# D-Hank/NeRF-tiny

Hardware: AMD Instinct MI355X
Metric: rays/sec (64 coarse + 128 fine samples), lego 400x400 (higher is better)
Workload: dtype f32

## Files before the change

### nerf-tiny_amd/csrc/api.hip

```cpp
#include <math.h>
#include <stdlib.h>

#include <atomic>
#include <mutex>

#include "api_common.h"
#include "bf16_common.h"

using namespace nerf;

thread_local char nerf::g_err[512] = "";

namespace {

int next_pow2(int n) {
  int p = 2;
  while (p < n) p <<= 1;
  return p;
}

int check_sizes(int B, int Nc, int Nf) {
  if (B < 2) return fail(NERF_HIP_ERR_ARG, "B=%d: the reference needs B >= 2 (nerf.py:208 .squeeze())", B);
  if (Nc < 2 || Nc > 1024 || Nf < 1 || Nf > 1024) return fail(NERF_HIP_ERR_ARG, "Nc=%d Nf=%d outside 2..1024 / 1..1024", Nc, Nf);
  if ((long long)B * (Nc + Nf) + DUMP_ROWS + 256 >= (1ll << 31))
// ... 119 lines not shown
  }
  L.total = c.o;
  return L;
}

struct Prof {
  std::atomic<bool> on{false};
  std::mutex mu;
  int cap = 0, used = 0, pool_used = 0;
  hipEvent_t* ev = nullptr;
  hipEvent_t* e0 = nullptr;
  hipEvent_t* e1 = nullptr;
  int* kid = nullptr;
} g_prof;

struct ProfChain {
  hipEvent_t last = nullptr;
};

struct ProfScope {
  hipStream_t st;
  hipEvent_t stop = nullptr;
  ProfChain* chain;
  ProfScope(int kernel_id, hipStream_t s, ProfChain* ch = nullptr) : st(s), chain(ch) {
    if (!g_prof.on.load(std::memory_order_acquire)) return;
    hipEvent_t start = nullptr;
    bool record_start = false;
    {
      std::lock_guard<std::mutex> lk(g_prof.mu);
      if (g_prof.on.load(std::memory_order_relaxed) && g_prof.used < g_prof.cap) {
        const int slot = g_prof.used++;
        g_prof.kid[slot] = kernel_id;
        if (chain && chain->last) {
          start = chain->last;
        } else {
          start = g_prof.ev[g_prof.pool_used++];
          record_start = true;
        }
        stop = g_prof.ev[g_prof.pool_used++];
        g_prof.e0[slot] = start;
        g_prof.e1[slot] = stop;
      }
    }
    if (record_start) (void)hipEventRecord(start, st);
  }
  ~ProfScope() {
    if (stop) (void)hipEventRecord(stop, st);
    if (chain) chain->last = stop;
  }
};

}

extern "C" {

int nerf_hip_abi_version(void) { return NERF_HIP_ABI_VERSION; }

const char* nerf_hip_last_error(void) { return g_err; }

int nerf_hip_ws_bytes(int B, int Nc, int Nf, int flags, size_t* bytes) {
  if (!bytes) return fail(NERF_HIP_ERR_ARG, "bytes is null");
  if (int rc = check_sizes(B, Nc, Nf)) return rc;
  *bytes = layout(B, Nc, Nf, flags).total;
  return NERF_HIP_OK;
}

}

namespace {
struct TrainLoss {
  const float* C_true;
  float *dC_c, *dC_f, *terms, *loss;
  bool fused;
};
int forward_impl(const float* const* weights24, const int64_t* row, const int64_t* col, const float* poses_bound, const float* K_inv9,
                 const float* ray0_near_far, int B, int Nc, int Nf, float last_delta, float* C_coarse, float* C_fine, void* ws, size_t ws_bytes,
                 int flags, void* stream, TrainLoss* tl, float* maps = nullptr);
int backward_impl(const float* const* weights24, const float* dC_coarse, const float* dC_fine, const float* ray0_near_far, int B, int Nc, int Nf,
                  float last_delta, float* const* dweights24, void* ws, size_t ws_bytes, int flags, void* stream, void* early_event,
                  const TrainLoss* tl, const float* dmaps = nullptr);
}

extern "C" {

int nerf_hip_forward(const float* const* weights24, const int64_t* row, const int64_t* col, const float* poses_bound,
                     const float* K_inv9, const float* ray0_near_far, int B, int Nc, int Nf, float last_delta, float* C_coarse,
                     float* C_fine, void* ws, size_t ws_bytes, int flags, void* stream) {
  return forward_impl(weights24, row, col, poses_bound, K_inv9, ray0_near_far, B, Nc, Nf, last_delta, C_coarse, C_fine, ws, ws_bytes, flags, stream,
                      nullptr);
}

int nerf_hip_forward_maps(const float* const* weights24, const int64_t* row, const int64_t* col, const float* poses_bound,
                          const float* K_inv9, const float* ray0_near_far, int B, int Nc, int Nf, float last_delta, float* C_coarse,
                          float* C_fine, float* maps, void* ws, size_t ws_bytes, int flags, void* stream) {
  if (flags & NERF_HIP_SAVE_FOR_BACKWARD) return fail(NERF_HIP_ERR_ARG, "nerf_hip_forward_maps is inference only (NERF_HIP_SAVE_FOR_BACKWARD set)");
  if (!maps) return fail(NERF_HIP_ERR_ARG, "maps is null");
  return forward_impl(weights24, row, col, poses_bound, K_inv9, ray0_near_far, B, Nc, Nf, last_delta, C_coarse, C_fine, ws, ws_bytes, flags, stream,
                      nullptr, maps);
}

int nerf_hip_forward_maps_train(const float* const* weights24, const int64_t* row, const int64_t* col, const float* poses_bound,
                                const float* K_inv9, const float* ray0_near_far, int B, int Nc, int Nf, float last_delta, float* C_coarse,
                                float* C_fine, float* maps, void* ws, size_t ws_bytes, int flags, void* stream) {
  if (!(flags & NERF_HIP_SAVE_FOR_BACKWARD))
    return fail(NERF_HIP_ERR_ARG, "nerf_hip_forward_maps_train is training only (NERF_HIP_SAVE_FOR_BACKWARD not set)");
  if (!maps) return fail(NERF_HIP_ERR_ARG, "maps is null");
  return forward_impl(weights24, row, col, poses_bound, K_inv9, ray0_near_far, B, Nc, Nf, last_delta, C_coarse, C_fine, ws, ws_bytes, flags, stream,
                      nullptr, maps);
}

}

namespace {

int forward_impl(const float* const* weights24, const int64_t* row, const int64_t* col, const float* poses_bound, const float* K_inv9,
                 const float* ray0_near_far, int B, int Nc, int Nf, float last_delta, float* C_coarse, float* C_fine, void* ws, size_t ws_bytes,
                 int flags, void* stream, TrainLoss* tl, float* maps) {
  if (int rc = check_sizes(B, Nc, Nf)) return rc;
  if (int rc = check_weights(weights24)) return rc;
  if (!row || !col || !poses_bound || !K_inv9 || !C_coarse || !C_fine || !ws) return fail(NERF_HIP_ERR_ARG, "null argument");
  const WsLayout L = layout(B, Nc, Nf, flags);
  if (int rc = check_ws(ws, ws_bytes, L.total)) return rc;
  if (int rc = check_device()) return rc;
  hipStream_t st = static_cast<hipStream_t>(stream);
  const bool save = (flags & NERF_HIP_SAVE_FOR_BACKWARD) != 0;
  const bool bf16 = (flags & NERF_HIP_BF16_MLP) != 0;
  const bool bf16x = bf16 && !save && !(flags & NERF_HIP_FORCE_TILE_KERNEL);
  const bool split = (flags & NERF_HIP_SPLIT_MLP) && !bf16;
  const Weights24 w = as_w24(weights24);

  ProfChain pc;
  const bool one_prep = bf16 && !split && !prep_bf16_disabled();
  const bool corrected = (flags & NERF_HIP_CORRECTED) != 0;
  const bool pair = bf16x && Nc == 64 && Nf == 128 && pair_bf16(B) && !corrected && !maps;
  if (!(flags & NERF_HIP_WEIGHTS_UNCHANGED) && !one_prep) {
    ProfScope ps(NERF_HIP_K_PACK, st, &pc);
    if (bf16 || split) HIP_TRY(launch_fold_weights(w, at<float>(ws, L.fold), st));
    if (split) {
      HIP_TRY(launch_pack_weights_split(w, at<float>(ws, L.fold), at<unsigned char>(ws, L.packed_sp), st));
      if (save) HIP_TRY(launch_pack_weights_split_bwd(w, at<float>(ws, L.fold), at<unsigned char>(ws, L.packed_sp_bwd), st));
    } else
    if (bf16 && bf16x) HIP_TRY(launch_pack_weights_bf16x(w, at<float>(ws, L.fold), at<unsigned char>(ws, L.packed_bf), st));
    else if (bf16) HIP_TRY(launch_pack_weights_bf16(w, at<float>(ws, L.fold), at<unsigned char>(ws, L.packed_bf), st));
    else HIP_TRY(launch_pack_weights(w, at<float>(ws, L.fold), at<float4>(ws, L.packed), save ? NSEG : NSEG_FWD, st));
  }

  RaysArgs ra;
  memset(&ra, 0, sizeof(ra));
  ra.row = row; ra.col = col; ra.pb = poses_bound;
  memcpy(ra.K, K_inv9, 9 * sizeof(float));
  ra.B = B; ra.Nc = Nc;
  ra.rayf = at<float>(ws, L.rayf);
  ra.dvec = (bf16 || split) ? nullptr : at<float>(ws, L.dvec);
  ra.w_dir = w.p[W_DIR]; ra.b_dir = w.p[B_DIR];
  ra.b_fold = at<float>(ws, L.fold);
  ra.t_c = at<float>(ws, L.t_c);
  ra.status = at<unsigned>(ws, L.status);
  static std::atomic<unsigned> g_token{0};
  unsigned token = ++g_token;
  if ((token & 0xffffffu) == 0) token = ++g_token;
  if (one_prep) {
    const bool pack = !(flags & NERF_HIP_WEIGHTS_UNCHANGED);
    RaysArgs rp = ra;
    if (pair) rp.B = 0;
    if (pack || rp.B > 0) {
      ProfScope ps(pack ? NERF_HIP_K_PACK : NERF_HIP_K_RAYS, st, &pc);
      HIP_TRY(launch_prep_bf16(w, at<float>(ws, L.fold), pack ? at<unsigned char>(ws, L.packed_bf) : nullptr, bf16x ? 1 : 0,
                               pack && save ? at<unsigned char>(ws, L.packed_bf_bwd) : nullptr,
                               reinterpret_cast<unsigned*>(at<float>(ws, L.fold) + FOLD_FLOATS), token,
                               at<unsigned>(ws, L.status) + STATUS_STICKY_WORD, rp, st));
    }
  } else if (!pair) {
    ProfScope ps(NERF_HIP_K_RAYS, st, &pc);
    HIP_TRY(launch_rays(ra, st));
  }

  FieldArgs fa;
  memset(&fa, 0, sizeof(fa));
  fa.wp = at<float4>(ws, L.packed);
  if (bf16) fa.wbf = at<unsigned char>(ws, L.packed_bf);
  if (split) fa.wbf = at<unsigned char>(ws, L.packed_sp);
  fa.w = w;
  fa.rayf = at<float>(ws, L.rayf);
  fa.dvec = at<float>(ws, L.dvec);
  fa.t = at<float>(ws, L.t_c);
  fa.rgb = at<float>(ws, L.rgb_c);
  fa.sigma = at<float>(ws, L.sig_c);
  fa.N = Nc; fa.M = B * Nc;
#ifdef NERF_STAMPS
  fa.stamps = at<unsigned long long>(ws, L.dbg);
#endif
  const int tiles_c = (B * Nc + TM - 1) / TM, tiles_f = (B * Nf + TM - 1) / TM;
  if (save) {
    fa.spre = at<float>(ws, L.spre);
    fa.row0 = 0; fa.tile0 = 0; fa.tiles_tot = tiles_c + tiles_f; fa.Mtot = (long long)B * (Nc + Nf); fa.MSrows = fa.Mtot + DUMP_ROWS;
    if (bf16 || split) {
      fa.bsave = at<unsigned char>(ws, L.bsave); fa.bmask = at<uint16_t>(ws, L.bmask);
      if (split) fa.bsave2 = at<unsigned char>(ws, L.bsave2);
      fa.wb0 = 0; fa.wb_tot = (int)(wave_blocks(B, Nc) + wave_blocks(B, Nf));
    } else {
      fa.save = at<float>(ws, L.save); fa.masks = at<uint16_t>(ws, L.masks);
    }
  }
  if (pair) {
    PairArgs pa;
    memset(&pa, 0, sizeof(pa));
    pa.wbf = at<unsigned char>(ws, L.packed_bf); pa.rays = ra; pa.rays.status = nullptr; pa.B = B; pa.gen = token & 0xffffffu;
    if (ray0_near_far) { pa.ray0_override = 1; pa.near0 = ray0_near_far[0]; pa.far0 = ray0_near_far[1]; }
    pa.last = last_delta; pa.C_coarse = C_coarse; pa.C_fine = C_fine;
    pa.status = at<uint32_t>(ws, L.status); pa.sticky = at<uint32_t>(ws, L.status) + STATUS_STICKY_WORD;
    pa.sig_c = at<float>(ws, L.sig_c); pa.rgb_c = at<float>(ws, L.rgb_c); pa.w_c = at<float>(ws, L.w_c); pa.t_f = at<float>(ws, L.t_f);
    pa.sig_f = at<float>(ws, L.sig_f); pa.rgb_f = at<float>(ws, L.rgb_f);
    ProfScope ps(NERF_HIP_K_RENDER_PAIR, st, &pc);
    HIP_TRY(launch_render_pair_bf16x(pa, st));
    return NERF_HIP_OK;
  }
  const bool fuse_rays = bf16 && save && Nc == 64 && Nf == 128 && fuse_rays_bf16(B) && !corrected && !maps;
  FwdFuse ff;
  memset(&ff, 0, sizeof(ff));
  const bool tile_kernel = (flags & NERF_HIP_FORCE_TILE_KERNEL) != 0;
  auto field = [&](const FieldArgs& f) { return split ? launch_field_fwd_split(f, save, st) : bf16x ? launch_field_fwd_bf16x(f, st) : bf16 ? launch_field_fwd_bf16(f, save, st, ff.mode ? &ff : nullptr) : tile_kernel ? launch_field_fwd(f, save, st) : launch_field_fwd_reg(f, save, st); };

  CoarseArgs ca;
  memset(&ca, 0, sizeof(ca));
  ca.t_c = at<float>(ws, L.t_c); ca.sigma = at<float>(ws, L.sig_c); ca.rgb = at<float>(ws, L.rgb_c);
  ca.rayf = at<float>(ws, L.rayf);
  ca.B = B; ca.Nc = Nc; ca.Nf = Nf;
  ca.delta0_mode = 0;
  if (ray0_near_far) { ca.ray0_override = 1; ca.near0 = ray0_near_far[0]; ca.far0 = ray0_near_far[1]; }
  ca.w_c = at<float>(ws, L.w_c); ca.C_coarse = C_coarse; ca.t_f = at<float>(ws, L.t_f);
  ca.status = at<uint32_t>(ws, L.status);
  ca.sticky = at<uint32_t>(ws, L.status) + STATUS_STICKY_WORD;
  if (fuse_rays) {
    ff.mode = 1; ff.c = ca;
    { ProfScope ps(NERF_HIP_K_FIELD_COARSE, st, &pc); HIP_TRY(field(fa)); }
    ff.mode = 0;
  } else {
    { ProfScope ps(NERF_HIP_K_FIELD_COARSE, st, &pc); HIP_TRY(field(fa)); }
    { ProfScope ps(NERF_HIP_K_COARSE, st, &pc); HIP_TRY(launch_coarse(ca, st, maps)); }
  }

  fa.t = at<float>(ws, L.t_f);
  fa.rgb = at<float>(ws, L.rgb_f);
  fa.sigma = at<float>(ws, L.sig_f);
  fa.N = Nf; fa.M = B * Nf;
  if (save) { fa.row0 = B * Nc; fa.tile0 = tiles_c; fa.wb0 = (int)wave_blocks(B, Nc); }
  MergeArgs ma;
  memset(&ma, 0, sizeof(ma));
  ma.t_c = at<float>(ws, L.t_c); ma.t_f = at<float>(ws, L.t_f);
  ma.sig_c = at<float>(ws, L.sig_c); ma.sig_f = at<float>(ws, L.sig_f);
  ma.rgb_c = at<float>(ws, L.rgb_c); ma.rgb_f = at<float>(ws, L.rgb_f);
  ma.B = B; ma.Nc = Nc; ma.Nf = Nf; ma.P = next_pow2(Nc + Nf);
  ma.last = last_delta;
  ma.joint = corrected ? 1 : 0;
  if (save) { ma.bundle = at<float>(ws, L.bundle); ma.w = at<float>(ws, L.w_m); ma.perm = at<uint16_t>(ws, L.perm); }
  ma.C_fine = C_fine;
  if (fuse_rays) {
    ff.mode = 2; ff.m = ma;
    if (tl) {
      ff.C_true = tl->C_true; ff.C_coarse = C_coarse; ff.dC_c = tl->dC_c; ff.dC_f = tl->dC_f; ff.loss_terms = tl->terms;
      tl->fused = true;
    }
    { ProfScope ps(NERF_HIP_K_FIELD_FINE, st, &pc); HIP_TRY(field(fa)); }
  } else {
    { ProfScope ps(NERF_HIP_K_FIELD_FINE, st, &pc); HIP_TRY(field(fa)); }
    { ProfScope ps(NERF_HIP_K_MERGE, st, &pc); HIP_TRY(launch_merge(ma, st, maps)); }
  }
  return NERF_HIP_OK;
}

}

extern "C" {

int nerf_hip_profile_begin(int max_launches) {
  if (g_prof.ev) return fail(NERF_HIP_ERR_ARG, "profile already active");
  if (max_launches < 1 || max_launches > (1 << 20)) return fail(NERF_HIP_ERR_ARG, "bad max_launches");
  g_prof.ev = new hipEvent_t[2 * (size_t)max_launches];
  g_prof.e0 = new hipEvent_t[max_launches];
  g_prof.e1 = new hipEvent_t[max_launches];
  g_prof.kid = new int[max_launches];
  for (int i = 0; i < 2 * max_launches; ++i) HIP_TRY(hipEventCreate(&g_prof.ev[i]));
  g_prof.cap = max_launches;
  g_prof.used = 0;
  g_prof.pool_used = 0;
  g_prof.on.store(true, std::memory_order_release);
  return NERF_HIP_OK;
}

int nerf_hip_profile_end(double* ms_sum, int* count, int n_kernels) {
  if (!g_prof.ev) return fail(NERF_HIP_ERR_ARG, "profile not active");
  {
    std::lock_guard<std::mutex> lk(g_prof.mu);
    g_prof.on.store(false, std::memory_order_release);
  }
  for (int k = 0; k < n_kernels; ++k) { if (ms_sum) ms_sum[k] = 0.0; if (count) count[k] = 0; }
  int rc = NERF_HIP_OK;
  for (int i = 0; i < g_prof.used; ++i) {
    float ms = 0.f;
    hipError_t e = hipEventSynchronize(g_prof.e1[i]);
    if (e == hipSuccess) e = hipEventElapsedTime(&ms, g_prof.e0[i], g_prof.e1[i]);
    if (e != hipSuccess) { rc = fail(NERF_HIP_ERR_DEVICE, "profile event: %s", hipGetErrorString(e)); break; }
    const int k = g_prof.kid[i];
    if (k >= 0 && k < n_kernels) { if (ms_sum) ms_sum[k] += ms; if (count) count[k] += 1; }
  }
  for (int i = 0; i < 2 * g_prof.cap; ++i) (void)hipEventDestroy(g_prof.ev[i]);
// ... 156 lines not shown
    sg.save = save; sg.G = G; sg.dz = at<float>(ws, L.dz); sg.dspre = at<float>(ws, L.dspre); sg.rayf = at<float>(ws, L.rayf);
    sg.Mtot = Mtot; sg.MSrows = Mtot + DUMP_ROWS; sg.B = B; sg.Nc = Nc; sg.Nf = Nf;
    sg.dW_color = dw[W_COLOR]; sg.db_color = dw[B_COLOR]; sg.dw_sigma = dw[W_SIGMA]; sg.db_sigma = dw[B_SIGMA]; sg.dW_dir = dw[W_DIR];
    sg.sbuf = at<float>(ws, L.sbuf); sg.gdbuf = at<float>(ws, L.gdbuf); sg.sums_done = ray_duty ? 1 : 0;
    HIP_TRY(launch_small_grads(sg, slabs, st));
  }
  return NERF_HIP_OK;
}

}

extern "C" {

int nerf_hip_train_step(const float* const* weights24, const int64_t* row, const int64_t* col, const float* poses_bound,
                        const float* K_inv9, const float* ray0_near_far, const float* C_true, int B, int Nc, int Nf, float last_delta,
                        float* C_coarse, float* C_fine, float* loss, float* const* dweights24, void* ws, size_t ws_bytes, int flags,
                        void* stream, void* early_event) {
  if (!C_true || !loss || !C_coarse || !C_fine) return fail(NERF_HIP_ERR_ARG, "null argument");
  flags |= NERF_HIP_SAVE_FOR_BACKWARD;
  if (int rc = check_weights(const_cast<const float* const*>(dweights24))) return rc;
  if (int rc = check_sizes(B, Nc, Nf)) return rc;
  if (!ws) return fail(NERF_HIP_ERR_ARG, "null argument");
  const WsLayout L = layout(B, Nc, Nf, flags);
  if (ws_bytes < L.total) return fail(NERF_HIP_ERR_WORKSPACE, "workspace %zu < %zu bytes", ws_bytes, L.total);
  TrainLoss tl;
  tl.C_true = C_true; tl.dC_c = at<float>(ws, L.dC); tl.dC_f = tl.dC_c + (size_t)B * 3; tl.terms = tl.dC_f + (size_t)B * 3; tl.loss = loss;
  tl.fused = false;
  if (int rc = forward_impl(weights24, row, col, poses_bound, K_inv9, ray0_near_far, B, Nc, Nf, last_delta, C_coarse, C_fine, ws, ws_bytes, flags,
                            stream, &tl))
    return rc;
  if (!tl.fused)
    if (int rc = nerf_hip_ray_loss(C_coarse, C_fine, C_true, B, loss, tl.dC_c, tl.dC_f, stream)) return rc;
  return backward_impl(weights24, tl.dC_c, tl.dC_f, ray0_near_far, B, Nc, Nf, last_delta, dweights24, ws, ws_bytes,
                       flags & ~NERF_HIP_WEIGHTS_UNCHANGED, stream, early_event, &tl);
}

int nerf_hip_ws_offset(int B, int Nc, int Nf, int flags, const char* name, size_t* offset) {
  if (!name || !offset) return fail(NERF_HIP_ERR_ARG, "null argument");
  if (int rc = check_sizes(B, Nc, Nf)) return rc;
  const WsLayout L = layout(B, Nc, Nf, flags);
  struct { const char* n; size_t o; } tab[] = {
      {"status", L.status}, {"dbg", L.dbg}, {"packed", L.packed}, {"packed_bf", L.packed_bf}, {"bsave", L.bsave}, {"bsave2", L.bsave2}, {"bmask", L.bmask}, {"bG", L.bG}, {"bG2", L.bG2}, {"rayf", L.rayf}, {"dvec", L.dvec}, {"t_c", L.t_c}, {"sig_c", L.sig_c},
      {"rgb_c", L.rgb_c}, {"w_c", L.w_c}, {"t_f", L.t_f}, {"sig_f", L.sig_f}, {"rgb_f", L.rgb_f}, {"perm", L.perm},
      {"w_m", L.w_m}, {"bundle", L.bundle}, {"save", L.save}, {"masks", L.masks}, {"spre", L.spre}, {"G", L.G}, {"dz", L.dz},
      {"dspre", L.dspre}, {"mbuf", L.mbuf}, {"fold", L.fold}, {"drgb_c", L.drgb_c}, {"dsig_c", L.dsig_c}, {"drgb_f", L.drgb_f}, {"dsig_f", L.dsig_f},
      {"dt_f", L.dt_f}, {"slabs", L.slabs}, {"masks", L.masks}, {"sbuf", L.sbuf}, {"gdbuf", L.gdbuf}};
  for (auto& e : tab)
    if (strcmp(e.n, name) == 0) {
      if (e.o == 0 && strcmp(name, "status") != 0) return fail(NERF_HIP_ERR_ARG, "buffer %s is not part of this layout (flags=%d)", name, flags);
      *offset = e.o;
      return NERF_HIP_OK;
    }
  return fail(NERF_HIP_ERR_ARG, "unknown workspace buffer %s", name);
}

int nerf_hip_ray_loss(const float* C_coarse, const float* C_fine, const float* C_true, int B, float* loss, float* dC_coarse,
                      float* dC_fine, void* stream) {
  if (!C_coarse || !C_fine || !C_true || !loss || B < 1) return fail(NERF_HIP_ERR_ARG, "null argument");
  HIP_TRY(launch_ray_loss(C_coarse, C_fine, C_true, B, loss, dC_coarse, dC_fine, static_cast<hipStream_t>(stream)));
  return NERF_HIP_OK;
}

int nerf_hip_read_status(const void* ws, size_t ws_bytes, uint32_t* status, void* stream) {
  if (!ws || !status || ws_bytes < 256) return fail(NERF_HIP_ERR_ARG, "null argument");
  hipStream_t st = static_cast<hipStream_t>(stream);
  uint32_t w[STATUS_STICKY_WORD + 3];
  memset(w, 0, sizeof(w));
  HIP_TRY(hipMemcpyAsync(w, ws, sizeof(w), hipMemcpyDeviceToHost, st));
  HIP_TRY(hipStreamSynchronize(st));
  if (w[STATUS_SCHEME_WORD] == 1u) *status = ((w[STATUS_STAMPED_WORD] >> 8) == w[STATUS_GEN_WORD]) ? (w[STATUS_STAMPED_WORD] & 0xffu) : 0u;
  else *status = w[0] & ~(uint32_t)NERF_HIP_STATUS_PREP_TIMEOUT;
  if (w[STATUS_STICKY_WORD + 1] != 0u && w[STATUS_STICKY_WORD + 1] == w[STATUS_STICKY_WORD + 2]) *status |= NERF_HIP_STATUS_PREP_TIMEOUT;
  return NERF_HIP_OK;
}

int nerf_hip_read_status_sticky(void* ws, size_t ws_bytes, uint32_t* status, int clear, void* stream) {
  if (!ws || !status || ws_bytes < 256) return fail(NERF_HIP_ERR_ARG, "null argument");
  hipStream_t st = static_cast<hipStream_t>(stream);
  uint32_t* word = static_cast<uint32_t*>(ws) + STATUS_STICKY_WORD;
  HIP_TRY(hipMemcpyAsync(status, word, sizeof(uint32_t), hipMemcpyDeviceToHost, st));
  if (clear) HIP_TRY(hipMemsetAsync(word, 0, sizeof(uint32_t), st));
  HIP_TRY(hipStreamSynchronize(st));
  return NERF_HIP_OK;
}

int nerf_hip_rays(const int64_t* row, const int64_t* col, const float* poses_bound, const float* K_inv9, int B, int Nc,
                  float* d_cam, float* d_wrd, float* t_coarse, void* stream) {
  if (!row || !col || !poses_bound || !K_inv9 || B < 1 || Nc < 2) return fail(NERF_HIP_ERR_ARG, "bad argument");
  if (int rc = check_device()) return rc;
  RaysArgs ra;
  memset(&ra, 0, sizeof(ra));
  ra.row = row; ra.col = col; ra.pb = poses_bound;
  memcpy(ra.K, K_inv9, 9 * sizeof(float));
  ra.B = B; ra.Nc = Nc;
  ra.d_cam = d_cam; ra.d_wrd = d_wrd; ra.t_c = t_coarse;
  HIP_TRY(launch_rays(ra, static_cast<hipStream_t>(stream)));
  return NERF_HIP_OK;
}

int nerf_hip_field(const float* const* weights24, const int64_t* row, const int64_t* col, const float* poses_bound,
                   const float* K_inv9, const float* t, int B, int N, float* rgb, float* sigma, float* pts, float* gamma_p,
                   void* ws, size_t ws_bytes, void* stream) {
  if (B < 1 || N < 1 || N > 1024) return fail(NERF_HIP_ERR_ARG, "bad sizes");
  if (int rc = check_weights(weights24)) return rc;
  if (!row || !col || !poses_bound || !K_inv9 || !t || !rgb || !sigma || !ws) return fail(NERF_HIP_ERR_ARG, "null argument");
  const int Nl = N < 2 ? 2 : N;
  const WsLayout L = layout(B < 2 ? 2 : B, Nl, Nl, 0);
  if (ws_bytes < L.total) return fail(NERF_HIP_ERR_WORKSPACE, "workspace %zu < %zu bytes", ws_bytes, L.total);
  if (int rc = check_device()) return rc;
  hipStream_t st = static_cast<hipStream_t>(stream);
  const Weights24 w = as_w24(weights24);
  HIP_TRY(launch_pack_weights(w, at<float>(ws, L.fold), at<float4>(ws, L.packed), NSEG_FWD, st));
  RaysArgs ra;
  memset(&ra, 0, sizeof(ra));
  ra.row = row; ra.col = col; ra.pb = poses_bound;
  memcpy(ra.K, K_inv9, 9 * sizeof(float));
  ra.B = B; ra.Nc = Nl;
  ra.rayf = at<float>(ws, L.rayf);
  ra.dvec = at<float>(ws, L.dvec);
  ra.w_dir = w.p[W_DIR]; ra.b_dir = w.p[B_DIR]; ra.b_fold = at<float>(ws, L.fold);
  HIP_TRY(launch_rays(ra, st));
  FieldArgs fa;
  memset(&fa, 0, sizeof(fa));
  fa.wp = at<float4>(ws, L.packed);
  fa.w = w;
  fa.rayf = at<float>(ws, L.rayf);
  fa.dvec = at<float>(ws, L.dvec);
  fa.t = t; fa.rgb = rgb; fa.sigma = sigma; fa.pts_dbg = pts; fa.gp_dbg = gamma_p;
  fa.N = N; fa.M = B * N;
  HIP_TRY(launch_field_fwd_reg(fa, false, st));
  return NERF_HIP_OK;
}

int nerf_hip_field_bf16(const float* const* weights24, const int64_t* row, const int64_t* col, const float* poses_bound,
                        const float* K_inv9, const float* t, int B, int N, float* rgb, float* sigma, void* ws, size_t ws_bytes,
                        void* stream) {
  if (B < 1 || N < 1 || N > 1024) return fail(NERF_HIP_ERR_ARG, "bad sizes");
  if (int rc = check_weights(weights24)) return rc;
  if (!row || !col || !poses_bound || !K_inv9 || !t || !rgb || !sigma || !ws) return fail(NERF_HIP_ERR_ARG, "null argument");
  const int Nl = N < 2 ? 2 : N;
  const WsLayout L = layout(B < 2 ? 2 : B, Nl, Nl, NERF_HIP_BF16_MLP);
  if (ws_bytes < L.total) return fail(NERF_HIP_ERR_WORKSPACE, "workspace %zu < %zu bytes", ws_bytes, L.total);
  if (int rc = check_device()) return rc;
  hipStream_t st = static_cast<hipStream_t>(stream);
  const Weights24 w = as_w24(weights24);
  HIP_TRY(launch_fold_weights(w, at<float>(ws, L.fold), st));
  HIP_TRY(launch_pack_weights_bf16(w, at<float>(ws, L.fold), at<unsigned char>(ws, L.packed_bf), st));
  RaysArgs ra;
  memset(&ra, 0, sizeof(ra));
  ra.row = row; ra.col = col; ra.pb = poses_bound;
  memcpy(ra.K, K_inv9, 9 * sizeof(float));
  ra.B = B; ra.Nc = Nl;
  ra.rayf = at<float>(ws, L.rayf);
  HIP_TRY(launch_rays(ra, st));
  FieldArgs fa;
  memset(&fa, 0, sizeof(fa));
  fa.wbf = at<unsigned char>(ws, L.packed_bf);
  fa.w = w;
  fa.rayf = at<float>(ws, L.rayf);
  fa.t = t; fa.rgb = rgb; fa.sigma = sigma;
  fa.N = N; fa.M = B * N;
  HIP_TRY(launch_field_fwd_bf16(fa, false, st));
  return NERF_HIP_OK;
}

int nerf_hip_coarse_composite(const float* t_c, const float* sigma_c, const float* rgb_c, const float* near_far, float delta0,
                              int B, int Nc, int Nf, float* w_c, float* C_coarse, float* t_f, uint32_t* status, void* stream) {
  if (!t_c || !sigma_c || !rgb_c || !near_far || !t_f) return fail(NERF_HIP_ERR_ARG, "null argument");
  if (B < 1 || Nc < 2 || Nc > 1024 || Nf < 1 || Nf > 1024) return fail(NERF_HIP_ERR_ARG, "bad sizes");
  CoarseArgs ca;
  memset(&ca, 0, sizeof(ca));
  ca.t_c = t_c; ca.sigma = sigma_c; ca.rgb = rgb_c; ca.near_far = near_far;
  ca.B = B; ca.Nc = Nc; ca.Nf = Nf;
  ca.delta0_mode = 1; ca.delta0 = delta0;
  ca.w_c = w_c; ca.C_coarse = C_coarse; ca.t_f = t_f; ca.status = status;
  HIP_TRY(launch_coarse(ca, static_cast<hipStream_t>(stream)));
  return NERF_HIP_OK;
}

static const int kParamNumel[24] = {256 * 60, 256, 256 * 256, 256, 256 * 256, 256, 256 * 256, 256, 256 * 316, 256, 256 * 256, 256,
                                     256 * 256, 256, 256 * 256, 256, 256, 1, 256 * 256, 256, 128 * 280, 128, 3 * 128, 3};

int nerf_hip_adam_step(float* const* params24, const float* const* grads24, float* exp_avg, float* exp_avg_sq, int step, float lr,
                       float beta1, float beta2, float eps, void* stream) {
  if (!params24 || !grads24 || !exp_avg || !exp_avg_sq || step < 1) return fail(NERF_HIP_ERR_ARG, "bad argument");
  AdamArgs a;
  memset(&a, 0, sizeof(a));
  int off = 0;
  for (int i = 0; i < 24; ++i) {
    if (!params24[i] || !grads24[i]) return fail(NERF_HIP_ERR_ARG, "null tensor %d", i);
    a.param[i] = params24[i]; a.grad[i] = grads24[i]; a.numel[i] = kParamNumel[i]; a.offset[i] = off;
    off += kParamNumel[i];
  }
  a.m = exp_avg; a.v = exp_avg_sq;
  const double bc1 = 1.0 - pow((double)beta1, (double)step), bc2 = 1.0 - pow((double)beta2, (double)step);
  a.step_size = (float)((double)lr / bc1);
  a.bias2_sqrt = (float)sqrt(bc2);
  a.one_minus_beta1 = 1.0f - beta1; a.beta2 = beta2; a.one_minus_beta2 = 1.0f - beta2; a.eps = eps;
  HIP_TRY(launch_adam(a, static_cast<hipStream_t>(stream)));
  return NERF_HIP_OK;
}

int nerf_hip_gather_rays(const int64_t* index, const float* pixels, const float* poses17, int B, int H, int W, int64_t* row,
                         int64_t* col, int64_t* pic, float* pix_val, float* poses_bound, void* stream) {
  if (!index || !pixels || !poses17 || !row || !col || !pic || !pix_val || !poses_bound || B < 1 || H < 1 || W < 1)
    return fail(NERF_HIP_ERR_ARG, "bad argument");
  GatherArgs g;
  memset(&g, 0, sizeof(g));
  g.index = reinterpret_cast<const long long*>(index); g.pixels = pixels; g.poses = poses17; g.B = B; g.H = H; g.W = W;
  g.row = reinterpret_cast<long long*>(row); g.col = reinterpret_cast<long long*>(col); g.pic = reinterpret_cast<long long*>(pic);
  g.pix_val = pix_val; g.poses_bound = poses_bound;
  HIP_TRY(launch_gather_rays(g, static_cast<hipStream_t>(stream)));
  return NERF_HIP_OK;
}

int nerf_hip_coarse_composite_backward(const float* t_c, const float* sigma_c, const float* rgb_c, const float* near_far,
                                       float delta0, int B, int Nc, int Nf, const float* dC_coarse, const float* dt_f,
                                       float* dsig_c, float* drgb_c, void* stream) {
  if (!t_c || !sigma_c || !rgb_c || !near_far || !dC_coarse || !dt_f || !dsig_c || !drgb_c) return fail(NERF_HIP_ERR_ARG, "null argument");
  if (B < 1 || Nc < 2 || Nc > 1024 || Nf < 1 || Nf > 1024) return fail(NERF_HIP_ERR_ARG, "bad sizes");
  CoarseBwdArgs cb;
  memset(&cb, 0, sizeof(cb));
  cb.dC_c = dC_coarse; cb.dt_f = dt_f; cb.t_c = t_c; cb.sigma = sigma_c; cb.rgb = rgb_c; cb.near_far = near_far;
  cb.B = B; cb.Nc = Nc; cb.Nf = Nf; cb.delta0_mode = 1; cb.delta0 = delta0;
  cb.drgb_c = drgb_c; cb.dsig_c = dsig_c;
  HIP_TRY(launch_coarse_bwd(cb, static_cast<hipStream_t>(stream)));
  return NERF_HIP_OK;
}

int nerf_hip_merge_composite(const float* t_c, const float* t_f, const float* sigma_c, const float* sigma_f, const float* rgb_c,
                             const float* rgb_f, int B, int Nc, int Nf, float last_delta, float* bundle, float* w, float* C_fine,
                             void* stream) {
  if (!t_c || !t_f || !sigma_c || !sigma_f || !rgb_c || !rgb_f || !C_fine) return fail(NERF_HIP_ERR_ARG, "null argument");
  if (B < 1 || Nc < 1 || Nf < 1 || Nc + Nf > 2048) return fail(NERF_HIP_ERR_ARG, "bad sizes");
  MergeArgs ma;
  memset(&ma, 0, sizeof(ma));
  ma.t_c = t_c; ma.t_f = t_f; ma.sig_c = sigma_c; ma.sig_f = sigma_f; ma.rgb_c = rgb_c; ma.rgb_f = rgb_f;
  ma.B = B; ma.Nc = Nc; ma.Nf = Nf; ma.P = next_pow2(Nc + Nf); ma.last = last_delta;
  ma.bundle = bundle; ma.w = w; ma.C_fine = C_fine;
  HIP_TRY(launch_merge(ma, static_cast<hipStream_t>(stream)));
  return NERF_HIP_OK;
}

}
```

### nerf-tiny_amd/csrc/bf16_stream.h

```cpp
#pragma once
#include "bf16_common.h"
#include "field_common.h"

#include <stdlib.h>
#include <type_traits>
#include <utility>

namespace nerf {

typedef __bf16 bf16x8 __attribute__((ext_vector_type(8)));
typedef __bf16 bf16x2 __attribute__((ext_vector_type(2)));
typedef float f32x2 __attribute__((ext_vector_type(2)));
typedef short s16x2 __attribute__((ext_vector_type(2)));
typedef unsigned u32x4 __attribute__((ext_vector_type(4)));
typedef void __attribute__((address_space(3)))* lptr_t;

constexpr int BF_NS = 8;
constexpr int BF_SYNC_POS = 8;
constexpr int BF_D = 6;
constexpr int BF_EPI_POS = 2;
constexpr int BF_WG = 512;
constexpr int BF_LDS_BYTES = BF_BIAS_BYTES + BF_NS * BF_CHUNK * BF_FRAG_BYTES;
constexpr int BF_SMALL_MAX_WGS = 256;
inline bool bf16_four_waves_disabled() {
// ... 60 lines not shown
  c.lane = threadIdx.x & 63;
  c.wv = __builtin_amdgcn_readfirstlane(threadIdx.x >> 6);
  return c;
}

__device__ __forceinline__ void glds16(const unsigned char* gsrc, unsigned lds_dst) {
  unsigned keep;
  asm volatile("s_mov_b32 %0, m0\n\ts_mov_b32 m0, %2\n\ts_nop 0\n\tglobal_load_lds_dwordx4 %1, off\n\ts_mov_b32 m0, %0"
               : "=&s"(keep)
               : "v"(gsrc), "s"(lds_dst)
               : "memory");
}

__device__ __forceinline__ void store_piece(unsigned char* dst, const u32x4& v) {
  __builtin_nontemporal_store(v, reinterpret_cast<u32x4*>(dst));
}

template <class S>
__device__ __forceinline__ void bf_dma_chunk(const BfCtx& c, int chunk) {
  const int slot = chunk % S::NS;
  constexpr int PW = BfPW<S>::v;
#pragma unroll
  for (int e = 0; e < PW; ++e) {
    const int fr = PW * c.wv + e;
    glds16(c.wimg + BF_BIAS_BYTES + ((size_t)chunk * BF_CHUNK + fr) * BF_FRAG_BYTES + c.lane * 16,
           c.lds_base + S::RING_OFF + (slot * BF_CHUNK + fr) * BF_FRAG_BYTES);
  }
}

template <class S>
__device__ __forceinline__ constexpr int bf_wait_count(int c) {
  const int last = (c + S::NS - 2 < S::NCHUNK - 1) ? c + S::NS - 2 : S::NCHUNK - 1;
  const int loads = (last >= c + 2) ? BfPW<S>::v * (last - (c + 2) + 1) : 0;
  const int c_req = c + 2 - S::NS;
  const int now = S::stores_before(c * BF_CHUNK + BF_SYNC_POS);
  const int then = c_req >= 0 ? S::stores_before(c_req * BF_CHUNK + BF_SYNC_POS) : -S::PROLOGUE_STORES;
  const int n = loads + (now - then);
  return n > 63 ? 63 : n;
}

template <class S, int chunk>
__device__ __forceinline__ void bf_sync(const BfCtx& c) {
  wait_vmcnt<bf_wait_count<S>(chunk)>();
  __builtin_amdgcn_s_barrier();
  asm volatile("" ::: "memory");
  if (chunk + S::NS - 1 < S::NCHUNK) bf_dma_chunk<S>(c, chunk + S::NS - 1);
}

template <class S>
__device__ __forceinline__ void bf_stream_start(const BfCtx& c) {
  if constexpr (S::HAS_BIAS) {
    constexpr int PW = BfPW<S>::v;
#pragma unroll
    for (int e = 0; e < PW; ++e) {
      const int fr = PW * c.wv + e;
      glds16(c.wimg + fr * BF_FRAG_BYTES + c.lane * 16, c.lds_base + fr * BF_FRAG_BYTES);
    }
  }
#pragma unroll
  for (int ch = 0; ch < S::NS - 1; ++ch) bf_dma_chunk<S>(c, ch);
}

template <class S>
__device__ __forceinline__ u32x4 bf_frag(const BfCtx& c, int idx) {
  const int slot = (idx / BF_CHUNK) % S::NS;
  return *reinterpret_cast<const u32x4*>(c.lds + S::RING_OFF + (slot * BF_CHUNK + idx % BF_CHUNK) * BF_FRAG_BYTES + c.lane * 16);
}

template <class S>
__device__ __forceinline__ void bf_stream_first(const BfCtx& c, u32x4 (&fr)[S::D]) {
  constexpr int n = BfPW<S>::v * (S::NS - 2) + S::PROLOGUE_STORES;
  wait_vmcnt<(n > 63 ? 63 : n)>();
  __builtin_amdgcn_s_barrier();
  asm volatile("" ::: "memory");
  static_assert(S::D <= BF_CHUNK - BF_SYNC_POS, "a prefetched fragment must not lie in an unpublished chunk");
#pragma unroll
  for (int i = 0; i < S::D; ++i) fr[i] = bf_frag<S>(c, i);
}

__device__ __forceinline__ f32x16 bf_bias_tile(const BfCtx& c, int tile) {
  const int h = c.lane >> 5;
  f32x16 a;
#pragma unroll
  for (int g = 0; g < 4; ++g) {
    const float4 q = *reinterpret_cast<const float4*>(c.lds + (tile * 32 + 8 * g + 4 * h) * 4);
    a[4 * g + 0] = q.x;
    a[4 * g + 1] = q.y;
    a[4 * g + 2] = q.z;
    a[4 * g + 3] = q.w;
  }
  return a;
}

__device__ __forceinline__ f32x16 bf_mfma(const u32x4& a, const u32x4& b, const f32x16& c) {
  return __builtin_amdgcn_mfma_f32_32x32x16_bf16(__builtin_bit_cast(bf16x8, a), __builtin_bit_cast(bf16x8, b), c, 0, 0, 0);
}

template <class S, int ROW, class Epi, class PrevEpi>
__device__ __forceinline__ void bf_segment(const BfCtx& c, u32x4 (&fr)[S::D], f32x16 (&acc)[2], const u32x4* inA, const u32x4* inB,
                                           Epi&& epi, PrevEpi&& prev_epi) {
  constexpr BfSeg G = S::SEGS[ROW];
  constexpr int S0 = G.s0, NFT = G.nft, KSA = G.ksa, KSB = G.ksb, BT0 = G.bt0, KS = KSA + KSB;
  constexpr int P0 = bf_seg_p0(S::SEGS, ROW), NEXT_BT = bf_seg_next_bt(S::SEGS, S::NSEG, ROW);
  static_assert(KS > BF_EPI_POS + 1, "segment too short for the deferred epilogue");
  const f32x16 zero = {0.f, 0.f, 0.f, 0.f, 0.f, 0.f, 0.f, 0.f, 0.f, 0.f, 0.f, 0.f, 0.f, 0.f, 0.f, 0.f};
  static_for<NFT * KS>([&](auto I) {
    constexpr int f = I / KS, ks = I % KS, idx = S0 + I;
    constexpr int cur = (P0 + f) & 1, oth = (P0 + f + 1) & 1;
    if constexpr (idx % BF_CHUNK == BF_SYNC_POS) bf_sync<S, idx / BF_CHUNK>(c);
    const u32x4 a = fr[idx % S::D];
    if constexpr (idx + S::D < S::NFRAG) fr[idx % S::D] = bf_frag<S>(c, idx + S::D);
    if constexpr (ks < KSA)
      acc[cur] = bf_mfma(a, inA[ks], acc[cur]);
    else
      acc[cur] = bf_mfma(a, inB[ks - KSA], acc[cur]);
    if constexpr (ks == BF_EPI_POS) {
      if constexpr (f == 0)
        prev_epi(acc[oth]);
      else
        epi(f - 1, acc[oth]);
      if constexpr (f + 1 < NFT)
        acc[oth] = BT0 >= 0 ? bf_bias_tile(c, BT0 + f + 1) : zero;
      else if constexpr (NEXT_BT >= 0)
        acc[oth] = bf_bias_tile(c, NEXT_BT);
      else
        acc[oth] = zero;
    }
  });
}

template <int NFRAG_>
struct BfStoreTable {
  int cum[NFRAG_ + 1];
};
constexpr int bf_burst_kstep(int parts, int next_ks) { return BF_EPI_POS + (parts == 2 && next_ks >= BF_EPI_POS + 8 ? 7 : 0); }
template <int NFRAG_, int PARTS>
constexpr BfStoreTable<NFRAG_> bf_store_table(const BfSeg* segs, int nseg, int mul, int extra) {
  constexpr int NSTEP = NFRAG_ / PARTS;
  BfStoreTable<NFRAG_> t{};
  int ev[NSTEP + 1] = {};
  for (int r = 0; r < nseg; ++r) {
    if (segs[r].pieces == 0) continue;
    const int e = bf_seg_end(segs[r]) + bf_burst_kstep(PARTS, r + 1 < nseg ? bf_seg_ks(segs[r + 1]) : 0);
    if (e < NSTEP) ev[e] += mul * segs[r].pieces + extra;
  }
  int run = 0, step = 0;
  for (int i = 0; i <= NFRAG_; ++i) {
    while (step < i / PARTS) run += ev[step++];
    t.cum[i] = run;
  }
  return t;
}

template <int L>
__device__ __forceinline__ void encode_pair(const float (&v)[3], const uint32_t (&freq_bits)[L], int pi, float& sv, float& cv) {
  sv = 0.f;
  cv = 0.f;
  if (pi < 3 * L) {
    const int cc = pi / L, l = pi - L * cc;
    const float x = (cc == 0) ? v[0] : ((cc == 1) ? v[1] : v[2]);
    sincos_phase(x * __uint_as_float(freq_bits[l]), sv, cv);
  }
}
__device__ __forceinline__ void encode_point_pair(const float (&p)[3], int pi, float& sv, float& cv) { encode_pair(p, kFreqPointBits, pi, sv, cv); }
__device__ __forceinline__ void encode_dir_pair(const float (&d)[3], int pi, float& sv, float& cv) { encode_pair(d, kFreqDirBits, pi, sv, cv); }

}
```

### nerf-tiny_amd/csrc/common.h

```cpp
#pragma once
#include <hip/hip_runtime.h>
#include <stddef.h>
#include <stdint.h>

namespace nerf {

constexpr int WIDTH = 256;
constexpr int POINT_DIM = 60;
constexpr int DIR_DIM = 24;
constexpr int L_POINT = 10;
constexpr int L_DIR = 4;
constexpr int HALF = 128;
constexpr int TM = 64;
constexpr int STATUS_GEN_WORD = 1, STATUS_SCHEME_WORD = 2, STATUS_STAMPED_WORD = 3;
constexpr int STATUS_STICKY_WORD = 32;
constexpr int DBG_WORDS = 16384;
constexpr int DUMP_ROWS = 64;
constexpr int RAYF = 24;

enum { RF_R = 0, RF_O = 9, RF_DCAM = 12, RF_DWRD = 15, RF_NEAR = 18, RF_FAR = 19, RF_STEP = 20, RF_DELTA = 21 };

struct Seg { int off4; int nft; int kb; };
constexpr int SEG_L0 = 0, SEG_L1 = 1, SEG_L2 = 2, SEG_L3 = 3, SEG_L4A = 4, SEG_L4B = 5, SEG_L5 = 6, SEG_L6 = 7,
              SEG_L7 = 8, SEG_PI = 9, SEG_DIR = 10, SEG_FOLD = 11, NSEG_FWD = 12;
constexpr int SEG_T_DIR = 12, SEG_T_PI = 13, SEG_T_L7 = 14, SEG_T_L6 = 15, SEG_T_L5 = 16, SEG_T_L4A = 17, SEG_T_L4B = 18,
              SEG_T_L3 = 19, SEG_T_L2 = 20, SEG_T_L1 = 21, SEG_T_L0 = 22, SEG_T_FOLD = 23, NSEG = 24;

__host__ __device__ constexpr int seg_nft(int s) {
  return (s == SEG_DIR || s == SEG_FOLD) ? 4 : (s == SEG_T_L4B || s == SEG_T_L0) ? 2 : 8;
}
__host__ __device__ constexpr int seg_kb(int s) {
  return (s == SEG_L0 || s == SEG_L4B) ? 8 : (s == SEG_T_DIR || s == SEG_T_FOLD) ? 16 : 32;
}
__host__ __device__ constexpr int seg_off4(int s) {
  int o = 0;
  for (int i = 0; i < s; ++i) o += seg_nft(i) * seg_kb(i) * 64;
  return o;
}
constexpr int PACKED_FWD_F4 = seg_off4(NSEG_FWD);
constexpr int PACKED_ALL_F4 = seg_off4(NSEG);

#define NERF_FREQ_POINT_BITS 0x40490fdbu, 0x40d928aeu, 0x416a8b6cu, 0x41fd527bu, 0x4288cd33u, 0x4313c0fau, 0x439f953cu, 0x442c5befu, 0x44ba2881u, 0x45490fdbu
__device__ __constant__ const uint32_t kFreqPointBits[10] = {NERF_FREQ_POINT_BITS};
constexpr uint32_t kFreqPointLit[10] = {NERF_FREQ_POINT_BITS};
__device__ __constant__ const uint32_t kFreqDirBits[4] = {0x40490fdbu, 0x40fd527au, 0x419f953cu, 0x42490fdbu};

enum { W_L0 = 0, B_L0 = 1, W_SIGMA = 16, B_SIGMA = 17, W_PI = 18, B_PI = 19, W_DIR = 20, B_DIR = 21, W_COLOR = 22, B_COLOR = 23 };

struct Weights24 { const float* p[24]; };
constexpr int FOLD_FLOATS = HALF + HALF * WIDTH;
struct Grads24 { float* p[24]; };

struct WsLayout {
  size_t status, dbg, packed, packed_bf, packed_sp, fold, rayf, dvec, t_c, sig_c, rgb_c, w_c, t_f, sig_f, rgb_f;
  size_t packed_bf_bwd, bsave, bmask, bG, bslabs;
  size_t packed_sp_bwd, bsave2, bG2;
  size_t perm, w_m, bundle, save, masks, spre, G, dz, dspre, drgb_c, dsig_c, drgb_f, dsig_f, dt_f, slabs, sbuf, gdbuf, mbuf, dC;
  size_t total;
};

}
```

### nerf-tiny_amd/csrc/field_bwd_bf16.hip

```cpp
#include "bf16_stream.h"
#include "bf16_weights.h"
#include "ray_parts_bwd.h"
#include "ray_parts.h"

#include <string.h>

namespace nerf {

constexpr int BB_NS = 5;
constexpr int BB_MASK_BYTES = 8 * BM_LAYERS * 1024;
constexpr int BB_LDS_BYTES = BB_MASK_BYTES + BB_NS * BF_CHUNK * BF_FRAG_BYTES;

template <bool FINE>
struct BwdStream {
  static constexpr int NFRAG = FINE ? BBF_NFRAG : BBC_NFRAG;
  static constexpr int NCHUNK = FINE ? BBF_NCHUNK : BBC_NCHUNK;
  static constexpr int NS = BB_NS, RING_OFF = BB_MASK_BYTES, D = 4;
  static constexpr const BfSeg* SEGS = kBwdSegs;
  static constexpr int NSEG = FINE ? BSEG_N : BSEG_G0T;
  static constexpr bool HAS_BIAS = false;
  static constexpr int PROLOGUE_STORES = 2;
  static constexpr BfStoreTable<NFRAG> tab = bf_store_table<NFRAG, 1>(SEGS, NSEG, 1, 0);
  __device__ static constexpr int stores_before(int idx) { return tab.cum[idx]; }
};

template <bool FINE, int WAVES>
__global__ __launch_bounds__(64 * WAVES, 1) void k_field_bwd_bf16(const FieldBwdArgs a, const BwdFuse fz) {
  extern __shared__ __attribute__((aligned(16))) unsigned char lds[];
  using S = std::conditional_t<WAVES == 4, FourWaves<BwdStream<FINE>>, BwdStream<FINE>>;
  const BfCtx c = bf_ctx(a.wbf, lds);
  const int lane = c.lane, j = lane & 31, h = lane >> 5;
  const int m = blockIdx.x * (32 * WAVES) + c.wv * 32 + j;
  const bool valid = m < a.M;
  const int mc = valid ? m : a.M - 1;
  const int wb = a.wb0 + blockIdx.x * WAVES + c.wv;

  if (fz.mode != 0) {
    float* const scr = reinterpret_cast<float*>(lds);
    auto wave_fence = [] {
      asm volatile("s_waitcnt vmcnt(0) lgkmcnt(0)" ::: "memory");
      __builtin_amdgcn_wave_barrier();
    };
    if (FINE) {
      if (c.wv < WAVES / 4) {
        const int ray = blockIdx.x * (WAVES / 4) + c.wv;
        if (ray < fz.m.B) merge_bwd_ray(fz.m, ray, lane, scr + c.wv * 4 * 192, wave_fence);
      }
      if (blockIdx.x == 0 && fz.loss_terms) ray_loss_sum<64 * WAVES>(fz.loss_terms, 3 * fz.m.B, fz.loss, scr + 4 * 4 * 192, threadIdx.x);
    } else {
      if (c.wv < WAVES / 2) {
        const int ray_raw = blockIdx.x * (WAVES / 2) + c.wv;
        const bool live = ray_raw < fz.c.B;
        float* w = scr + c.wv * (5 * 64 + 64);
        coarse_bwd_ray(fz.c, live ? ray_raw : fz.c.B - 1, live, lane, w, reinterpret_cast<uint16_t*>(w + 5 * 64), wave_fence);
      }
    }
    __syncthreads();
  }
  float dz[3];
#pragma unroll
  for (int ch = 0; ch < 3; ++ch) {
    const float o = a.rgb[(size_t)mc * 3 + ch];
    dz[ch] = valid ? a.drgb[(size_t)mc * 3 + ch] * ((1.0f - o) * o) : 0.f;
  }
  const float sp = a.spre[a.row0 + mc];
  const float sgn = sp > 0.f ? 1.0f : (sp < 0.f ? -1.0f : 0.f);
  const float ds = valid ? a.dsig[mc] * sgn : 0.f;
  u32x4 zin[4];
  zin[0][0] = h == 0 ? pack2(dz[0], dz[1]) : 0u;
  zin[0][1] = h == 0 ? pack2(dz[2], ds) : 0u;
  zin[0][2] = 0u;
  zin[0][3] = 0u;
#pragma unroll
  for (int q = 0; q < 4; ++q) asm volatile("" : "+v"(zin[0][q]));
  zin[1] = zin[2] = zin[3] = u32x4{0u, 0u, 0u, 0u};

#pragma unroll
  for (int l = 0; l < BM_LAYERS; ++l)
    glds16(reinterpret_cast<const unsigned char*>(a.bmask) + ((size_t)l * a.wb_tot + wb) * 1024 + lane * 16,
           c.lds_base + (c.wv * BM_LAYERS + l) * 1024);
  bf_stream_start<S>(c);

  auto grad_piece = [&](int tensor, int ks, const u32x4& v, unsigned lane16) {
    store_piece(a.bG + ((size_t)a.wb_tot * bg_cum(tensor) + (size_t)wb * bg_ks(tensor) + ks) * BF_FRAG_BYTES + lane16, v);
  };
  grad_piece(BG_Z, 0, zin[0], lane * 16);
  grad_piece(BG_Z, 1, zin[1], lane * 16);

  u32x4 fr[S::D];
  bf_stream_first<S>(c, fr);

  u32x4 X[16], Y[16];
  f32x16 acc[2];
  const f32x16 zero = {0.f, 0.f, 0.f, 0.f, 0.f, 0.f, 0.f, 0.f, 0.f, 0.f, 0.f, 0.f, 0.f, 0.f, 0.f, 0.f};
  acc[0] = zero;
  const uint16_t* const mk = reinterpret_cast<const uint16_t*>(lds + c.wv * BM_LAYERS * 1024) + lane * 8;
  auto grad_to = [&](u32x4* out, int tensor, int mlayer, int ntiles = 8) {
    return [&, out, tensor, mlayer, ntiles](int f, const f32x16& A) {
      f32x16 D = A;
      if (mlayer >= 0) {
        const int bits = mk[mlayer * 512 + f];
#pragma unroll
        for (int r = 0; r < 16; ++r)
          D[r] = __uint_as_float(__float_as_uint(A[r]) & (unsigned)__builtin_amdgcn_sbfe(bits, 15 - r, 1));
      }
#pragma unroll
      for (int mh = 0; mh < 2; ++mh)
#pragma unroll
        for (int q = 0; q < 4; ++q) out[2 * f + mh][q] = pack2(D[8 * mh + 2 * q], D[8 * mh + 2 * q + 1]);
      if (f == ntiles - 1) {
        const unsigned lane16 = 16u * lane_id_here();
#pragma unroll
        for (int ks = 0; ks < 16; ++ks)
          if (ks < 2 * ntiles) grad_piece(tensor, ks, out[ks], lane16);
      }
    };
  };
  auto last_of = [](auto epi, int f) { return [epi, f](const f32x16& A) { epi(f, A); }; };
  auto nothing = [](const f32x16&) {};

  bf_segment<S, BSEG_COLT>(c, fr, acc, zin, nullptr, grad_to(X, BG_D, 8, 4), nothing);
  bf_segment<S, BSEG_FOLDT>(c, fr, acc, X, zin, grad_to(Y, BG_L0 + 7, 7), last_of(grad_to(X, BG_D, 8, 4), 3));
  bf_segment<S, BSEG_L7T>(c, fr, acc, Y, nullptr, grad_to(X, BG_L0 + 6, 6), last_of(grad_to(Y, BG_L0 + 7, 7), 7));
  bf_segment<S, BSEG_L6T>(c, fr, acc, X, nullptr, grad_to(Y, BG_L0 + 5, 5), last_of(grad_to(X, BG_L0 + 6, 6), 7));
  bf_segment<S, BSEG_L5T>(c, fr, acc, Y, nullptr, grad_to(X, BG_L0 + 4, 4), last_of(grad_to(Y, BG_L0 + 5, 5), 7));
  bf_segment<S, BSEG_L4T>(c, fr, acc, X, nullptr, grad_to(Y, BG_L0 + 3, 3), last_of(grad_to(X, BG_L0 + 4, 4), 7));
  bf_segment<S, BSEG_L3T>(c, fr, acc, Y, nullptr, grad_to(X, BG_L0 + 2, 2), last_of(grad_to(Y, BG_L0 + 3, 3), 7));
  bf_segment<S, BSEG_L2T>(c, fr, acc, X, nullptr, grad_to(Y, BG_L0 + 1, 1), last_of(grad_to(X, BG_L0 + 2, 2), 7));
  bf_segment<S, BSEG_L1T>(c, fr, acc, Y, nullptr, grad_to(X, BG_L0 + 0, 0), last_of(grad_to(Y, BG_L0 + 1, 1), 7));
  if constexpr (!FINE) {
    grad_to(X, BG_L0 + 0, 0)(7, acc[1]);
  } else {
    f32x16 dgp[2];
    {
      const unsigned lane16 = 16u * lane_id_here();
#pragma unroll
      for (int ks = 0; ks < 16; ++ks)
        Y[ks] = *reinterpret_cast<const u32x4*>(a.bG + ((size_t)a.wb_tot * bg_cum(BG_L0 + 4) + (size_t)wb * 16 + ks) * BF_FRAG_BYTES + lane16);
    }
    bf_segment<S, BSEG_G0T>(c, fr, acc, X, Y, [&](int, const f32x16& A) { dgp[0] = A; },
                                                 last_of(grad_to(X, BG_L0 + 0, 0), 7));
    dgp[1] = acc[1];
    const int lane_e = (int)lane_id_here();
    const int h_e = lane_e >> 5;
    const int m_e = blockIdx.x * (32 * WAVES) + c.wv * 32 + (lane_e & 31);
    const bool valid_e = m_e < a.M;
    const int mcl = valid_e ? m_e : a.M - 1;
    const int ray = mcl / a.N;
    const float* rf = a.rayf + (size_t)ray * RAYF;
    float p[3];
    sample_point(rf, a.t[mcl], p);
    float dp[3] = {0.f, 0.f, 0.f};
#pragma unroll
    for (int g8 = 0; g8 < 8; ++g8)
#pragma unroll
      for (int e = 0; e < 2; ++e) {
        const int pi = 4 * g8 + 2 * h_e + e;
        if (pi < 30) {
          const int cc = pi / 10, l = pi - 10 * cc;
          const float x = (cc == 0) ? p[0] : ((cc == 1) ? p[1] : p[2]);
          const float fl = __uint_as_float(kFreqPointBits[l]);
          float sn, cn;
          sincos_phase(x * fl, sn, cn);
          const float dgs = dgp[g8 >> 2][4 * (g8 & 3) + 2 * e], dgc = dgp[g8 >> 2][4 * (g8 & 3) + 2 * e + 1];
          const float contrib = fl * (cn * dgs - sn * dgc);
          if (cc == 0) dp[0] += contrib; else if (cc == 1) dp[1] += contrib; else dp[2] += contrib;
        }
      }
#pragma unroll
    for (int i = 0; i < 3; ++i) dp[i] += __shfl_xor(dp[i], 32);
    if (valid_e && h_e == 0) {
      const float dtp = __builtin_fmaf(rf[RF_DWRD + 2], dp[2], __builtin_fmaf(rf[RF_DWRD + 1], dp[1], rf[RF_DWRD] * dp[0]));
      a.dt[m_e] += dtp;
    }
  }
}

__global__ __launch_bounds__(256) void k_pack_weights_bf16_bwd(const Weights24 w, const float* __restrict__ fold, unsigned char* __restrict__ img) {
  const int gid = blockIdx.x * 256 + threadIdx.x;
  if (gid >= BBF_NCHUNK * BF_CHUNK * 64) return;
  const int frag = gid >> 6, lane = gid & 63;
  *reinterpret_cast<u32x4*>(img + BF_BIAS_BYTES + (size_t)frag * BF_FRAG_BYTES + lane * 16) = frag_lane_bf16<32, bb_weight>(w, fold, frag, lane);
}

hipError_t launch_pack_weights_bf16_bwd(const Weights24& w, const float* fold, unsigned char* img, hipStream_t st) {
  const int threads = BBF_NCHUNK * BF_CHUNK * 64;
  hipLaunchKernelGGL(k_pack_weights_bf16_bwd, dim3((threads + 255) / 256), dim3(256), 0, st, w, fold, img);
  return hipGetLastError();
}

hipError_t launch_field_bwd_bf16(const FieldBwdArgs& a, bool fine, hipStream_t st, const BwdFuse* fuse) {
  BwdFuse fz;
  if (fuse) fz = *fuse; else memset(&fz, 0, sizeof(fz));
  if (fz.mode && (a.N != (fine ? 128 : 64) || (fz.mode == 1) != fine)) return hipErrorInvalidValue;
  static std::atomic<unsigned long long> opted{0};
  if (hipError_t e = ensure_dynamic_lds(opted, {reinterpret_cast<const void*>(&k_field_bwd_bf16<false, 8>), reinterpret_cast<const void*>(&k_field_bwd_bf16<true, 8>),
                                                reinterpret_cast<const void*>(&k_field_bwd_bf16<false, 4>), reinterpret_cast<const void*>(&k_field_bwd_bf16<true, 4>)}, BB_LDS_BYTES)) return e;
  const int wgs = (a.M + BF_WG / 2 - 1) / (BF_WG / 2);
  if (bf16_small_pass(wgs)) {
    if (fine)
      hipLaunchKernelGGL((k_field_bwd_bf16<true, 4>), dim3(2 * wgs), dim3(256), BB_LDS_BYTES, st, a, fz);
    else
      hipLaunchKernelGGL((k_field_bwd_bf16<false, 4>), dim3(2 * wgs), dim3(256), BB_LDS_BYTES, st, a, fz);
    return hipGetLastError();
  }
  if (fine)
    hipLaunchKernelGGL((k_field_bwd_bf16<true, 8>), dim3(wgs), dim3(BF_WG), BB_LDS_BYTES, st, a, fz);
  else
    hipLaunchKernelGGL((k_field_bwd_bf16<false, 8>), dim3(wgs), dim3(BF_WG), BB_LDS_BYTES, st, a, fz);
  return hipGetLastError();
}

}
```

### nerf-tiny_amd/csrc/field_bwd_reg.hip

```cpp
#include "field_common.h"

namespace nerf {

constexpr int RMB = 32;

template <int NFT>
struct WStageB {
  float4 w[NFT];
};

__device__ __forceinline__ float f4cb(const float4& v, int c) { return c == 0 ? v.x : (c == 1 ? v.y : (c == 2 ? v.z : v.w)); }

__device__ __forceinline__ unsigned mask_word(const uint16_t* __restrict__ mlayer, int t) { return mlayer[((t & 1) * 2) * 256 + (t >> 1) * 64]; }

template <int KB, int NFT, int NKB, int NNFT, bool ZERO_INIT, bool MASK_IN, bool STORE = true, bool HAS_NEXT_MASK = MASK_IN>
__device__ __forceinline__ void reg_layer_bwd(const int seg, const int next_seg , int lane,
                                              const f32x16* prev, f32x16* acc, WStageB<8>& st0, const uint16_t* __restrict__ mlayer,
                                              const uint16_t* __restrict__ mnext, unsigned& mfirst, float* __restrict__ grow, const RegBuf& rb) {
  constexpr int KT = KB / 4;
  WStageB<8> st1;
  const f32x16 zero = {0.f, 0.f, 0.f, 0.f, 0.f, 0.f, 0.f, 0.f, 0.f, 0.f, 0.f, 0.f, 0.f, 0.f, 0.f, 0.f};
  f32x16 tin[2];
  unsigned mw = mfirst;
  auto activate = [&](int t) {
    unsigned mn = 0;
    if (MASK_IN) {
      if (t + 1 < KT) mn = mask_word(mlayer, t + 1);
      else if (mnext != nullptr) mfirst = mask_word(mnext, 0);
    }
#pragma unroll
    for (int r = 0; r < 16; ++r) tin[t & 1][r] = MASK_IN ? (((mw >> r) & 1u) ? prev[t][r] : 0.f) : prev[t][r];
    if (grow == nullptr) {
#pragma unroll
      for (int r = 0; r < 16; ++r) asm volatile("" : "+v"(tin[t & 1][r]));
    }
    if (grow != nullptr) {
#pragma unroll
      for (int g = 0; g < 4; ++g)
        store_row4(grow + 32 * t + 8 * g, make_float4(tin[t & 1][4 * g], tin[t & 1][4 * g + 1], tin[t & 1][4 * g + 2], tin[t & 1][4 * g + 3]));
    }
    if (MASK_IN) mw = mn;
  };
  activate(0);
  auto kblock = [&](int kb, const WStageB<8>& cur, WStageB<8>& ld) {
    if (kb + 1 < KB) {
#pragma unroll
      for (int f = 0; f < NFT; ++f) ld.w[f] = reg_ldw(rb, seg + (int)(f * KB + kb + 1) * 64);
    } else if (next_seg >= 0) {
#pragma unroll
      for (int f = 0; f < NNFT; ++f) ld.w[f] = reg_ldw(rb, next_seg + (int)(f * NKB) * 64);
    }
    __builtin_amdgcn_sched_barrier(0);
    if ((kb & 3) == 2 && (kb >> 2) + 1 < KT) activate((kb >> 2) + 1);
#pragma unroll
    for (int s = 0; s < 4; ++s) {
      const float b = tin[(kb >> 2) & 1][4 * (kb & 3) + s];
#pragma unroll
      for (int f = 0; f < NFT; ++f) {
        if (ZERO_INIT && kb == 0 && s == 0)
          acc[f] = __builtin_amdgcn_mfma_f32_32x32x2f32(f4cb(cur.w[f], s), b, zero, 0, 0, 0);
        else
          acc[f] = __builtin_amdgcn_mfma_f32_32x32x2f32(f4cb(cur.w[f], s), b, acc[f], 0, 0, 0);
      }
    }
  };
#pragma unroll
  for (int kb = 0; kb < KB; kb += 2) {
    kblock(kb, st0, st1);
    kblock(kb + 1, st1, st0);
  }
}

template <int KB, int NKB, int NNFT, bool ZERO_INIT, bool STORE, bool HAS_NEXT_MASK>
__device__ __forceinline__ void reg_layer_bwd_thin(const int seg, const int next_seg , int lane,
                                                   const f32x16* prev, f32x16* acc, WStageB<8>& st0, const uint16_t* __restrict__ mlayer,
                                                   const uint16_t* __restrict__ mnext, unsigned& mfirst, float* __restrict__ grow, const RegBuf& rb) {
  static_assert(KB == 32, "ring indexing below assumes 32 k-blocks");
  constexpr int KT = KB / 4, D = 8;
  WStageB<8> st1;
  const f32x16 zero = {0.f, 0.f, 0.f, 0.f, 0.f, 0.f, 0.f, 0.f, 0.f, 0.f, 0.f, 0.f, 0.f, 0.f, 0.f, 0.f};
  f32x16 tin[2];
  unsigned mw = mfirst;
  auto slot = [&](int kb, int f) -> float4& { return ((kb % D) < 4) ? st0.w[2 * (kb % 4) + f] : st1.w[2 * (kb % 4) + f]; };
  auto activate = [&](int t) {
    unsigned mn = 0;
    if (t + 1 < KT) mn = mask_word(mlayer, t + 1);
    else if (HAS_NEXT_MASK) mfirst = mask_word(mnext, 0);
#pragma unroll
    for (int r = 0; r < 16; ++r) tin[t & 1][r] = ((mw >> r) & 1u) ? prev[t][r] : 0.f;
    if (STORE) {
#pragma unroll
      for (int g = 0; g < 4; ++g)
        store_row4(grow + 32 * t + 8 * g, make_float4(tin[t & 1][4 * g], tin[t & 1][4 * g + 1], tin[t & 1][4 * g + 2], tin[t & 1][4 * g + 3]));
    } else {
#pragma unroll
      for (int r = 0; r < 16; ++r) asm volatile("" : "+v"(tin[t & 1][r]));
    }
    mw = mn;
  };
#pragma unroll
  for (int kb = 1; kb < D; ++kb)
#pragma unroll
    for (int f = 0; f < 2; ++f) slot(kb, f) = reg_ldw(rb, seg + (int)(f * KB + kb) * 64);
  activate(0);
#pragma unroll
  for (int kb = 0; kb < KB; ++kb) {
    if ((kb & 3) == 2 && (kb >> 2) + 1 < KT) activate((kb >> 2) + 1);
    const float4 w0 = slot(kb, 0), w1 = slot(kb, 1);
#pragma unroll
    for (int s = 0; s < 4; ++s) {
      const float b = tin[(kb >> 2) & 1][4 * (kb & 3) + s];
      if (ZERO_INIT && kb == 0 && s == 0) {
        acc[0] = __builtin_amdgcn_mfma_f32_32x32x2f32(f4cb(w0, s), b, zero, 0, 0, 0);
        acc[1] = __builtin_amdgcn_mfma_f32_32x32x2f32(f4cb(w1, s), b, zero, 0, 0, 0);
      } else {
        acc[0] = __builtin_amdgcn_mfma_f32_32x32x2f32(f4cb(w0, s), b, acc[0], 0, 0, 0);
        acc[1] = __builtin_amdgcn_mfma_f32_32x32x2f32(f4cb(w1, s), b, acc[1], 0, 0, 0);
      }
    }
    __builtin_amdgcn_sched_barrier(0);
    if (kb + D < KB) {
#pragma unroll
      for (int f = 0; f < 2; ++f) slot(kb, f) = reg_ldw(rb, seg + (int)(f * KB + kb + D) * 64);
    } else if (kb == KB - 4 && next_seg >= 0) {
#pragma unroll
      for (int f = 0; f < NNFT; ++f) st0.w[f] = reg_ldw(rb, next_seg + (int)(f * NKB) * 64);
    }
    __builtin_amdgcn_sched_barrier(0);
  }
}

#ifdef NERF_STAMPS
#define BSTAMP(slot)                                            \
  do {                                                          \
    __builtin_amdgcn_sched_barrier(0);                          \
    const unsigned long long t_ = __builtin_readcyclecounter(); \
    __builtin_amdgcn_sched_barrier(0);                          \
    tsum[slot] += t_ - tlast;                                   \
    tlast = t_;                                                 \
  } while (0)
#else
#define BSTAMP(slot) do { } while (0)
#endif

template <bool FINE, bool QUERY = false, bool RGB = true>
__global__ __launch_bounds__(64, 1) void k_field_bwd_reg(const FieldBwdArgs a) {
  static_assert(FINE || !QUERY, "the query form carries the chain back to the points");
#ifdef NERF_STAMPS
  unsigned long long tsum[8] = {0, 0, 0, 0, 0, 0, 0, 0};
  unsigned long long tlast = __builtin_readcyclecounter();
#endif
  const int lane = threadIdx.x, j = lane & 31, h = lane >> 5;
  const int m0 = blockIdx.x * RMB;
  const int m = m0 + j;
  const bool valid = m < a.M;
  const int mc = valid ? m : a.M - 1;
  const size_t MS = (size_t)a.MSrows * WIDTH;
  const long long rrow = valid ? (long long)(a.row0 + m) : a.Mtot + j;
  const size_t grow_off = (size_t)rrow * WIDTH + 4 * h;
  float* const grow = a.G + grow_off;
  const float* const srow = a.save + grow_off;
  const uint16_t* const mrow = a.masks + ((size_t)(a.tile0 + (m0 >> 6)) * 4 + ((m0 >> 5) & 1)) * 256 + h * 32 + j;
  const size_t MKS = (size_t)a.tiles_tot * 4 * 256;
  const RegBuf rb = reg_buf(a.wp, threadIdx.x);
  constexpr int L256 = 8 * 32 * 64;
  const f32x16 zero = {0.f, 0.f, 0.f, 0.f, 0.f, 0.f, 0.f, 0.f, 0.f, 0.f, 0.f, 0.f, 0.f, 0.f, 0.f, 0.f};

  WStageB<8> st0;
  if constexpr (RGB) {
#pragma unroll
    for (int f = 0; f < 8; ++f) st0.w[f] = reg_ldw(rb, seg_off4(SEG_T_FOLD) + (f * 16) * 64);
  } else {
#pragma unroll
    for (int f = 0; f < 8; ++f) st0.w[f] = reg_ldw(rb, seg_off4(SEG_T_L7) + (f * 32) * 64);
  }
  auto mlayer = [&](int layer) { return mrow + (size_t)layer * MKS; };
  unsigned mfirst = mask_word(mlayer(7), 0);

  f32x16 D0[4];
  float ds;
  {
    const float* crow = QUERY ? a.save + (size_t)a.MSrows * QGRAD_GP + (size_t)rrow * QGRAD_C + 4 * h : srow + S_C * MS;
    float4 cv[4][4];
    float dz[3];
    if constexpr (RGB) {
#pragma unroll
      for (int t = 0; t < 4; ++t)
#pragma unroll
        for (int g = 0; g < 4; ++g) cv[t][g] = *reinterpret_cast<const float4*>(crow + 32 * t + 8 * g);
#pragma unroll
      for (int ch = 0; ch < 3; ++ch) {
        const float o = a.rgb[(size_t)mc * 3 + ch];
        const float up = a.drgb[(size_t)mc * 3 + ch];
        dz[ch] = valid ? up * ((1.0f - o) * o) : 0.f;
      }
    }
    const float sp = a.spre[a.row0 + mc];
    const float sgn = sp > 0.f ? 1.0f : (sp < 0.f ? -1.0f : 0.f);
    if constexpr (QUERY)
      ds = valid ? (a.dsig != nullptr ? a.dsig[mc] : 1.0f) * sgn : 0.f;
    else
      ds = valid ? a.dsig[mc] * sgn : 0.f;
    if (!QUERY && valid && h == 0) {
      *reinterpret_cast<float4*>(a.dz + (size_t)(a.row0 + m) * 4) = make_float4(dz[0], dz[1], dz[2], ds);
      a.dspre[a.row0 + m] = ds;
    }
    const float* wc = a.w.p[W_COLOR] + 4 * h;
#pragma unroll
    for (int t = 0; t < (RGB ? 4 : 0); ++t) {
      float4 q0[4], q1[4], q2[4];
#pragma unroll
      for (int g = 0; g < 4; ++g) {
        q0[g] = *reinterpret_cast<const float4*>(wc + 32 * t + 8 * g);
        q1[g] = *reinterpret_cast<const float4*>(wc + HALF + 32 * t + 8 * g);
        q2[g] = *reinterpret_cast<const float4*>(wc + 2 * HALF + 32 * t + 8 * g);
      }
      __builtin_amdgcn_sched_barrier(0);
#pragma unroll
      for (int g = 0; g < 4; ++g) {
        const float v0 = __builtin_fmaf(q2[g].x, dz[2], __builtin_fmaf(q1[g].x, dz[1], q0[g].x * dz[0]));
        const float v1 = __builtin_fmaf(q2[g].y, dz[2], __builtin_fmaf(q1[g].y, dz[1], q0[g].y * dz[0]));
        const float v2 = __builtin_fmaf(q2[g].z, dz[2], __builtin_fmaf(q1[g].z, dz[1], q0[g].z * dz[0]));
        const float v3 = __builtin_fmaf(q2[g].w, dz[2], __builtin_fmaf(q1[g].w, dz[1], q0[g].w * dz[0]));
        D0[t][4 * g + 0] = cv[t][g].x > 0.f ? v0 : 0.f;
        D0[t][4 * g + 1] = cv[t][g].y > 0.f ? v1 : 0.f;
        D0[t][4 * g + 2] = cv[t][g].z > 0.f ? v2 : 0.f;
        D0[t][4 * g + 3] = cv[t][g].w > 0.f ? v3 : 0.f;
      }
      __builtin_amdgcn_sched_barrier(0);
    }
  }
  BSTAMP(0);
  f32x16 A[8], B[8];
  {
    const float dsb = (h == 0) ? ds : 0.f;
    const float* ws = a.w.p[W_SIGMA];
#pragma unroll
    for (int f = 0; f < 8; ++f) B[f] = __builtin_amdgcn_mfma_f32_32x32x2f32(ws[f * 32 + j], dsb, zero, 0, 0, 0);
  }
  if constexpr (RGB)
    reg_layer_bwd<16, 8, 32, 8, false, false>(seg_off4(SEG_T_FOLD), seg_off4(SEG_T_L7), lane, D0, B, st0, nullptr, nullptr, mfirst,
                                              QUERY ? a.G : grow + G_D * MS, rb);
  BSTAMP(1);
  BSTAMP(2);
  constexpr int sT7 = seg_off4(SEG_T_L7);
  reg_layer_bwd<32, 8, 32, 8, true, true>(sT7, sT7 + L256, lane, B, A, st0, mlayer(7), mlayer(6), mfirst, QUERY ? a.G : grow + 7 * MS, rb);
  reg_layer_bwd<32, 8, 32, 8, true, true>(sT7 + L256, sT7 + 2 * L256, lane, A, B, st0, mlayer(6), mlayer(5), mfirst, QUERY ? a.G : grow + 6 * MS, rb);
  reg_layer_bwd<32, 8, 32, 8, true, true>(sT7 + 2 * L256, seg_off4(SEG_T_L4A), lane, B, A, st0, mlayer(5), mlayer(4), mfirst, QUERY ? a.G : grow + 5 * MS, rb);
  BSTAMP(3);
  f32x16 accg[2];
  if (FINE) {
    reg_layer_bwd<32, 8, 32, 2, true, true>(seg_off4(SEG_T_L4A), seg_off4(SEG_T_L4B), lane, A, B, st0, mlayer(4), mlayer(4), mfirst, QUERY ? a.G : grow + 4 * MS, rb);
    reg_layer_bwd_thin<32, 32, 8, true, false, true>(seg_off4(SEG_T_L4B), seg_off4(SEG_T_L3), lane, A, accg, st0, mlayer(4), mlayer(3), mfirst, nullptr, rb);
  } else {
    reg_layer_bwd<32, 8, 32, 8, true, true>(seg_off4(SEG_T_L4A), seg_off4(SEG_T_L3), lane, A, B, st0, mlayer(4), mlayer(3), mfirst, grow + 4 * MS, rb);
  }
  BSTAMP(4);
  constexpr int sT3 = seg_off4(SEG_T_L3);
  reg_layer_bwd<32, 8, 32, 8, true, true>(sT3, sT3 + L256, lane, B, A, st0, mlayer(3), mlayer(2), mfirst, QUERY ? a.G : grow + 3 * MS, rb);
  reg_layer_bwd<32, 8, 32, 8, true, true>(sT3 + L256, sT3 + 2 * L256, lane, A, B, st0, mlayer(2), mlayer(1), mfirst, QUERY ? a.G : grow + 2 * MS, rb);
  unsigned mb0[8];
  if (!FINE) {
#pragma unroll
    for (int t = 0; t < 8; ++t) mb0[t] = mask_word(mlayer(0), t);
  }
  reg_layer_bwd<32, 8, 32, 2, true, true, true, FINE>(sT3 + 2 * L256, FINE ? seg_off4(SEG_T_L0) : -1, lane, B, A, st0, mlayer(1),
                                                      mlayer(0), mfirst, QUERY ? a.G : grow + 1 * MS, rb);
  BSTAMP(5);
  if (FINE) {
    reg_layer_bwd_thin<32, 32, 2, false, !QUERY, false>(seg_off4(SEG_T_L0), -1, lane, A, accg, st0, mlayer(0), nullptr, mfirst,
                                                        QUERY ? nullptr : grow, rb);
    const int lane_e = __builtin_amdgcn_mbcnt_hi(~0u, __builtin_amdgcn_mbcnt_lo(~0u, 0u));
    const int j_e = lane_e & 31, h_e = lane_e >> 5;
    const int m_e = blockIdx.x * RMB + j_e;
    const bool valid_e = m_e < a.M;
    const int mc_e = valid_e ? m_e : a.M - 1;
    const long long rrow_e = valid_e ? (long long)(a.row0 + m_e) : a.Mtot + j_e;
    const float* rf = QUERY ? nullptr : a.rayf + (size_t)(mc_e / a.N) * RAYF;
    const float* gprow = QUERY ? a.save + (size_t)rrow_e * QGRAD_GP + 4 * h_e : a.save + (size_t)rrow_e * WIDTH + 4 * h_e + S_GP * ((size_t)a.MSrows * WIDTH);
    float4 gq[8];
#pragma unroll
    for (int g8 = 0; g8 < 8; ++g8) gq[g8] = *reinterpret_cast<const float4*>(gprow + 8 * g8);
    float dp[3] = {0.f, 0.f, 0.f};
#pragma unroll
    for (int g8 = 0; g8 < 8; ++g8)
#pragma unroll
      for (int e = 0; e < 2; ++e) {
        const int pi = 4 * g8 + 2 * h_e + e;
        if (pi < 30) {
          const int c = pi / 10, l = pi - 10 * c;
          const float fl = __uint_as_float(kFreqPointBits[l]);
          const float sn = e == 0 ? gq[g8].x : gq[g8].z, cn = e == 0 ? gq[g8].y : gq[g8].w;
          const float dgs = accg[g8 >> 2][4 * (g8 & 3) + 2 * e], dgc = accg[g8 >> 2][4 * (g8 & 3) + 2 * e + 1];
          const float contrib = fl * (cn * dgs - sn * dgc);
          if (c == 0) dp[0] += contrib; else if (c == 1) dp[1] += contrib; else dp[2] += contrib;
        }
      }
#pragma unroll
    for (int c = 0; c < 3; ++c) dp[c] += __shfl_xor(dp[c], 32);
    if (QUERY && valid_e && h_e == 0) {
#pragma unroll
      for (int c = 0; c < 3; ++c) a.dt[(size_t)m_e * 3 + c] = dp[c];
    }
    if (!QUERY && valid_e && h_e == 0) {
      const float dtp = __builtin_fmaf(rf[RF_DWRD + 2], dp[2], __builtin_fmaf(rf[RF_DWRD + 1], dp[1], rf[RF_DWRD] * dp[0]));
      a.dt[m_e] += dtp;
    }
  } else {
#pragma unroll
    for (int t = 0; t < 8; ++t)
#pragma unroll
      for (int g = 0; g < 4; ++g) {
        float4 v;
        v.x = ((mb0[t] >> (4 * g + 0)) & 1u) ? A[t][4 * g + 0] : 0.f;
        v.y = ((mb0[t] >> (4 * g + 1)) & 1u) ? A[t][4 * g + 1] : 0.f;
        v.z = ((mb0[t] >> (4 * g + 2)) & 1u) ? A[t][4 * g + 2] : 0.f;
        v.w = ((mb0[t] >> (4 * g + 3)) & 1u) ? A[t][4 * g + 3] : 0.f;
        store_row4(grow + 32 * t + 8 * g, v);
      }
  }
#ifdef NERF_STAMPS
  BSTAMP(6);
  if (a.stamps && lane == 0) {
    for (int i = 0; i < 7; ++i) atomicAdd(a.stamps + (FINE ? 8 : 0) + i, tsum[i]);
    atomicAdd(a.stamps + (FINE ? 30 : 31), 1ull);
  }
#endif
}

hipError_t launch_query_grad_bwd(const FieldBwdArgs& a, bool rgb, hipStream_t st) {
  if (a.M <= 0) return hipSuccess;
  const unsigned tiles = (unsigned)(((long long)a.M + RMB - 1) / RMB);
  if (rgb)
    hipLaunchKernelGGL((k_field_bwd_reg<true, true, true>), dim3(tiles), dim3(64), 0, st, a);
  else
    hipLaunchKernelGGL((k_field_bwd_reg<true, true, false>), dim3(tiles), dim3(64), 0, st, a);
  return hipGetLastError();
}

hipError_t launch_field_bwd_reg(const FieldBwdArgs& a, bool fine, hipStream_t st) {
  const int tiles = (a.M + RMB - 1) / RMB;
  if (fine)
    hipLaunchKernelGGL(k_field_bwd_reg<true>, dim3(tiles), dim3(64), 0, st, a);
  else
    hipLaunchKernelGGL(k_field_bwd_reg<false>, dim3(tiles), dim3(64), 0, st, a);
  return hipGetLastError();
}

}
```

### nerf-tiny_amd/csrc/field_bwd_split.hip

```cpp
#include "bf16_split.h"

namespace nerf {

constexpr int SPB_WG = 256;
constexpr int SPB_NS = 7;
constexpr int SPB_MASK_BYTES = 4 * BM_LAYERS * 1024;
constexpr int SPB_LDS_BYTES = SPB_MASK_BYTES + SPB_NS * BF_CHUNK * BF_FRAG_BYTES;
static_assert(SPB_LDS_BYTES <= 160 * 1024, "LDS of one CU");
static_assert((2 * BBC_NFRAG) % BF_CHUNK == 0 && (2 * BBF_NFRAG) % BF_CHUNK == 0, "whole chunks");

template <bool FINE>
struct SplitBwdStream {
  static constexpr int NFRAG = 2 * (FINE ? BBF_NFRAG : BBC_NFRAG), NCHUNK = NFRAG / BF_CHUNK;
  static constexpr int NS = SPB_NS, RING_OFF = SPB_MASK_BYTES, D = 6, PW = 4;
  static constexpr const BfSeg* SEGS = kBwdSegs;
  static constexpr int NSEG = FINE ? BSEG_N : BSEG_G0T;
  static constexpr bool HAS_BIAS = false;
  static constexpr int PROLOGUE_STORES = 4;
  static constexpr BfStoreTable<NFRAG> tab = bf_store_table<NFRAG, 2>(SEGS, NSEG, 2, 0);
  __device__ static constexpr int stores_before(int idx) { return tab.cum[idx]; }
};

template <bool FINE>
__global__ __launch_bounds__(SPB_WG, 1) void k_field_bwd_split(const FieldBwdArgs a) {
  extern __shared__ __attribute__((aligned(16))) unsigned char lds[];
  using S = SplitBwdStream<FINE>;
  const BfCtx c = bf_ctx(a.wbf, lds);
  const int lane = c.lane, j = lane & 31, h = lane >> 5;
  const int m = blockIdx.x * (SPB_WG / 2) + c.wv * 32 + j;
  const bool valid = m < a.M;
  const int mc = valid ? m : a.M - 1;
  const int wb = a.wb0 + blockIdx.x * (SPB_WG / 64) + c.wv;

  float dz[3];
#pragma unroll
  for (int ch = 0; ch < 3; ++ch) {
    const float o = a.rgb[(size_t)mc * 3 + ch];
    dz[ch] = valid ? a.drgb[(size_t)mc * 3 + ch] * ((1.0f - o) * o) : 0.f;
  }
  const float sp = a.spre[a.row0 + mc];
  const float sgn = sp > 0.f ? 1.0f : (sp < 0.f ? -1.0f : 0.f);
  const float ds = valid ? a.dsig[mc] * sgn : 0.f;
  u32x4 zh[4], zm[4];
  {
    const HiMid e0 = split2(dz[0], dz[1]), e1 = split2(dz[2], ds);
    zh[0] = u32x4{h == 0 ? e0.hi : 0u, h == 0 ? e1.hi : 0u, 0u, 0u};
    zm[0] = u32x4{h == 0 ? e0.mid : 0u, h == 0 ? e1.mid : 0u, 0u, 0u};
  }
#pragma unroll
  for (int q = 0; q < 4; ++q) asm volatile("" : "+v"(zh[0][q]), "+v"(zm[0][q]));
  zh[1] = zh[2] = zh[3] = zm[1] = zm[2] = zm[3] = u32x4{0u, 0u, 0u, 0u};

#pragma unroll
  for (int l = 0; l < BM_LAYERS; ++l)
    glds16(reinterpret_cast<const unsigned char*>(a.bmask) + ((size_t)l * a.wb_tot + wb) * 1024 + lane * 16,
           c.lds_base + (c.wv * BM_LAYERS + l) * 1024);
  bf_stream_start<S>(c);

  auto grad_pair = [&](int tensor, int ks, const u32x4& vh, const u32x4& vm, unsigned lane16) {
    const size_t off = ((size_t)a.wb_tot * bg_cum(tensor) + (size_t)wb * bg_ks(tensor) + ks) * BF_FRAG_BYTES + lane16;
    store_piece(a.bG + off, vh);
    store_piece(a.bG2 + off, vm);
  };
  grad_pair(BG_Z, 0, zh[0], zm[0], lane * 16);
  grad_pair(BG_Z, 1, zh[1], zm[1], lane * 16);

  u32x4 fr[S::D];
  bf_stream_first<S>(c, fr);

  u32x4 Xh[16], Xm[16], Yh[16], Ym[16];
  f32x16 acc[2];
  const f32x16 zero = {0.f, 0.f, 0.f, 0.f, 0.f, 0.f, 0.f, 0.f, 0.f, 0.f, 0.f, 0.f, 0.f, 0.f, 0.f, 0.f};
  acc[0] = zero;
  const uint16_t* const mk = reinterpret_cast<const uint16_t*>(lds + c.wv * BM_LAYERS * 1024) + lane * 8;
  auto grad_to = [&](u32x4* oh, u32x4* om, int tensor, int mlayer, int ntiles = 8) {
    return [&, oh, om, tensor, mlayer, ntiles](int f, int part, int ph, const f32x16& A, EpiTmp& t) {
      const int mh = part >> 2, q = part & 3, r = 8 * mh + 2 * q;
      if (ph == 0) {
        const int bits = mk[mlayer * 512 + f];
        t.x0 = __uint_as_float(__float_as_uint(A[r]) & (unsigned)__builtin_amdgcn_sbfe(bits, 15 - r, 1));
        t.x1 = __uint_as_float(__float_as_uint(A[r + 1]) & (unsigned)__builtin_amdgcn_sbfe(bits, 14 - r, 1));
        t.hi = pack2(t.x0, t.x1);
        oh[2 * f + mh][q] = t.hi;
      } else if (ph == 1) {
        t.x0 -= __uint_as_float(t.hi << 16);
        t.x1 -= __uint_as_float(t.hi & 0xffff0000u);
      } else {
        om[2 * f + mh][q] = pack2(t.x0, t.x1);
        if (f == ntiles - 1 && part == 7) {
          const unsigned lane16 = 16u * lane_id_here();
#pragma unroll
          for (int ks = 0; ks < 16; ++ks)
            if (ks < 2 * ntiles) grad_pair(tensor, ks, oh[ks], om[ks], lane16);
        }
      }
    };
  };
  auto last_of = [](auto epi, int f) { return [epi, f](int part, int ph, const f32x16& A, EpiTmp& t) { epi(f, part, ph, A, t); }; };
  auto nothing = [](int, int, const f32x16&, EpiTmp&) {};

  auto gd = grad_to(Xh, Xm, BG_D, 8, 4);
  auto g7 = grad_to(Yh, Ym, BG_L0 + 7, 7), g6 = grad_to(Xh, Xm, BG_L0 + 6, 6), g5 = grad_to(Yh, Ym, BG_L0 + 5, 5), g4 = grad_to(Xh, Xm, BG_L0 + 4, 4);
  auto g3 = grad_to(Yh, Ym, BG_L0 + 3, 3), g2 = grad_to(Xh, Xm, BG_L0 + 2, 2), g1 = grad_to(Yh, Ym, BG_L0 + 1, 1), g0 = grad_to(Xh, Xm, BG_L0 + 0, 0);
  sp_segment<S, BSEG_COLT>(c, fr, acc, zh, zm, nullptr, nullptr, gd, nothing);
  sp_segment<S, BSEG_FOLDT>(c, fr, acc, Xh, Xm, zh, zm, g7, last_of(gd, 3));
  sp_segment<S, BSEG_L7T>(c, fr, acc, Yh, Ym, nullptr, nullptr, g6, last_of(g7, 7));
  sp_segment<S, BSEG_L6T>(c, fr, acc, Xh, Xm, nullptr, nullptr, g5, last_of(g6, 7));
  sp_segment<S, BSEG_L5T>(c, fr, acc, Yh, Ym, nullptr, nullptr, g4, last_of(g5, 7));
  sp_segment<S, BSEG_L4T>(c, fr, acc, Xh, Xm, nullptr, nullptr, g3, last_of(g4, 7));
  sp_segment<S, BSEG_L3T>(c, fr, acc, Yh, Ym, nullptr, nullptr, g2, last_of(g3, 7));
  sp_segment<S, BSEG_L2T>(c, fr, acc, Xh, Xm, nullptr, nullptr, g1, last_of(g2, 7));
  sp_segment<S, BSEG_L1T>(c, fr, acc, Yh, Ym, nullptr, nullptr, g0, last_of(g1, 7));
  if constexpr (!FINE) {
    EpiTmp t = {0.f, 0.f, 0u};
    static_for<8>([&](auto P) { static_for<3>([&](auto PH) { g0(7, (int)P, (int)PH, acc[1], t); }); });
  } else {
    f32x16 dgp[2];
    {
      const unsigned lane16 = 16u * lane_id_here();
#pragma unroll
      for (int ks = 0; ks < 16; ++ks) {
        const size_t off = ((size_t)a.wb_tot * bg_cum(BG_L0 + 4) + (size_t)wb * 16 + ks) * BF_FRAG_BYTES + lane16;
        Yh[ks] = *reinterpret_cast<const u32x4*>(a.bG + off);
        Ym[ks] = *reinterpret_cast<const u32x4*>(a.bG2 + off);
      }
    }
    auto take0 = [&](int, int part, int ph, const f32x16& A, EpiTmp&) { if (part == 0 && ph == 0) dgp[0] = A; };
    sp_segment<S, BSEG_G0T>(c, fr, acc, Xh, Xm, Yh, Ym, take0, last_of(g0, 7));
    dgp[1] = acc[1];
    const int lane_e = (int)lane_id_here();
    const int h_e = lane_e >> 5;
    const int m_e = blockIdx.x * (SPB_WG / 2) + c.wv * 32 + (lane_e & 31);
    const bool valid_e = m_e < a.M;
    const int mcl = valid_e ? m_e : a.M - 1;
    const int ray = mcl / a.N;
    const float* rf = a.rayf + (size_t)ray * RAYF;
    float p[3];
    sample_point(rf, a.t[mcl], p);
    float dp[3] = {0.f, 0.f, 0.f};
#pragma unroll
    for (int g8 = 0; g8 < 8; ++g8)
#pragma unroll
      for (int e = 0; e < 2; ++e) {
        const int pi = 4 * g8 + 2 * h_e + e;
        if (pi < 30) {
          const int cc = pi / 10, l = pi - 10 * cc;
          const float x = (cc == 0) ? p[0] : ((cc == 1) ? p[1] : p[2]);
          const float fl = __uint_as_float(kFreqPointBits[l]);
          float sn, cn;
          sincos_phase(x * fl, sn, cn);
          const float dgs = dgp[g8 >> 2][4 * (g8 & 3) + 2 * e], dgc = dgp[g8 >> 2][4 * (g8 & 3) + 2 * e + 1];
          const float contrib = fl * (cn * dgs - sn * dgc);
          if (cc == 0) dp[0] += contrib; else if (cc == 1) dp[1] += contrib; else dp[2] += contrib;
        }
      }
#pragma unroll
    for (int i = 0; i < 3; ++i) dp[i] += __shfl_xor(dp[i], 32);
    if (valid_e && h_e == 0) {
      const float dtp = __builtin_fmaf(rf[RF_DWRD + 2], dp[2], __builtin_fmaf(rf[RF_DWRD + 1], dp[1], rf[RF_DWRD] * dp[0]));
      a.dt[m_e] += dtp;
    }
  }
}

__global__ __launch_bounds__(256) void k_pack_weights_split_bwd(const Weights24 w, const float* __restrict__ fold, unsigned char* __restrict__ img) {
  const int gid = blockIdx.x * 256 + threadIdx.x;
  if (gid >= BBF_NFRAG * 64) return;
  const int step = gid >> 6, lane = gid & 63;
  const FragHiMid v = frag_lane_split<32, bb_weight>(w, fold, step, lane);
  unsigned char* dst = img + BF_BIAS_BYTES + (size_t)(2 * step) * BF_FRAG_BYTES + lane * 16;
  *reinterpret_cast<u32x4*>(dst) = v.hi;
  *reinterpret_cast<u32x4*>(dst + BF_FRAG_BYTES) = v.mid;
}

size_t split_bwd_image_bytes() { return (size_t)BF_BIAS_BYTES + (size_t)2 * BBF_NFRAG * BF_FRAG_BYTES; }

hipError_t launch_pack_weights_split_bwd(const Weights24& w, const float* fold, unsigned char* img, hipStream_t st) {
  const int threads = BBF_NFRAG * 64;
  hipLaunchKernelGGL(k_pack_weights_split_bwd, dim3((threads + 255) / 256), dim3(256), 0, st, w, fold, img);
  return hipGetLastError();
}

hipError_t launch_field_bwd_split(const FieldBwdArgs& a, bool fine, hipStream_t st) {
  if (!a.wbf || !a.bmask || !a.bG || !a.bG2) return hipErrorInvalidValue;
  static std::atomic<unsigned long long> opted{0};
  if (hipError_t e = ensure_dynamic_lds(opted, {reinterpret_cast<const void*>(&k_field_bwd_split<false>), reinterpret_cast<const void*>(&k_field_bwd_split<true>)},
                                        SPB_LDS_BYTES))
    return e;
  const int wgs = ((a.M + SPB_WG / 2 - 1) / (SPB_WG / 2) + 1) / 2 * 2;
  if (fine)
    hipLaunchKernelGGL(k_field_bwd_split<true>, dim3(wgs), dim3(SPB_WG), SPB_LDS_BYTES, st, a);
  else
    hipLaunchKernelGGL(k_field_bwd_split<false>, dim3(wgs), dim3(SPB_WG), SPB_LDS_BYTES, st, a);
  return hipGetLastError();
}

}
```

### nerf-tiny_amd/csrc/field_fwd_bf16.hip

```cpp
#include "bf16_stream.h"

#include <string.h>
#include "bf16_weights.h"
#include "ray_parts.h"

namespace nerf {

constexpr BfStoreTable<BF_NFRAG> kFwdStoreTable = bf_store_table<BF_NFRAG, 1>(kFwdSegs, FSEG_N, 1, 1);

constexpr int BFW_LDS_BYTES = BF_LDS_BYTES + BF_WG * 32;
static_assert(BFW_LDS_BYTES <= 160 * 1024, "LDS of one CU");

template <bool SAVE>
struct FwdStream {
  static constexpr int NFRAG = BF_NFRAG, NCHUNK = BF_NCHUNK, NS = BF_NS, RING_OFF = BF_BIAS_BYTES, D = BF_D;
  static constexpr const BfSeg* SEGS = kFwdSegs;
  static constexpr int NSEG = FSEG_N;
  static constexpr bool HAS_BIAS = true;
  static constexpr int PROLOGUE_STORES = SAVE ? 6 : 0;
  __device__ static constexpr int stores_before(int idx) { return SAVE ? kFwdStoreTable.cum[idx] : 0; }
};

template <bool SAVE, int WAVES>
__global__ __launch_bounds__(64 * WAVES, 1) void k_field_fwd_bf16(const FieldArgs a, const FwdFuse fz) {
  extern __shared__ __attribute__((aligned(16))) unsigned char lds[];
  const BfCtx c = bf_ctx(a.wbf, lds);
  const int lane = c.lane, j = lane & 31, h = lane >> 5;
  const int m = blockIdx.x * (32 * WAVES) + c.wv * 32 + j;
  const bool valid = m < a.M;
  const int mc = valid ? m : a.M - 1;
  const int ray = mc / a.N;

  const float* rf = a.rayf + (size_t)ray * RAYF;
  float p[3], dw[3];
  sample_point(rf, a.t[mc], p);
#pragma unroll
  for (int i = 0; i < 3; ++i) dw[i] = rf[RF_DWRD + i];
#pragma unroll
  for (int i = 0; i < 3; ++i) asm volatile("" : "+v"(p[i]), "+v"(dw[i]));

  using S = std::conditional_t<WAVES == 4, FourWaves<FwdStream<SAVE>>, FwdStream<SAVE>>;
  bf_stream_start<S>(c);

  u32x4 gp[4], gd[2];
#pragma unroll
  for (int ks = 0; ks < 4; ++ks)
#pragma unroll
    for (int q = 0; q < 4; ++q) {
      float sv, cv;
      encode_point_pair(p, 8 * ks + 2 * h + (q & 1) + 4 * (q >> 1), sv, cv);
      gp[ks][q] = pack2(sv, cv);
    }
#pragma unroll
  for (int ks = 0; ks < 2; ++ks)
#pragma unroll
    for (int q = 0; q < 4; ++q) {
      float sv, cv;
      encode_dir_pair(dw, 8 * ks + 2 * h + (q & 1) + 4 * (q >> 1), sv, cv);
      gd[ks][q] = pack2(sv, cv);
    }

  const int wb = a.wb0 + blockIdx.x * WAVES + c.wv;
  unsigned mw[4];
  auto save_piece = [&](int tensor, int ks, const u32x4& v, unsigned lane16) {
    store_piece(a.bsave + ((size_t)a.wb_tot * bs_cum(tensor) + (size_t)wb * bs_ks(tensor) + ks) * BF_FRAG_BYTES + lane16, v);
  };
  if (SAVE) {
#pragma unroll
    for (int ks = 0; ks < 4; ++ks) save_piece(BS_GP, ks, gp[ks], lane * 16);
#pragma unroll
    for (int ks = 0; ks < 2; ++ks) save_piece(BS_GD, ks, gd[ks], lane * 16);
  }

  u32x4* const gd_park = reinterpret_cast<u32x4*>(lds + BF_LDS_BYTES) + 2 * threadIdx.x;
  gd_park[0] = gd[0];
  gd_park[1] = gd[1];

  u32x4 fr[S::D];
  bf_stream_first<S>(c, fr);

  u32x4 X[16], Y[16];
  f32x16 acc[2];
  acc[0] = bf_bias_tile(c, BFB_L0);
  auto relu_to = [&](u32x4* out, int tensor = -1, int mlayer = -1, int ntiles = 8) {
    return [&, out, tensor, mlayer, ntiles](int f, const f32x16& A) {
#pragma unroll
      for (int mh = 0; mh < 2; ++mh)
#pragma unroll
        for (int q = 0; q < 4; ++q) out[2 * f + mh][q] = pack2_relu(A[8 * mh + 2 * q], A[8 * mh + 2 * q + 1]);
      if constexpr (SAVE) {
        if (f & 1)
          mw[f >> 1] |= alive_bits(A) << 16;
        else
          mw[f >> 1] = alive_bits(A);
        if (f == ntiles - 1) {
          const unsigned lane16 = 16u * lane_id_here();
          u32x4 mv = {mw[0], mw[1], ntiles > 4 ? mw[2] : 0u, ntiles > 4 ? mw[3] : 0u};
          store_piece(reinterpret_cast<unsigned char*>(a.bmask) + ((size_t)mlayer * a.wb_tot + wb) * 1024 + lane16, mv);
#pragma unroll
          for (int ks = 0; ks < 16; ++ks)
            if (ks < 2 * ntiles) save_piece(tensor, ks, out[ks], lane16);
        }
      }
    };
  };
  auto last_of = [](auto epi, int f) { return [epi, f](const f32x16& A) { epi(f, A); }; };
  auto nothing = [](const f32x16&) {};
  auto nothing_f = [](int, const f32x16&) {};

  bf_segment<S, FSEG_L0>(c, fr, acc, gp, nullptr, relu_to(X, BS_H0 + 0, 0), nothing);
  bf_segment<S, FSEG_L1>(c, fr, acc, X, nullptr, relu_to(Y, BS_H0 + 1, 1), last_of(relu_to(X, BS_H0 + 0, 0), 7));
  bf_segment<S, FSEG_L2>(c, fr, acc, Y, nullptr, relu_to(X, BS_H0 + 2, 2), last_of(relu_to(Y, BS_H0 + 1, 1), 7));
  bf_segment<S, FSEG_L3>(c, fr, acc, X, nullptr, relu_to(Y, BS_H0 + 3, 3), last_of(relu_to(X, BS_H0 + 2, 2), 7));
  bf_segment<S, FSEG_L4>(c, fr, acc, Y, gp, relu_to(X, BS_H0 + 4, 4), last_of(relu_to(Y, BS_H0 + 3, 3), 7));
  bf_segment<S, FSEG_L5>(c, fr, acc, X, nullptr, relu_to(Y, BS_H0 + 5, 5), last_of(relu_to(X, BS_H0 + 4, 4), 7));
  bf_segment<S, FSEG_L6>(c, fr, acc, Y, nullptr, relu_to(X, BS_H0 + 6, 6), last_of(relu_to(Y, BS_H0 + 5, 5), 7));
  bf_segment<S, FSEG_L7>(c, fr, acc, X, nullptr, relu_to(Y, BS_H0 + 7, 7), last_of(relu_to(X, BS_H0 + 6, 6), 7));
  float spre = 0.f;
  auto sig_epi = [&](const f32x16& A) { spre = A[0]; };
  bf_segment<S, FSEG_SIG>(c, fr, acc, Y, nullptr, nothing_f, last_of(relu_to(Y, BS_H0 + 7, 7), 7));
  {
    const int lane_d = (int)lane_id_here();
    const u32x4* const back = reinterpret_cast<const u32x4*>(lds + BF_LDS_BYTES) + 2 * (c.wv * 64 + lane_d);
    gd[0] = back[0];
    gd[1] = back[1];
  }
  bf_segment<S, FSEG_DIR>(c, fr, acc, gd, Y, relu_to(X, BS_C, 8, 4), sig_epi);
  const int lane_e = (int)lane_id_here();
  const int m_e = blockIdx.x * (32 * WAVES) + c.wv * 32 + (lane_e & 31);
  const bool out_e = m_e < a.M && lane_e < 32;
  if (out_e) {
    a.sigma[m_e] = fabsf(spre);
    if (SAVE) a.spre[a.row0 + m_e] = spre;
  }
  unsigned char* const park_w = lds + BF_LDS_BYTES + c.wv * 2048;
  if (SAVE && fz.mode != 0 && lane_e < 32) reinterpret_cast<float*>(park_w)[lane_e] = fabsf(spre);
  bf_segment<S, FSEG_COL>(c, fr, acc, X, nullptr, nothing_f, last_of(relu_to(X, BS_C, 8, 4), 3));
  {
    const float r0 = 1.0f / (1.0f + expf(-acc[1][0])), r1 = 1.0f / (1.0f + expf(-acc[1][1])), r2 = 1.0f / (1.0f + expf(-acc[1][2]));
    if (out_e) {
      a.rgb[(size_t)m_e * 3 + 0] = r0;
      a.rgb[(size_t)m_e * 3 + 1] = r1;
      a.rgb[(size_t)m_e * 3 + 2] = r2;
    }
    if (SAVE && fz.mode != 0 && lane_e < 32) {
      float* pr = reinterpret_cast<float*>(park_w + 128) + 3 * lane_e;
      pr[0] = r0; pr[1] = r1; pr[2] = r2;
    }
  }
  if constexpr (SAVE) {
    if (fz.mode != 0) {
      asm volatile("s_waitcnt lgkmcnt(0)" ::: "memory");
      __builtin_amdgcn_s_barrier();
      asm volatile("" ::: "memory");
      float* const scr = reinterpret_cast<float*>(lds + BF_BIAS_BYTES);
      const unsigned char* const park = lds + BF_LDS_BYTES;
      const int lane_f = (int)__builtin_amdgcn_mbcnt_hi(~0u, __builtin_amdgcn_mbcnt_lo(~0u, 0u));
      auto wave_fence = [] {
        asm volatile("s_waitcnt lgkmcnt(0)" ::: "memory");
        __builtin_amdgcn_wave_barrier();
      };
      if (fz.mode == 1) {
        if (c.wv < WAVES / 2) {
          float* w = scr + c.wv * (3 * 64 + 4 * 64);
          float* sg = w + 3 * 64;
          float* cl = sg + 64;
          sg[lane_f] = park_sigma(park, 64 * c.wv + lane_f);
#pragma unroll
          for (int k = 0; k < 3; ++k) cl[3 * lane_f + k] = park_rgb(park, 64 * c.wv + lane_f, k);
          wave_fence();
          const int ray_raw = blockIdx.x * (WAVES / 2) + c.wv;
          const size_t g0 = (size_t)(ray_raw < fz.c.B ? ray_raw : fz.c.B - 1) * 64;
          CoarseArgs ca = fz.c;
          ca.sigma = sg - g0;
          ca.rgb = cl - 3 * g0;
          coarse_ray_stage(ca, ray_raw, lane_f, w, w + 64, w + 128, wave_fence);
        }
      } else {
        constexpr int R = WAVES / 4;
        float* const val0 = scr;
        uint16_t* const idx0 = reinterpret_cast<uint16_t*>(scr + R * 5 * 256);
        for (int j = c.wv; j < 5 * R; j += WAVES) {
          const int rl = j / 5, ch = j - 5 * rl;
          const int ray = blockIdx.x * R + rl;
          if (ray < fz.m.B) merge_channel_job(fz.m, ray, ch, lane_f, val0 + (rl * 5 + ch) * 256, idx0 + (rl * 5 + ch) * 256, park, 128 * rl);
        }
        asm volatile("s_waitcnt lgkmcnt(0)" ::: "memory");
        __builtin_amdgcn_s_barrier();
        asm volatile("" ::: "memory");
        if (c.wv < R) {
          const int ray = blockIdx.x * R + c.wv;
          if (ray < fz.m.B) {
            constexpr int N = 192;
            const size_t gN = (size_t)ray * N;
            float cfin[3];
            merge_ray_composite<true>(val0 + c.wv * 5 * 256, idx0 + c.wv * 5 * 256, 256, N, fz.m.last, lane_f, fz.m.w ? fz.m.w + gN : nullptr,
                                      fz.m.bundle ? fz.m.bundle + gN * 5 : nullptr, fz.m.perm ? fz.m.perm + (size_t)ray * 5 * N : nullptr,
                                      fz.m.C_fine + (size_t)ray * 3, cfin);
            if (fz.C_true) {
              if (lane_f < 3) {
                const size_t e = (size_t)ray * 3 + lane_f;
                const float cf = lane_f == 0 ? cfin[0] : (lane_f == 1 ? cfin[1] : cfin[2]);
                float d1, d2, term;
                ray_loss_element(fz.C_coarse[e], cf, fz.C_true[e], d1, d2, term);
                fz.dC_c[e] = d1;
                fz.dC_f[e] = d2;
                fz.loss_terms[e] = term;
              }
            }
          }
        }
      }
    }
// ... 52 lines not shown
```

### nerf-tiny_amd/csrc/field_fwd_bf16x.hip

```cpp
#include "bf16_stream.h"
#include "bf16_weights.h"
#include "ray_parts.h"
#include "prep_parts.h"

namespace nerf {

typedef float f32x4 __attribute__((ext_vector_type(4)));

constexpr int BXB_SIGMA = 32 * BFB_SIGMA, BXB_DIR = 32 * BFB_DIR, BXB_COL = 32 * BFB_COL;

constexpr int BX_SMALL_MAX_WGS = 256;
constexpr int BX_LDS_BYTES = BF_LDS_BYTES + BF_WG * 32;
static_assert(BX_LDS_BYTES <= 160 * 1024, "LDS of one CU");

struct BxStream {
  static constexpr int NFRAG = BX_NFRAG, NCHUNK = BX_NCHUNK, NS = BF_NS, RING_OFF = BF_BIAS_BYTES, D = BF_D;
  static constexpr bool HAS_BIAS = true;
  static constexpr int PROLOGUE_STORES = 0;
  __device__ static constexpr int stores_before(int) { return 0; }
};
struct BxStream4 : BxStream {
  static constexpr int PW = 4;
};
template <int WAVES> struct BxStreamOf { using type = BxStream; };
template <> struct BxStreamOf<4> { using type = BxStream4; };

template <int NH> struct AccN { f32x4 c[NH]; };

__device__ __forceinline__ f32x4 bx_mfma(const u32x4& a, const u32x4& b, const f32x4& c) {
  return __builtin_amdgcn_mfma_f32_16x16x32_bf16(__builtin_bit_cast(bf16x8, a), __builtin_bit_cast(bf16x8, b), c, 0, 0, 0);
}

template <class S, int NH, int S0, int NT, int KSA, int KSB, int B0, int P0, int NEXT_B, class Epi, class PrevEpi>
__device__ __forceinline__ void bx_segment(const BfCtx& c, u32x4 (&fr)[BF_D], AccN<NH> (&acc)[2], const u32x4 (*inA)[8], const u32x4 (*inB)[8],
                                           Epi&& epi, PrevEpi&& prev_epi) {
  constexpr int KS = KSA + KSB;
  static_assert(KS >= 2, "segment too short for the deferred epilogue");
  const int q = c.lane >> 4;
  auto bias = [&](int off) {
    const float4 v = *reinterpret_cast<const float4*>(c.lds + (off + 4 * q) * 4);
    AccN<NH> a;
#pragma unroll
    for (int h = 0; h < NH; ++h) a.c[h] = f32x4{v.x, v.y, v.z, v.w};
    return a;
  };
  static_for<NT * KS>([&](auto I) {
    constexpr int f = I / KS, ks = I % KS, idx = S0 + I;
    constexpr int cur = (P0 + f) & 1, oth = (P0 + f + 1) & 1;
    if constexpr (idx % BF_CHUNK == BF_SYNC_POS) bf_sync<S, idx / BF_CHUNK>(c);
    const u32x4 a = fr[idx % S::D];
    if constexpr (idx + S::D < S::NFRAG) fr[idx % S::D] = bf_frag<S>(c, idx + S::D);
#pragma unroll
    for (int h = 0; h < NH; ++h) {
      if constexpr (ks < KSA)
        acc[cur].c[h] = bx_mfma(a, inA[h][ks], acc[cur].c[h]);
      else
        acc[cur].c[h] = bx_mfma(a, inB[h][ks - KSA], acc[cur].c[h]);
    }
    if constexpr (ks == 1) {
      if constexpr (f == 0)
        prev_epi(acc[oth]);
      else
        epi(f - 1, acc[oth]);
      if constexpr (f + 1 < NT)
        acc[oth] = bias(B0 + 16 * (f + 1));
      else if constexpr (NEXT_B >= 0)
        acc[oth] = bias(NEXT_B);
    }
  });
}

template <class S, int NH, class Mid>
__device__ __forceinline__ void bx_field_pass(const BfCtx& c, unsigned char* lds, const float (&p)[NH][3], const float (&dw)[NH][3], Mid&& mid,
                                              float (&cpre)[NH][3]) {
  using Acc = AccN<NH>;
  const int q = c.lane >> 4;
  bf_stream_start<S>(c);

  u32x4 gp[NH][8], gd[NH][8];
#pragma unroll
  for (int h = 0; h < NH; ++h) {
#pragma unroll
    for (int s = 0; s < 2; ++s)
#pragma unroll
      for (int e = 0; e < 4; ++e) {
        const int pi = 16 * s + 8 * (e >> 1) + 2 * q + (e & 1);
        float sv = 0.f, cv = 0.f;
        if (pi < 30) {
          const int cc = pi / 10, l = pi - 10 * cc;
          const float x = (cc == 0) ? p[h][0] : ((cc == 1) ? p[h][1] : p[h][2]);
          sincos_phase(x * __uint_as_float(kFreqPointBits[l]), sv, cv);
        }
        gp[h][s][e] = pack2(sv, cv);
      }
#pragma unroll
    for (int e = 0; e < 4; ++e) {
      const int pi = 8 * (e >> 1) + 2 * q + (e & 1);
      float sv = 0.f, cv = 0.f;
      if (pi < 12) {
        const int cc = pi / 4, l = pi - 4 * cc;
        const float x = (cc == 0) ? dw[h][0] : ((cc == 1) ? dw[h][1] : dw[h][2]);
        sincos_phase(x * __uint_as_float(kFreqDirBits[l]), sv, cv);
      }
      gd[h][0][e] = pack2(sv, cv);
    }
  }

  u32x4* const gd_park = reinterpret_cast<u32x4*>(lds + BF_LDS_BYTES) + NH * (c.wv * 64 + c.lane);
#pragma unroll
  for (int h = 0; h < NH; ++h) gd_park[h] = gd[h][0];

  u32x4 fr[BF_D];
  bf_stream_first<S>(c, fr);

  u32x4 X[NH][8], Y[NH][8];
  Acc acc[2];
  {
    const float4 v = *reinterpret_cast<const float4*>(lds + (4 * q) * 4);
#pragma unroll
    for (int h = 0; h < NH; ++h) acc[0].c[h] = f32x4{v.x, v.y, v.z, v.w};
  }
  auto relu_to = [&](u32x4 (*out)[8]) {
    return [out](int f, const Acc& A) {
#pragma unroll
      for (int h = 0; h < NH; ++h) {
        out[h][f >> 1][2 * (f & 1) + 0] = pack2_relu(A.c[h][0], A.c[h][1]);
        out[h][f >> 1][2 * (f & 1) + 1] = pack2_relu(A.c[h][2], A.c[h][3]);
      }
    };
  };
  auto last_of = [](auto epi, int f) { return [epi, f](const Acc& A) { epi(f, A); }; };
  auto nothing = [](const Acc&) {};
  auto nothing_f = [](int, const Acc&) {};

  bx_segment<S, NH, BXS_L0, 16, 2, 0, 0 * 256, 0, 1 * 256>(c, fr, acc, gp, nullptr, relu_to(X), nothing);
  bx_segment<S, NH, BXS_L1, 16, 8, 0, 1 * 256, 0, 2 * 256>(c, fr, acc, X, nullptr, relu_to(Y), last_of(relu_to(X), 15));
  bx_segment<S, NH, BXS_L1 + 128, 16, 8, 0, 2 * 256, 0, 3 * 256>(c, fr, acc, Y, nullptr, relu_to(X), last_of(relu_to(Y), 15));
  bx_segment<S, NH, BXS_L1 + 256, 16, 8, 0, 3 * 256, 0, 4 * 256>(c, fr, acc, X, nullptr, relu_to(Y), last_of(relu_to(X), 15));
  bx_segment<S, NH, BXS_L4, 16, 8, 2, 4 * 256, 0, 5 * 256>(c, fr, acc, Y, gp, relu_to(X), last_of(relu_to(Y), 15));
  bx_segment<S, NH, BXS_L5, 16, 8, 0, 5 * 256, 0, 6 * 256>(c, fr, acc, X, nullptr, relu_to(Y), last_of(relu_to(X), 15));
  bx_segment<S, NH, BXS_L5 + 128, 16, 8, 0, 6 * 256, 0, 7 * 256>(c, fr, acc, Y, nullptr, relu_to(X), last_of(relu_to(Y), 15));
  bx_segment<S, NH, BXS_L5 + 256, 16, 8, 0, 7 * 256, 0, BXB_SIGMA>(c, fr, acc, X, nullptr, relu_to(Y), last_of(relu_to(X), 15));
  float spre[NH] = {};
  auto sig_epi = [&](const Acc& A) {
#pragma unroll
    for (int h = 0; h < NH; ++h) spre[h] = A.c[h][0];
  };
  bx_segment<S, NH, BXS_SIG, 1, 8, 0, BXB_SIGMA, 0, BXB_DIR>(c, fr, acc, Y, nullptr, nothing_f, last_of(relu_to(Y), 15));
  {
    const int lane_d = __builtin_amdgcn_mbcnt_hi(~0u, __builtin_amdgcn_mbcnt_lo(~0u, 0u));
    const u32x4* const back = reinterpret_cast<const u32x4*>(lds + BF_LDS_BYTES) + NH * (c.wv * 64 + lane_d);
#pragma unroll
    for (int h = 0; h < NH; ++h) gd[h][0] = back[h];
  }
  bx_segment<S, NH, BXS_DIR, 8, 1, 8, BXB_DIR, 1, BXB_COL>(c, fr, acc, gd, Y, relu_to(X), sig_epi);
  mid(spre);
  bx_segment<S, NH, BXS_COL, 1, 4, 0, BXB_COL, 1, -1>(c, fr, acc, X, nullptr, nothing_f, last_of(relu_to(X), 7));
#pragma unroll
  for (int h = 0; h < NH; ++h)
#pragma unroll
    for (int ch = 0; ch < 3; ++ch) cpre[h][ch] = acc[1].c[h][ch];
}

template <int NH, int WAVES>
__global__ __launch_bounds__(64 * WAVES, 1) void k_field_fwd_bf16x(const FieldArgs a) {
  extern __shared__ __attribute__((aligned(16))) unsigned char lds[];
  using S = typename BxStreamOf<WAVES>::type;
  const BfCtx c = bf_ctx(a.wbf, lds);
  const int lane = c.lane, n = lane & 15;
  const int m0 = blockIdx.x * (16 * NH * WAVES) + c.wv * (16 * NH);

  int ms[NH];
  bool valid[NH];
  float p[NH][3], dw[NH][3];
#pragma unroll
  for (int h = 0; h < NH; ++h) {
    ms[h] = m0 + 16 * h + n;
    valid[h] = ms[h] < a.M;
    const int mc = valid[h] ? ms[h] : a.M - 1;
    const float* rf = a.rayf + (size_t)(mc / a.N) * RAYF;
    sample_point(rf, a.t[mc], p[h]);
#pragma unroll
    for (int i = 0; i < 3; ++i) dw[h][i] = rf[RF_DWRD + i];
  }
#pragma unroll
  for (int h = 0; h < NH; ++h)
#pragma unroll
    for (int i = 0; i < 3; ++i) asm volatile("" : "+v"(p[h][i]), "+v"(dw[h][i]));

  float cpre[NH][3];
  bx_field_pass<S, NH>(c, lds, p, dw, [&](const float (&spre)[NH]) {
    const int lane_e = __builtin_amdgcn_mbcnt_hi(~0u, __builtin_amdgcn_mbcnt_lo(~0u, 0u));
    const int n_e = lane_e & 15;
    const bool q0_e = lane_e < 16;
#pragma unroll
    for (int h = 0; h < NH; ++h) {
      const int me = m0 + 16 * h + n_e;
      if (me < a.M && q0_e) a.sigma[me] = fabsf(spre[h]);
    }
  }, cpre);
  const int lane_e = __builtin_amdgcn_mbcnt_hi(~0u, __builtin_amdgcn_mbcnt_lo(~0u, 0u));
  const int n_e = lane_e & 15;
  const bool q0_e = lane_e < 16;
#pragma unroll
  for (int h = 0; h < NH; ++h) {
    const int me = m0 + 16 * h + n_e;
    if (me < a.M && q0_e) {
#pragma unroll
      for (int ch = 0; ch < 3; ++ch) a.rgb[(size_t)me * 3 + ch] = 1.0f / (1.0f + expf(-cpre[h][ch]));
    }
  }
}

struct BxStreamNoBias : BxStream {
  static constexpr bool HAS_BIAS = false;
};
constexpr int PAIR_NC = 64, PAIR_NF = 128;
constexpr int PR_SIGC = 72 * 32;
constexpr int PR_RGBC = PR_SIGC + 2 * PAIR_NC;
constexpr int PR_TF = PR_RGBC + 6 * PAIR_NC;
constexpr int PR_SIGF = PR_TF + 2 * PAIR_NF;
constexpr int PR_RGBF = PR_SIGF + 2 * PAIR_NF;
static_assert((PR_RGBF + 6 * PAIR_NF) * 4 <= BF_BIAS_BYTES && PR_SIGC >= 32 * BF_NBIAS_TILES, "results live behind the bias tiles");

__device__ __forceinline__ float rf_lane(const float (&rf)[RAYF], int k) {
  float v = rf[0];
#pragma unroll
  for (int j = 1; j < RAYF; ++j) v = (k == j) ? rf[j] : v;
  return v;
}
__device__ __forceinline__ void status_stamp_or(unsigned* word, unsigned gen, unsigned bits) {
  unsigned cur = __hip_atomic_load(word, __ATOMIC_RELAXED, __HIP_MEMORY_SCOPE_AGENT);
  for (;;) {
    const unsigned want = ((cur >> 8) == gen) ? (cur | bits) : ((gen << 8) | bits);
    if (__hip_atomic_compare_exchange_strong(word, &cur, want, __ATOMIC_RELAXED, __ATOMIC_RELAXED, __HIP_MEMORY_SCOPE_AGENT)) break;
  }
}
__device__ __forceinline__ void wave_lds_fence() {
  asm volatile("s_waitcnt lgkmcnt(0)" ::: "memory");
  __builtin_amdgcn_wave_barrier();
}

__device__ __forceinline__ int lane_id_builtin() { return (int)__builtin_amdgcn_mbcnt_hi(~0u, __builtin_amdgcn_mbcnt_lo(~0u, 0u)); }

__device__ __forceinline__ BfCtx fresh_ctx(const BfCtx& c, unsigned char*& lds) {
  unsigned zero = 0;
  asm volatile("s_mov_b32 %0, 0" : "=s"(zero));
  BfCtx d;
  d.wimg = c.wimg;
  d.lds = lds + zero;
  d.lds_base = c.lds_base + zero;
  d.lane = (int)lane_id_here();
  d.wv = c.wv;
  lds = d.lds;
  return d;
}
__device__ __forceinline__ void pair_coarse_pass(const PairArgs& a, const BfCtx& c, unsigned char* lds, const int r0) {
  float* const res = reinterpret_cast<float*>(lds);
  {
    const int n = c.lane & 15;
    const int s = 16 * c.wv + n, rl = s >> 6, i = s & 63;
    const int ray = min(r0 + rl, a.B - 1);
    float rf[RAYF];
    ray_record(a.rays, ray, rf);
    float p[1][3], dw[1][3];
    sample_point(rf, coarse_depth(rf[RF_NEAR], rf[RF_FAR], rf[RF_STEP], i, PAIR_NC), p[0]);
#pragma unroll
    for (int k = 0; k < 3; ++k) dw[0][k] = rf[RF_DWRD + k];
#pragma unroll
    for (int k = 0; k < 3; ++k) asm volatile("" : "+v"(p[0][k]), "+v"(dw[0][k]));
    float cpre[1][3];
    bx_field_pass<BxStream, 1>(c, lds, p, dw, [&](const float (&spre)[1]) {
      const int le = lane_id_builtin();
      if (le < 16) res[PR_SIGC + 16 * c.wv + le] = fabsf(spre[0]);
    }, cpre);
    const int le = lane_id_builtin();
    if (le < 16) {
      const int se = 16 * c.wv + le;
#pragma unroll
      for (int ch = 0; ch < 3; ++ch) res[PR_RGBC + 3 * se + ch] = 1.0f / (1.0f + expf(-cpre[0][ch]));
    }
  }
}

__device__ __forceinline__ void pair_fine_pass(const PairArgs& a, const BfCtx& c, unsigned char* lds, const int r0) {
  float* const res = reinterpret_cast<float*>(lds);
  {
    const int n = c.lane & 15;
    float p[2][3], dw[2][3];
#pragma unroll
    for (int h = 0; h < 2; ++h) {
      const int s = 32 * c.wv + 16 * h + n, rl = s >> 7;
      const int ray = min(r0 + rl, a.B - 1);
      float rf[RAYF];
      ray_record(a.rays, ray, rf);
      sample_point(rf, res[PR_TF + s], p[h]);
#pragma unroll
      for (int k = 0; k < 3; ++k) dw[h][k] = rf[RF_DWRD + k];
    }
#pragma unroll
    for (int h = 0; h < 2; ++h)
#pragma unroll
      for (int k = 0; k < 3; ++k) asm volatile("" : "+v"(p[h][k]), "+v"(dw[h][k]));
    float cpre[2][3];
    bx_field_pass<BxStreamNoBias, 2>(c, lds, p, dw, [&](const float (&spre)[2]) {
      const int le = lane_id_builtin();
      if (le < 16) {
#pragma unroll
        for (int h = 0; h < 2; ++h) res[PR_SIGF + 32 * c.wv + 16 * h + le] = fabsf(spre[h]);
      }
    }, cpre);
    const int le = lane_id_builtin();
    if (le < 16) {
#pragma unroll
      for (int h = 0; h < 2; ++h) {
        const int se = 32 * c.wv + 16 * h + le;
#pragma unroll
        for (int ch = 0; ch < 3; ++ch) res[PR_RGBF + 3 * se + ch] = 1.0f / (1.0f + expf(-cpre[h][ch]));
      }
    }
  }
}

__global__ __launch_bounds__(BF_WG, 1) void k_render_pair_bf16x(const PairArgs a) {
  extern __shared__ __attribute__((aligned(16))) unsigned char lds[];
  const BfCtx c = bf_ctx(a.wbf, lds);
  float* const res = reinterpret_cast<float*>(lds);
  const int r0 = 2 * blockIdx.x;
  if (blockIdx.x == 0 && threadIdx.x == 0 && a.status) {
    a.status[STATUS_GEN_WORD] = a.gen;
    a.status[STATUS_SCHEME_WORD] = 1u;
  }

  pair_coarse_pass(a, c, lds, r0);
  __syncthreads();
  if (c.wv < 2) {
    const int lane = lane_id_builtin();
    const int rl = c.wv, ray_raw = r0 + rl;
    const bool live = ray_raw < a.B;
    const int ray = live ? ray_raw : a.B - 1;
    float rf[RAYF];
    ray_record(a.rays, ray, rf);
    const float near = rf[RF_NEAR], far = rf[RF_FAR];
    const float n0 = a.ray0_override ? a.near0 : a.rays.pb[15], f0 = a.ray0_override ? a.far0 : a.rays.pb[16];
    const float delta0 = ray0_spacing(n0, f0, PAIR_NC);
    float* scr = reinterpret_cast<float*>(lds + BF_BIAS_BYTES) + rl * 4 * PAIR_NC;
    float* sw = scr, *scdf = scr + PAIR_NC, *stc = scr + 2 * PAIR_NC, *stin = scr + 3 * PAIR_NC;
    const size_t g0 = (size_t)ray * PAIR_NC;
    stin[lane] = coarse_depth(near, far, rf[RF_STEP], lane, PAIR_NC);
    wave_lds_fence();
    float lo, hi;
    coarse_ray_weights(res + PR_SIGC + PAIR_NC * rl, res + PR_RGBC + 3 * PAIR_NC * rl, stin, near, far, PAIR_NC, lane, sw, scdf, stc,
                       (live && a.w_c) ? a.w_c + g0 : nullptr, live ? a.C_coarse + (size_t)ray * 3 : nullptr, lo, hi);
    wave_lds_fence();
    const bool bad = coarse_ray_resample(sw, scdf, stc, lo, hi, delta0, PAIR_NC, PAIR_NF, lane, res + PR_TF + PAIR_NF * rl);
    if (live && bad && a.status) status_stamp_or(a.status + STATUS_STAMPED_WORD, a.gen, 1u);
    if (live && bad && a.sticky) atomicOr(a.sticky, 1u);
    wave_lds_fence();
    if (live) {
      if (lane < RAYF && a.rays.rayf) a.rays.rayf[(size_t)ray * RAYF + lane] = rf_lane(rf, lane);
      if (a.rays.t_c) a.rays.t_c[g0 + lane] = stin[lane];
      if (a.sig_c) a.sig_c[g0 + lane] = res[PR_SIGC + PAIR_NC * rl + lane];
      if (a.rgb_c)
#pragma unroll
        for (int k = 0; k < 3; ++k) a.rgb_c[g0 * 3 + 64 * k + lane] = res[PR_RGBC + 3 * PAIR_NC * rl + 64 * k + lane];
      if (a.t_f)
#pragma unroll
        for (int k = 0; k < 2; ++k) a.t_f[(size_t)ray * PAIR_NF + 64 * k + lane] = res[PR_TF + PAIR_NF * rl + 64 * k + lane];
    }
  }
  __syncthreads();
  {
    unsigned char* lds2 = lds;
    const BfCtx c2 = fresh_ctx(c, lds2);
    pair_fine_pass(a, c2, lds2, r0);
  }
  __syncthreads();
  {
    constexpr int P = 256, N = PAIR_NC + PAIR_NF;
    float* const val_all = reinterpret_cast<float*>(lds + BF_BIAS_BYTES);
    const int lane = lane_id_builtin();
    for (int j = c.wv; j < 10; j += 8) {
      const int rl = j / 5, ch = j - 5 * rl;
      const int ray = min(r0 + rl, a.B - 1);
      const float nearm = a.rays.pb[(size_t)ray * 17 + 15], farm = a.rays.pb[(size_t)ray * 17 + 16];
      const float stepm = (farm - nearm) / (float)(PAIR_NC - 1);
      float v[4];
#pragma unroll
      for (int r = 0; r < 4; ++r) {
        const int i = 4 * lane + r;
        float x;
        if (i < PAIR_NC) {
          const int sc = PAIR_NC * rl + i;
          x = ch == 0 ? coarse_depth(nearm, farm, stepm, i, PAIR_NC) : ch == 4 ? res[PR_SIGC + sc] : res[PR_RGBC + 3 * sc + (ch - 1)];
        } else if (i < N) {
          const int sf = PAIR_NF * rl + (i - PAIR_NC);
          x = ch == 0 ? res[PR_TF + sf] : ch == 4 ? res[PR_SIGF + sf] : res[PR_RGBF + 3 * sf + (ch - 1)];
        } else {
          x = __builtin_nanf("");
        }
        v[r] = x;
      }
      sort256_one_channel(v, lane);
      *reinterpret_cast<float4*>(val_all + (rl * 5 + ch) * P + 4 * lane) = make_float4(v[0], v[1], v[2], v[3]);
    }
    __syncthreads();
    if (c.wv < 2) {
      const int rl = c.wv, ray_raw = r0 + rl;
      const bool live = ray_raw < a.B;
      const int ray = live ? ray_raw : a.B - 1;
      if (live) {
        const size_t gf = (size_t)ray * PAIR_NF;
#pragma unroll
        for (int k = 0; k < 2; ++k)
          if (a.sig_f) a.sig_f[gf + 64 * k + lane] = res[PR_SIGF + PAIR_NF * rl + 64 * k + lane];
#pragma unroll
        for (int k = 0; k < 6; ++k)
          if (a.rgb_f) a.rgb_f[gf * 3 + 64 * k + lane] = res[PR_RGBF + 3 * PAIR_NF * rl + 64 * k + lane];
      }
      float cf[3];
      float* const cout = live ? a.C_fine + (size_t)ray * 3 : cf;
      merge_ray_composite<false>(val_all + rl * 5 * P, nullptr, P, N, a.last, lane, nullptr, nullptr, nullptr, cout);
    }
  }
}

hipError_t launch_render_pair_bf16x(const PairArgs& a, hipStream_t st) {
  static std::atomic<unsigned long long> opted{0};
  if (hipError_t e = ensure_dynamic_lds(opted, {reinterpret_cast<const void*>(&k_render_pair_bf16x)}, BX_LDS_BYTES)) return e;
  hipLaunchKernelGGL(k_render_pair_bf16x, dim3((a.B + 1) / 2), dim3(BF_WG), BX_LDS_BYTES, st, a);
  return hipGetLastError();
}

__global__ __launch_bounds__(256) void k_pack_weights_bf16x(const Weights24 w, const float* __restrict__ fold, unsigned char* __restrict__ img) {
  const int gid = blockIdx.x * 256 + threadIdx.x;
  if (gid >= BX_NCHUNK * BF_CHUNK * 64) return;
  const int frag = gid >> 6, lane = gid & 63;
  *reinterpret_cast<u32x4*>(img + BF_BIAS_BYTES + (size_t)frag * BF_FRAG_BYTES + lane * 16) = frag_lane_bf16<16, bx_weight>(w, fold, frag, lane);
}

hipError_t launch_pack_weights_bf16x(const Weights24& w, const float* fold, unsigned char* img, hipStream_t st) {
  hipError_t e = launch_pack_bias_block_bf16(w, fold, img, st);
  if (e != hipSuccess) return e;
  const int threads = BX_NCHUNK * BF_CHUNK * 64;
  hipLaunchKernelGGL(k_pack_weights_bf16x, dim3((threads + 255) / 256), dim3(256), 0, st, w, fold, img);
  return hipGetLastError();
}

template <int NH, int WAVES>
static hipError_t bx_launch(const FieldArgs& a, hipStream_t st) {
  static std::atomic<unsigned long long> opted{0};
  constexpr int lds_bytes = BF_LDS_BYTES + 64 * WAVES * NH * 16, per_wg = 16 * NH * WAVES;
  static_assert(lds_bytes <= BX_LDS_BYTES, "LDS of one CU");
  if (hipError_t e = ensure_dynamic_lds(opted, {reinterpret_cast<const void*>(&k_field_fwd_bf16x<NH, WAVES>)}, lds_bytes)) return e;
  hipLaunchKernelGGL((k_field_fwd_bf16x<NH, WAVES>), dim3((a.M + per_wg - 1) / per_wg), dim3(64 * WAVES), lds_bytes, st, a);
  return hipGetLastError();
}

// ... 7 lines not shown
```

### nerf-tiny_amd/csrc/field_fwd_split.hip

```cpp
#include "bf16_split.h"

namespace nerf {

constexpr int SP_NFRAG = 2 * BF_NFRAG;
constexpr int SP_NCHUNK = SP_NFRAG / BF_CHUNK;
static_assert(SP_NCHUNK * BF_CHUNK == SP_NFRAG, "whole chunks");
constexpr int SP_WG = 256;

constexpr BfStoreTable<SP_NFRAG> kSplitStoreTable = bf_store_table<SP_NFRAG, 2>(kFwdSegs, FSEG_N, 2, 1);

template <bool SAVE>
struct SplitStreamT {
  static constexpr int NFRAG = SP_NFRAG, NCHUNK = SP_NCHUNK, NS = BF_NS, RING_OFF = BF_BIAS_BYTES, D = 6, PW = 4;
  static constexpr const BfSeg* SEGS = kFwdSegs;
  static constexpr int NSEG = FSEG_N;
  static constexpr bool HAS_BIAS = true;
  static constexpr int PROLOGUE_STORES = SAVE ? 12 : 0;
  __device__ static constexpr int stores_before(int idx) { return SAVE ? kSplitStoreTable.cum[idx] : 0; }
};
using SplitStream = SplitStreamT<false>;
static_assert(BF_SYNC_POS % 2 == 0 && SplitStream::D % 2 == 0, "a step's two fragments stay in one chunk / keep their ring parity");

template <bool SAVE>
__global__ __launch_bounds__(SP_WG, 1) void k_field_fwd_split(const FieldArgs a) {
  extern __shared__ __attribute__((aligned(16))) unsigned char lds[];
  using S = SplitStreamT<SAVE>;
  const BfCtx c = bf_ctx(a.wbf, lds);
  const int lane = c.lane, j = lane & 31, h = lane >> 5;
  const int m = blockIdx.x * (SP_WG / 2) + c.wv * 32 + j;
  const bool valid = m < a.M;
  const int mc = valid ? m : a.M - 1;
  const int ray = mc / a.N;

  const float* rf = a.rayf + (size_t)ray * RAYF;
  float p[3], dw[3];
  sample_point(rf, a.t[mc], p);
#pragma unroll
  for (int i = 0; i < 3; ++i) dw[i] = rf[RF_DWRD + i];
#pragma unroll
  for (int i = 0; i < 3; ++i) asm volatile("" : "+v"(p[i]), "+v"(dw[i]));

  bf_stream_start<S>(c);

  u32x4 gp_hi[4], gp_mid[4], gd_hi[2], gd_mid[2];
#pragma unroll
  for (int ks = 0; ks < 4; ++ks)
#pragma unroll
    for (int q = 0; q < 4; ++q) {
      float sv, cv;
      encode_point_pair(p, 8 * ks + 2 * h + (q & 1) + 4 * (q >> 1), sv, cv);
      const HiMid e = split2(sv, cv);
      gp_hi[ks][q] = e.hi;
      gp_mid[ks][q] = e.mid;
    }
#pragma unroll
  for (int ks = 0; ks < 2; ++ks)
#pragma unroll
    for (int q = 0; q < 4; ++q) {
      float sv, cv;
      encode_dir_pair(dw, 8 * ks + 2 * h + (q & 1) + 4 * (q >> 1), sv, cv);
      const HiMid e = split2(sv, cv);
      gd_hi[ks][q] = e.hi;
      gd_mid[ks][q] = e.mid;
    }

  const int wb = a.wb0 + blockIdx.x * (SP_WG / 64) + c.wv;
  unsigned mw[4];
  auto save_pair = [&](int tensor, int ks, const u32x4& vh, const u32x4& vm, unsigned lane16) {
    const size_t off = ((size_t)a.wb_tot * bs_cum(tensor) + (size_t)wb * bs_ks(tensor) + ks) * BF_FRAG_BYTES + lane16;
    store_piece(a.bsave + off, vh);
    store_piece(a.bsave2 + off, vm);
  };
  if (SAVE) {
#pragma unroll
    for (int ks = 0; ks < 4; ++ks) save_pair(BS_GP, ks, gp_hi[ks], gp_mid[ks], lane * 16);
#pragma unroll
    for (int ks = 0; ks < 2; ++ks) save_pair(BS_GD, ks, gd_hi[ks], gd_mid[ks], lane * 16);
  }

  u32x4 fr[S::D];
  bf_stream_first<S>(c, fr);

  u32x4 Xh[16], Xm[16], Yh[16], Ym[16];
  f32x16 acc[2];
  acc[0] = bf_bias_tile(c, BFB_L0);
  auto relu_to = [&](u32x4* oh, u32x4* om, int tensor = -1, int mlayer = -1, int ntiles = 8) {
    return [&, oh, om, tensor, mlayer, ntiles](int f, int part, int ph, const f32x16& A, EpiTmp& t) {
      const int mh = part >> 2, q = part & 3;
      if (ph == 0) {
        t.x0 = __int_as_float(max(__float_as_int(A[8 * mh + 2 * q]), 0));
        t.x1 = __int_as_float(max(__float_as_int(A[8 * mh + 2 * q + 1]), 0));
        t.hi = pack2(t.x0, t.x1);
        oh[2 * f + mh][q] = t.hi;
        if (SAVE && mlayer >= 0) {
          const unsigned bits = alive_pair(t.x0, t.x1, 8 * mh + 2 * q) << (16 * (f & 1));
          mw[f >> 1] = (part == 0 && (f & 1) == 0) ? bits : (mw[f >> 1] | bits);
        }
      } else if (ph == 1) {
        t.x0 -= __uint_as_float(t.hi << 16);
        t.x1 -= __uint_as_float(t.hi & 0xffff0000u);
      } else {
        om[2 * f + mh][q] = pack2(t.x0, t.x1);
        if (SAVE && tensor >= 0 && f == ntiles - 1 && part == 7) {
          const unsigned lane16 = 16u * lane_id_here();
          if (mlayer >= 0) {
            const u32x4 mv = {mw[0], mw[1], ntiles > 4 ? mw[2] : 0u, ntiles > 4 ? mw[3] : 0u};
            store_piece(reinterpret_cast<unsigned char*>(a.bmask) + ((size_t)mlayer * a.wb_tot + wb) * 1024 + lane16, mv);
          }
#pragma unroll
          for (int ks = 0; ks < 16; ++ks)
            if (ks < 2 * ntiles) save_pair(tensor, ks, oh[ks], om[ks], lane16);
        }
      }
    };
  };
  auto last_of = [](auto epi, int f) { return [epi, f](int part, int ph, const f32x16& A, EpiTmp& t) { epi(f, part, ph, A, t); }; };
  auto nothing = [](int, int, const f32x16&, EpiTmp&) {};
  auto nothing_f = [](int, int, int, const f32x16&, EpiTmp&) {};

  auto e0 = relu_to(Xh, Xm, BS_H0 + 0, 0), e1 = relu_to(Yh, Ym, BS_H0 + 1, 1), e2 = relu_to(Xh, Xm, BS_H0 + 2, 2), e3 = relu_to(Yh, Ym, BS_H0 + 3, 3);
  auto e4 = relu_to(Xh, Xm, BS_H0 + 4, 4), e5 = relu_to(Yh, Ym, BS_H0 + 5, 5), e6 = relu_to(Xh, Xm, BS_H0 + 6, 6), e7 = relu_to(Yh, Ym, BS_H0 + 7, 7);
  auto ec = relu_to(Xh, Xm, BS_C, 8, 4);
  sp_segment<S, FSEG_L0>(c, fr, acc, gp_hi, gp_mid, nullptr, nullptr, e0, nothing);
  sp_segment<S, FSEG_L1>(c, fr, acc, Xh, Xm, nullptr, nullptr, e1, last_of(e0, 7));
  sp_segment<S, FSEG_L2>(c, fr, acc, Yh, Ym, nullptr, nullptr, e2, last_of(e1, 7));
  sp_segment<S, FSEG_L3>(c, fr, acc, Xh, Xm, nullptr, nullptr, e3, last_of(e2, 7));
  sp_segment<S, FSEG_L4>(c, fr, acc, Yh, Ym, gp_hi, gp_mid, e4, last_of(e3, 7));
  sp_segment<S, FSEG_L5>(c, fr, acc, Xh, Xm, nullptr, nullptr, e5, last_of(e4, 7));
  sp_segment<S, FSEG_L6>(c, fr, acc, Yh, Ym, nullptr, nullptr, e6, last_of(e5, 7));
  sp_segment<S, FSEG_L7>(c, fr, acc, Xh, Xm, nullptr, nullptr, e7, last_of(e6, 7));
  float spre = 0.f;
  auto sig_epi = [&](int part, int ph, const f32x16& A, EpiTmp&) { if (part == 0 && ph == 0) spre = A[0]; };
  sp_segment<S, FSEG_SIG>(c, fr, acc, Yh, Ym, nullptr, nullptr, nothing_f, last_of(e7, 7));
  sp_segment<S, FSEG_DIR>(c, fr, acc, gd_hi, gd_mid, Yh, Ym, ec, sig_epi);
  if (SAVE && valid && h == 0) a.spre[a.row0 + m] = spre;
  if (valid && h == 0) a.sigma[m] = fabsf(spre);
  sp_segment<S, FSEG_COL>(c, fr, acc, Xh, Xm, nullptr, nullptr, nothing_f, last_of(ec, 3));
  if (valid && h == 0) {
    a.rgb[(size_t)m * 3 + 0] = 1.0f / (1.0f + expf(-acc[1][0]));
    a.rgb[(size_t)m * 3 + 1] = 1.0f / (1.0f + expf(-acc[1][1]));
    a.rgb[(size_t)m * 3 + 2] = 1.0f / (1.0f + expf(-acc[1][2]));
  }
}

__global__ __launch_bounds__(256) void k_pack_weights_split(const Weights24 w, const float* __restrict__ fold, unsigned char* __restrict__ img) {
  const int gid = blockIdx.x * 256 + threadIdx.x;
  if (gid < BF_NFRAG * 64) {
    const int step = gid >> 6, lane = gid & 63;
    const FragHiMid v = frag_lane_split<32, bf_weight>(w, fold, step, lane);
    unsigned char* dst = img + BF_BIAS_BYTES + (size_t)(2 * step) * BF_FRAG_BYTES + lane * 16;
    *reinterpret_cast<u32x4*>(dst) = v.hi;
    *reinterpret_cast<u32x4*>(dst + BF_FRAG_BYTES) = v.mid;
  } else {
    const int b = gid - BF_NFRAG * 64;
    if (b < BF_BIAS_BYTES / 4) {
      const int tile = b >> 5, i = b & 31;
      reinterpret_cast<float*>(img)[b] = tile < BF_NBIAS_TILES ? bf_bias(w, fold, tile, i) : 0.f;
    }
  }
}

size_t split_image_bytes() { return (size_t)BF_BIAS_BYTES + (size_t)SP_NFRAG * BF_FRAG_BYTES; }

hipError_t launch_pack_weights_split(const Weights24& w, const float* fold, unsigned char* img, hipStream_t st) {
  const int threads = BF_NFRAG * 64 + BF_BIAS_BYTES / 4;
  hipLaunchKernelGGL(k_pack_weights_split, dim3((threads + 255) / 256), dim3(256), 0, st, w, fold, img);
  return hipGetLastError();
}

hipError_t launch_field_fwd_split(const FieldArgs& a, bool save, hipStream_t st) {
  static std::atomic<unsigned long long> opted{0}, opted_save{0};
  int wgs = (a.M + SP_WG / 2 - 1) / (SP_WG / 2);
  if (save) wgs = (wgs + 1) / 2 * 2;
  if (save) {
    if (!a.bsave || !a.bsave2 || !a.bmask || !a.spre) return hipErrorInvalidValue;
    if (hipError_t e = ensure_dynamic_lds(opted_save, {reinterpret_cast<const void*>(&k_field_fwd_split<true>)}, BF_LDS_BYTES)) return e;
    hipLaunchKernelGGL(k_field_fwd_split<true>, dim3(wgs), dim3(SP_WG), BF_LDS_BYTES, st, a);
  } else {
    if (hipError_t e = ensure_dynamic_lds(opted, {reinterpret_cast<const void*>(&k_field_fwd_split<false>)}, BF_LDS_BYTES)) return e;
    hipLaunchKernelGGL(k_field_fwd_split<false>, dim3(wgs), dim3(SP_WG), BF_LDS_BYTES, st, a);
  }
  return hipGetLastError();
}

}
```

### nerf-tiny_amd/csrc/kernels.h

```cpp
#pragma once
#include "common.h"

#include <atomic>
#include <initializer_list>

namespace nerf {

inline hipError_t ensure_dynamic_lds(std::atomic<unsigned long long>& mask, std::initializer_list<const void*> kernels, int bytes) {
  int dev = 0;
  hipError_t e = hipGetDevice(&dev);
  if (e != hipSuccess) return e;
  if (dev < 64 && ((mask.load(std::memory_order_relaxed) >> dev) & 1ull)) return hipSuccess;
  for (const void* k : kernels) {
    e = hipFuncSetAttribute(k, hipFuncAttributeMaxDynamicSharedMemorySize, bytes);
    if (e != hipSuccess) return e;
  }
  if (dev < 64) mask.fetch_or(1ull << dev, std::memory_order_relaxed);
  return hipSuccess;
}

constexpr int LDA = 260;
constexpr int FIELD_LDS_FLOATS = TM * LDA + 4 * TM * 3;

struct FieldArgs {
  const float4* wp;
  const unsigned char* wbf;
  unsigned char* bsave;
  unsigned char* bsave2;
  uint16_t* bmask;
  int wb0, wb_tot;
  Weights24 w;
  const float* rayf;
  const float* dvec;
  const float* t;
  float* rgb;
  float* sigma;
  float* pts_dbg;
  float* gp_dbg;
  float* save;
  uint16_t* masks;
  float* spre;
  int row0;
  int tile0;
  int tiles_tot;
  long long Mtot;
  long long MSrows;
  int N;
  int M;
  unsigned long long* stamps;
};

struct QuerySrc {
  const float* points;
  float lo[3], step[3];
  int ny, nz;
  const int* list;
  const long long* nlist;
  int e0;
  int nx, r;
  int ext[3];
  int nby, nbz;
};
constexpr int QUERY_CHUNK = 256 * 4 * 32 * 8;
constexpr int QGRAD_CHUNK = 256 * 4 * 32 * 4;
constexpr int QGRAD_GP = 64, QGRAD_C = 128;

constexpr int S_H0 = 0, S_C = 8, S_GP = 9, NSAVE = 10;
constexpr int G_L0 = 0, G_D = 8, NGRAD = 9;

struct RaysArgs {
  const int64_t* row;
  const int64_t* col;
  const float* pb;
  float K[9];
  int B, Nc;
  float* rayf;
  float* dvec;
  const float* w_dir;
  const float* b_dir;
  const float* b_fold;
  float* t_c;
  float* d_cam;
  float* d_wrd;
  unsigned* status;
};

struct CoarseArgs {
  const float* t_c;
  const float* sigma;
  const float* rgb;
  const float* rayf;
  const float* near_far;
  int B, Nc, Nf;
  int delta0_mode;
  float delta0;
  int ray0_override;
  float near0, far0;
  float* w_c;
  float* C_coarse;
  float* t_f;
  uint32_t* status;
  uint32_t* sticky;
};

struct MergeArgs {
  const float *t_c, *t_f, *sig_c, *sig_f, *rgb_c, *rgb_f;
  int B, Nc, Nf, P;
  float last;
  float* bundle;
  float* w;
  uint16_t* perm;
  float* C_fine;
  int joint;
};

struct FwdFuse {
  int mode;
  CoarseArgs c;
  MergeArgs m;
  const float* C_true;
  const float* C_coarse;
  float *dC_c, *dC_f;
  float* loss_terms;
};
hipError_t launch_pack_weights(const Weights24& w, float* fold, float4* out, int nseg, hipStream_t st);
hipError_t launch_fold_weights(const Weights24& w, float* fold, hipStream_t st);
hipError_t launch_field_fwd(const FieldArgs& a, bool save, hipStream_t st);
hipError_t launch_field_fwd_reg(const FieldArgs& a, bool save, hipStream_t st);
hipError_t launch_query_reg(const FieldArgs& a, const QuerySrc& q, bool rgb, hipStream_t st);
hipError_t launch_query_grad_fwd(const FieldArgs& a, const QuerySrc& q, bool rgb, hipStream_t st);
hipError_t launch_dirs_dvec(const float* dirs, int n, const float* w_dir, const float* b_dir, const float* b_fold, float* dvec, hipStream_t st);
hipError_t launch_field_fwd_bf16(const FieldArgs& a, bool save, hipStream_t st, const FwdFuse* fuse = nullptr);
hipError_t launch_pack_weights_bf16(const Weights24& w, const float* fold, unsigned char* img, hipStream_t st);
hipError_t launch_pack_bias_block_bf16(const Weights24& w, const float* fold, unsigned char* img, hipStream_t st);
hipError_t launch_field_fwd_bf16x(const FieldArgs& a, hipStream_t st);
struct PairArgs {
  const unsigned char* wbf;
  RaysArgs rays;
  int B;
  unsigned gen;
  int ray0_override;
  float near0, far0;
  float last;
  float* C_coarse;
  float* C_fine;
  uint32_t* status;
  uint32_t* sticky;
  float *sig_c, *rgb_c, *w_c, *t_f, *sig_f, *rgb_f;
};
hipError_t launch_render_pair_bf16x(const PairArgs& a, hipStream_t st);
hipError_t launch_pack_weights_bf16x(const Weights24& w, const float* fold, unsigned char* img, hipStream_t st);
size_t split_image_bytes();
size_t split_bwd_image_bytes();
hipError_t launch_pack_weights_split_bwd(const Weights24& w, const float* fold, unsigned char* img, hipStream_t st);
hipError_t launch_pack_weights_split(const Weights24& w, const float* fold, unsigned char* img, hipStream_t st);
hipError_t launch_field_fwd_split(const FieldArgs& a, bool save, hipStream_t st);
hipError_t launch_rays(const RaysArgs& a, hipStream_t st);
constexpr int PREP_READY_WORDS = 256;
hipError_t launch_prep_bf16(const Weights24& w, float* fold, unsigned char* img_fwd, int fwd_form, unsigned char* img_bwd,
                            unsigned* ready, unsigned token, unsigned* sticky, const RaysArgs& rays, hipStream_t st);
hipError_t launch_coarse(const CoarseArgs& a, hipStream_t st, float* maps = nullptr);
size_t merge_lds_bytes(int P);
hipError_t launch_merge(const MergeArgs& a, hipStream_t st, float* maps = nullptr);
hipError_t launch_ray_loss(const float* Cc, const float* Cf, const float* Ct, int B, float* loss, float* dCc, float* dCf, hipStream_t st);

}

namespace nerf {

struct FieldBwdArgs {
  const float4* wp;
  Weights24 w;
  const float* rayf;
  const float* t;
  const float* rgb;
  const float* drgb;
  const float* dsig;
  const float* save;
  const uint16_t* masks;
  const float* spre;
  float* G;
  float* dz;
  float* dspre;
  float* dt;
  const unsigned char* wbf;
  const uint16_t* bmask;
  unsigned char* bG;
  unsigned char* bG2;
  int wb0, wb_tot;
  int row0, tile0, tiles_tot;
  long long Mtot;
  long long MSrows;
  int N, M;
  unsigned long long* stamps;
};

struct DwItem {
  const float* G;
  const float* X;
  const float* sig;
  int nout, nin;
  int nin_real;
  float* dW; int ldw, col0;
  float* db;
  float* dW2;
  float* db2;
  int thin;
  int has_sig;
  float* raysum;
  int ray_nc, ray_nf;
  int rows_c;
  int wg0, nwg;
  long long slab_off;
  unsigned long long* stamps;
};
constexpr int DW_WGS = 256;
constexpr int DW_MAX_ITEMS = 13;
constexpr int DW_GROUP_WGS = 36;
struct DwBatch {
  DwItem item[DW_MAX_ITEMS];
  int n;
  int grouped;
  const float* slabs;
};

struct FoldGradArgs {
  const float* M;
  const float* db_dir;
  const float* w_dir;
  const float* w_pi;
  const float* b_pi;
  float* dW_pi;
  float* db_pi;
  float* dW_dir;
};
hipError_t launch_fold_grads(const FoldGradArgs& a, hipStream_t st);
inline FoldGradArgs fold_grad_args(const Weights24& w, float* const* dw, const float* mbuf) {
// ... 429 lines not shown
```

### nerf-tiny_amd/csrc/prep_parts.h

```cpp
#pragma once
#include "kernels.h"

namespace nerf {

__device__ __forceinline__ void fold_block(const Weights24& w, float* __restrict__ fold, const int block ) {
  __shared__ float4 part_sum[3][64];
  const int t = threadIdx.x;
  if (block == HALF) {
    __shared__ float bsum[HALF];
    const int o = t & (HALF - 1), half = t >> 7;
    const float* dr = w.p[W_DIR] + (size_t)o * (WIDTH + DIR_DIM) + DIR_DIM + half * (WIDTH / 2);
    const float* bp = w.p[B_PI] + half * (WIDTH / 2);
    float s = 0.f;
#pragma unroll 8
    for (int j = 0; j < WIDTH / 2; ++j) s = __builtin_fmaf(dr[j], bp[j], s);
    if (half) bsum[o] = s;
    __syncthreads();
    if (!half) fold[o] = s + bsum[o];
    return;
  }
  const int o = block, k0 = 4 * (t & 63);
  const int part = __builtin_amdgcn_readfirstlane(t >> 6);
  const float* dr = w.p[W_DIR] + (size_t)o * (WIDTH + DIR_DIM) + DIR_DIM + part * (WIDTH / 4);
  const float* pc = w.p[W_PI] + (size_t)part * (WIDTH / 4) * WIDTH + k0;
  float4 acc = make_float4(0.f, 0.f, 0.f, 0.f);
#pragma unroll 8
  for (int j = 0; j < WIDTH / 4; ++j) {
    const float d = dr[j];
    const float4 q = *reinterpret_cast<const float4*>(pc + (size_t)j * WIDTH);
    acc.x = __builtin_fmaf(d, q.x, acc.x);
    acc.y = __builtin_fmaf(d, q.y, acc.y);
    acc.z = __builtin_fmaf(d, q.z, acc.z);
    acc.w = __builtin_fmaf(d, q.w, acc.w);
  }
  if (part) part_sum[part - 1][t & 63] = acc;
  __syncthreads();
  if (part == 0) {
    const float4 p1 = part_sum[0][t], p2 = part_sum[1][t], p3 = part_sum[2][t];
    acc.x = (acc.x + p1.x) + (p2.x + p3.x);
    acc.y = (acc.y + p1.y) + (p2.y + p3.y);
    acc.z = (acc.z + p1.z) + (p2.z + p3.z);
    acc.w = (acc.w + p1.w) + (p2.w + p3.w);
    *reinterpret_cast<float4*>(fold + HALF + (size_t)o * WIDTH + k0) = acc;
  }
}

__device__ __forceinline__ void ray_record(const RaysArgs& a, const int ray, float (&rec)[RAYF]) {
  const float* pb = a.pb + (size_t)ray * 17;
  const float x = (float)a.row[ray], y = (float)a.col[ray];
  float p[3];
#pragma unroll
  for (int j = 0; j < 3; ++j) p[j] = (x * a.K[j] + y * a.K[3 + j]) + a.K[6 + j];
  const float ss = __builtin_fmaf(p[2], p[2], __builtin_fmaf(p[1], p[1], p[0] * p[0]));
  float nrm = (float)sqrt((double)ss);
  nrm = fmaxf(nrm, 1e-12f);
  float d[3], dw[3];
#pragma unroll
  for (int j = 0; j < 3; ++j) d[j] = p[j] / nrm;
#pragma unroll
  for (int c = 0; c < 3; ++c) dw[c] = (pb[5 * c] * d[0] + pb[5 * c + 1] * d[1]) + pb[5 * c + 2] * d[2];
  const float near = pb[15], far = pb[16];
#pragma unroll
  for (int c = 0; c < 3; ++c) {
#pragma unroll
    for (int k = 0; k < 3; ++k) rec[RF_R + 3 * c + k] = pb[5 * c + k];
    rec[RF_O + c] = pb[5 * c + 3];
    rec[RF_DCAM + c] = d[c];
    rec[RF_DWRD + c] = dw[c];
  }
  rec[RF_NEAR] = near;
  rec[RF_FAR] = far;
  rec[RF_STEP] = (far - near) / (float)(a.Nc - 1);
  rec[RF_DELTA] = (far - near) / (float)a.Nc;
  rec[22] = 0.f;
  rec[23] = 0.f;
}
__device__ __forceinline__ float coarse_depth(float near, float far, float step, int i, int Nc) { return (i == Nc - 1) ? far : ((float)i * step + near); }

__device__ __forceinline__ void dvec_block(const float* dw, const float* w_dir, const float* b_dir, const float* b_fold, const int tid,
                                           float* gd, float* out) {
  if (tid < 12) {
    const int c = tid >> 2, l = tid & 3;
    const float ph = dw[c] * __uint_as_float(kFreqDirBits[l]);
    gd[c * 8 + 2 * l] = sinf(ph);
    gd[c * 8 + 2 * l + 1] = cosf(ph);
  }
  __syncthreads();
  const float* wr = w_dir + (size_t)tid * (WIDTH + DIR_DIM);
  float s = b_dir[tid];
#pragma unroll
  for (int k = 0; k < DIR_DIM; ++k) s = __builtin_fmaf(wr[k], gd[k], s);
  if (b_fold) s += b_fold[tid];
  out[tid] = s;
}

__device__ __forceinline__ void ray_block(const RaysArgs& a, const int ray, const int tid, float* gd ) {
  if (a.status && ray == 0 && tid < STATUS_STICKY_WORD) a.status[tid] = 0u;
  float rec[RAYF];
  ray_record(a, ray, rec);
  const float near = rec[RF_NEAR], far = rec[RF_FAR], step = rec[RF_STEP];
  if (tid == 0) {
    if (a.rayf) {
      float* rf = a.rayf + (size_t)ray * RAYF;
#pragma unroll
      for (int k = 0; k < RAYF; ++k) rf[k] = rec[k];
    }
    if (a.d_cam)
      for (int c = 0; c < 3; ++c) a.d_cam[(size_t)ray * 3 + c] = rec[RF_DCAM + c];
    if (a.d_wrd)
      for (int c = 0; c < 3; ++c) a.d_wrd[(size_t)ray * 3 + c] = rec[RF_DWRD + c];
  }
  if (a.t_c) {
    for (int i = tid; i < a.Nc; i += 128) a.t_c[(size_t)ray * a.Nc + i] = coarse_depth(near, far, step, i, a.Nc);
  }
  if (a.dvec) dvec_block(rec + RF_DWRD, a.w_dir, a.b_dir, a.b_fold, tid, gd, a.dvec + (size_t)ray * HALF);
}

}
```

Before: 732,500.

## Precompute per-ray direction encodings in ray prep and specialize point encoding at compile time

The ray-prep kernel now computes each ray's direction positional encoding once, as packed bf16 words (plus hi/mid split words), and stores it in the dvec workspace region. The field kernels load these words instead of recomputing sin/cos of the view direction for every sample. Point-encoding loops are also unrolled with compile-time pair indices, so the frequency and coordinate are picked with selects on literals rather than constant-memory lookups and divisions. This trades per-sample transcendental work and constant loads for an extra global load per sample and a small per-ray write in prep, and it reuses the dvec buffer for a new purpose.

```diff
diff --git a/nerf-tiny_amd/csrc/api.hip b/nerf-tiny_amd/csrc/api.hip
--- a/nerf-tiny_amd/csrc/api.hip
+++ b/nerf-tiny_amd/csrc/api.hip
@@ -295,6 +295,7 @@
   ra.B = B; ra.Nc = Nc;
   ra.rayf = at<float>(ws, L.rayf);
   ra.dvec = (bf16 || split) ? nullptr : at<float>(ws, L.dvec);
+  ra.denc = (bf16 || split) ? at<unsigned>(ws, L.dvec) : nullptr;
   ra.w_dir = w.p[W_DIR]; ra.b_dir = w.p[B_DIR];
   ra.b_fold = at<float>(ws, L.fold);
   ra.t_c = at<float>(ws, L.t_c);
@@ -757,12 +758,14 @@
   memcpy(ra.K, K_inv9, 9 * sizeof(float));
   ra.B = B; ra.Nc = Nl;
   ra.rayf = at<float>(ws, L.rayf);
+  ra.denc = at<unsigned>(ws, L.dvec);
   HIP_TRY(launch_rays(ra, st));
   FieldArgs fa;
   memset(&fa, 0, sizeof(fa));
   fa.wbf = at<unsigned char>(ws, L.packed_bf);
   fa.w = w;
   fa.rayf = at<float>(ws, L.rayf);
+  fa.dvec = at<float>(ws, L.dvec);
   fa.t = t; fa.rgb = rgb; fa.sigma = sigma;
   fa.N = N; fa.M = B * N;
   HIP_TRY(launch_field_fwd_bf16(fa, false, st));
diff --git a/nerf-tiny_amd/csrc/bf16_stream.h b/nerf-tiny_amd/csrc/bf16_stream.h
--- a/nerf-tiny_amd/csrc/bf16_stream.h
+++ b/nerf-tiny_amd/csrc/bf16_stream.h
@@ -236,17 +236,52 @@
   return t;
 }
 
-template <int L>
-__device__ __forceinline__ void encode_pair(const float (&v)[3], const uint32_t (&freq_bits)[L], int pi, float& sv, float& cv) {
+template <bool DIR>
+__device__ constexpr uint32_t freq_lit(int l) {
+  if constexpr (DIR) return kFreqDirLit[l];
+  else return kFreqPointLit[l];
+}
+template <bool DIR, int P0, int NC>
+__device__ __forceinline__ void pair_coord_freq(const float (&v)[3], int sel, float& x, float& f) {
+  constexpr int L = DIR ? 4 : 10;
+  static_assert(P0 >= 0 && P0 < 3 * L, "the first candidate is a real pair");
+  x = v[P0 / L];
+  f = __uint_as_float(freq_lit<DIR>(P0 % L));
+  static_for<NC - 1>([&](auto K) {
+    constexpr int k = K + 1, P = P0 + 2 * k, Q = P - 2;
+    if constexpr (P < 3 * L) {
+      if constexpr (P / L != Q / L) x = sel >= k ? v[P / L] : x;
+      f = sel >= k ? __uint_as_float(freq_lit<DIR>(P % L)) : f;
+    }
+  });
+}
+__device__ __forceinline__ void encode_point_pair_table(const float (&p)[3], int pi, float& sv, float& cv) {
   sv = 0.f;
   cv = 0.f;
-  if (pi < 3 * L) {
-    const int cc = pi / L, l = pi - L * cc;
-    const float x = (cc == 0) ? v[0] : ((cc == 1) ? v[1] : v[2]);
-    sincos_phase(x * __uint_as_float(freq_bits[l]), sv, cv);
-  }
-}
-__device__ __forceinline__ void encode_point_pair(const float (&p)[3], int pi, float& sv, float& cv) { encode_pair(p, kFreqPointBits, pi, sv, cv); }
-__device__ __forceinline__ void encode_dir_pair(const float (&d)[3], int pi, float& sv, float& cv) { encode_pair(d, kFreqDirBits, pi, sv, cv); }
-
-}
+  if (pi < 3 * L_POINT) {
+    const int cc = pi / L_POINT, l = pi - L_POINT * cc;
+    const float x = (cc == 0) ? p[0] : ((cc == 1) ? p[1] : p[2]);
+    sincos_phase(x * __uint_as_float(kFreqPointBits[l]), sv, cv);
+  }
+}
+template <bool DIR, int P0>
+constexpr int pair_pad_from = ((DIR ? 12 : 30) - P0 + 1) / 2;
+template <bool DIR, int P0, int NC>
+__device__ __forceinline__ void encode_pair(const float (&v)[3], int sel, float& sv, float& cv) {
+  constexpr int L = DIR ? 4 : 10;
+  if constexpr (P0 >= 3 * L) {
+    sv = 0.f;
+    cv = 0.f;
+  } else {
+    float x, f;
+    pair_coord_freq<DIR, P0, NC>(v, sel, x, f);
+    sincos_phase(x * f, sv, cv);
+    if constexpr (pair_pad_from<DIR, P0> < NC) {
+      const bool pad = sel >= pair_pad_from<DIR, P0>;
+      sv = pad ? 0.f : sv;
+      cv = pad ? 0.f : cv;
+    }
+  }
+}
+
+}
diff --git a/nerf-tiny_amd/csrc/common.h b/nerf-tiny_amd/csrc/common.h
--- a/nerf-tiny_amd/csrc/common.h
+++ b/nerf-tiny_amd/csrc/common.h
@@ -19,6 +19,9 @@
 constexpr int RAYF = 24;
 
 enum { RF_R = 0, RF_O = 9, RF_DCAM = 12, RF_DWRD = 15, RF_NEAR = 18, RF_FAR = 19, RF_STEP = 20, RF_DELTA = 21 };
+
+constexpr int DENC_X = 0, DENC_T_HI = 16, DENC_T_MID = 32, DENC_WORDS = 48;
+static_assert(DENC_WORDS <= HALF, "the row fits the ray's part of the dvec region");
 
 struct Seg { int off4; int nft; int kb; };
 constexpr int SEG_L0 = 0, SEG_L1 = 1, SEG_L2 = 2, SEG_L3 = 3, SEG_L4A = 4, SEG_L4B = 5, SEG_L5 = 6, SEG_L6 = 7,
@@ -43,7 +46,9 @@
 #define NERF_FREQ_POINT_BITS 0x40490fdbu, 0x40d928aeu, 0x416a8b6cu, 0x41fd527bu, 0x4288cd33u, 0x4313c0fau, 0x439f953cu, 0x442c5befu, 0x44ba2881u, 0x45490fdbu
 __device__ __constant__ const uint32_t kFreqPointBits[10] = {NERF_FREQ_POINT_BITS};
 constexpr uint32_t kFreqPointLit[10] = {NERF_FREQ_POINT_BITS};
-__device__ __constant__ const uint32_t kFreqDirBits[4] = {0x40490fdbu, 0x40fd527au, 0x419f953cu, 0x42490fdbu};
+#define NERF_FREQ_DIR_BITS 0x40490fdbu, 0x40fd527au, 0x419f953cu, 0x42490fdbu
+__device__ __constant__ const uint32_t kFreqDirBits[4] = {NERF_FREQ_DIR_BITS};
+constexpr uint32_t kFreqDirLit[4] = {NERF_FREQ_DIR_BITS};
 
 enum { W_L0 = 0, B_L0 = 1, W_SIGMA = 16, B_SIGMA = 17, W_PI = 18, B_PI = 19, W_DIR = 20, B_DIR = 21, W_COLOR = 22, B_COLOR = 23 };
 
diff --git a/nerf-tiny_amd/csrc/field_bwd_bf16.hip b/nerf-tiny_amd/csrc/field_bwd_bf16.hip
--- a/nerf-tiny_amd/csrc/field_bwd_bf16.hip
+++ b/nerf-tiny_amd/csrc/field_bwd_bf16.hip
@@ -151,22 +151,27 @@
     float p[3];
     sample_point(rf, a.t[mcl], p);
     float dp[3] = {0.f, 0.f, 0.f};
-#pragma unroll
-    for (int g8 = 0; g8 < 8; ++g8)
-#pragma unroll
-      for (int e = 0; e < 2; ++e) {
-        const int pi = 4 * g8 + 2 * h_e + e;
-        if (pi < 30) {
-          const int cc = pi / 10, l = pi - 10 * cc;
-          const float x = (cc == 0) ? p[0] : ((cc == 1) ? p[1] : p[2]);
-          const float fl = __uint_as_float(kFreqPointBits[l]);
-          float sn, cn;
-          sincos_phase(x * fl, sn, cn);
-          const float dgs = dgp[g8 >> 2][4 * (g8 & 3) + 2 * e], dgc = dgp[g8 >> 2][4 * (g8 & 3) + 2 * e + 1];
-          const float contrib = fl * (cn * dgs - sn * dgc);
-          if (cc == 0) dp[0] += contrib; else if (cc == 1) dp[1] += contrib; else dp[2] += contrib;
+    static_for<16>([&](auto I) {
+      constexpr int g8 = I / 2, e = I % 2, pa = 4 * g8 + e, pb = pa + 2;
+      constexpr bool pad = pb >= 30;
+      constexpr int ca = pa / 10, cb = pad ? ca : pb / 10;
+      float x, fl;
+      pair_coord_freq<false, pa, 2>(p, h_e, x, fl);
+      float sn, cn;
+      sincos_phase(x * fl, sn, cn);
+      const float dgs = dgp[g8 >> 2][4 * (g8 & 3) + 2 * e], dgc = dgp[g8 >> 2][4 * (g8 & 3) + 2 * e + 1];
+      const float contrib = fl * (cn * dgs - sn * dgc);
+      if constexpr (!pad && ca == cb) {
+        dp[ca] += contrib;
+      } else {
+        const float ta = dp[ca] + contrib;
+        if constexpr (!pad) {
+          const float tb = dp[cb] + contrib;
+          dp[cb] = h_e ? tb : dp[cb];
         }
-      }
+        dp[ca] = h_e ? dp[ca] : ta;
+      }
+    });
 #pragma unroll
     for (int i = 0; i < 3; ++i) dp[i] += __shfl_xor(dp[i], 32);
     if (valid_e && h_e == 0) {
diff --git a/nerf-tiny_amd/csrc/field_bwd_reg.hip b/nerf-tiny_amd/csrc/field_bwd_reg.hip
--- a/nerf-tiny_amd/csrc/field_bwd_reg.hip
+++ b/nerf-tiny_amd/csrc/field_bwd_reg.hip
@@ -1,8 +1,18 @@
 #include "field_common.h"
+#include <utility>
 
 namespace nerf {
 
 constexpr int RMB = 32;
+
+template <class F, int... I>
+__device__ __forceinline__ void static_for_impl(F&& f, std::integer_sequence<int, I...>) {
+  (f(std::integral_constant<int, I>{}), ...);
+}
+template <int N, class F>
+__device__ __forceinline__ void static_for(F&& f) {
+  static_for_impl(f, std::make_integer_sequence<int, N>{});
+}
 
 template <int NFT>
 struct WStageB {
@@ -282,20 +292,26 @@
 #pragma unroll
     for (int g8 = 0; g8 < 8; ++g8) gq[g8] = *reinterpret_cast<const float4*>(gprow + 8 * g8);
     float dp[3] = {0.f, 0.f, 0.f};
-#pragma unroll
-    for (int g8 = 0; g8 < 8; ++g8)
-#pragma unroll
-      for (int e = 0; e < 2; ++e) {
-        const int pi = 4 * g8 + 2 * h_e + e;
-        if (pi < 30) {
-          const int c = pi / 10, l = pi - 10 * c;
-          const float fl = __uint_as_float(kFreqPointBits[l]);
-          const float sn = e == 0 ? gq[g8].x : gq[g8].z, cn = e == 0 ? gq[g8].y : gq[g8].w;
-          const float dgs = accg[g8 >> 2][4 * (g8 & 3) + 2 * e], dgc = accg[g8 >> 2][4 * (g8 & 3) + 2 * e + 1];
-          const float contrib = fl * (cn * dgs - sn * dgc);
-          if (c == 0) dp[0] += contrib; else if (c == 1) dp[1] += contrib; else dp[2] += contrib;
+    static_for<16>([&](auto I) __attribute__((always_inline)) {
+      constexpr int g8 = I / 2, e = I % 2, pa = 4 * g8 + e, pb = pa + 2;
+      constexpr bool pad = pb >= 30;
+      constexpr int ca = pa / 10, la = pa - 10 * ca, cb = pad ? ca : pb / 10, lb = pad ? la : pb - 10 * cb;
+      constexpr uint32_t fa = kFreqPointLit[la], fb = kFreqPointLit[lb];
+      const float fl = h_e ? __uint_as_float(fb) : __uint_as_float(fa);
+      const float sn = e == 0 ? gq[g8].x : gq[g8].z, cn = e == 0 ? gq[g8].y : gq[g8].w;
+      const float dgs = accg[g8 >> 2][4 * (g8 & 3) + 2 * e], dgc = accg[g8 >> 2][4 * (g8 & 3) + 2 * e + 1];
+      const float contrib = fl * (cn * dgs - sn * dgc);
+      if constexpr (!pad && ca == cb) {
+        dp[ca] += contrib;
+      } else {
+        const float ta = dp[ca] + contrib;
+        if constexpr (!pad) {
+          const float tb = dp[cb] + contrib;
+          dp[cb] = h_e ? tb : dp[cb];
         }
-      }
+        dp[ca] = h_e ? dp[ca] : ta;
+      }
+    });
 #pragma unroll
     for (int c = 0; c < 3; ++c) dp[c] += __shfl_xor(dp[c], 32);
     if (QUERY && valid_e && h_e == 0) {
diff --git a/nerf-tiny_amd/csrc/field_bwd_split.hip b/nerf-tiny_amd/csrc/field_bwd_split.hip
--- a/nerf-tiny_amd/csrc/field_bwd_split.hip
+++ b/nerf-tiny_amd/csrc/field_bwd_split.hip
@@ -138,22 +138,27 @@
     float p[3];
     sample_point(rf, a.t[mcl], p);
     float dp[3] = {0.f, 0.f, 0.f};
-#pragma unroll
-    for (int g8 = 0; g8 < 8; ++g8)
-#pragma unroll
-      for (int e = 0; e < 2; ++e) {
-        const int pi = 4 * g8 + 2 * h_e + e;
-        if (pi < 30) {
-          const int cc = pi / 10, l = pi - 10 * cc;
-          const float x = (cc == 0) ? p[0] : ((cc == 1) ? p[1] : p[2]);
-          const float fl = __uint_as_float(kFreqPointBits[l]);
-          float sn, cn;
-          sincos_phase(x * fl, sn, cn);
-          const float dgs = dgp[g8 >> 2][4 * (g8 & 3) + 2 * e], dgc = dgp[g8 >> 2][4 * (g8 & 3) + 2 * e + 1];
-          const float contrib = fl * (cn * dgs - sn * dgc);
-          if (cc == 0) dp[0] += contrib; else if (cc == 1) dp[1] += contrib; else dp[2] += contrib;
+    static_for<16>([&](auto I) {
+      constexpr int g8 = I / 2, e = I % 2, pa = 4 * g8 + e, pb = pa + 2;
+      constexpr bool pad = pb >= 30;
+      constexpr int ca = pa / 10, cb = pad ? ca : pb / 10;
+      float x, fl;
+      pair_coord_freq<false, pa, 2>(p, h_e, x, fl);
+      float sn, cn;
+      sincos_phase(x * fl, sn, cn);
+      const float dgs = dgp[g8 >> 2][4 * (g8 & 3) + 2 * e], dgc = dgp[g8 >> 2][4 * (g8 & 3) + 2 * e + 1];
+      const float contrib = fl * (cn * dgs - sn * dgc);
+      if constexpr (!pad && ca == cb) {
+        dp[ca] += contrib;
+      } else {
+        const float ta = dp[ca] + contrib;
+        if constexpr (!pad) {
+          const float tb = dp[cb] + contrib;
+          dp[cb] = h_e ? tb : dp[cb];
         }
+        dp[ca] = h_e ? dp[ca] : ta;
       }
+    });
 #pragma unroll
     for (int i = 0; i < 3; ++i) dp[i] += __shfl_xor(dp[i], 32);
     if (valid_e && h_e == 0) {
diff --git a/nerf-tiny_amd/csrc/field_fwd_bf16.hip b/nerf-tiny_amd/csrc/field_fwd_bf16.hip
--- a/nerf-tiny_amd/csrc/field_fwd_bf16.hip
+++ b/nerf-tiny_amd/csrc/field_fwd_bf16.hip
@@ -24,6 +24,7 @@
 template <bool SAVE, int WAVES>
 __global__ __launch_bounds__(64 * WAVES, 1) void k_field_fwd_bf16(const FieldArgs a, const FwdFuse fz) {
   extern __shared__ __attribute__((aligned(16))) unsigned char lds[];
+  constexpr bool LITERAL_ENCODE = !(SAVE && WAVES == 8);
   const BfCtx c = bf_ctx(a.wbf, lds);
   const int lane = c.lane, j = lane & 31, h = lane >> 5;
   const int m = blockIdx.x * (32 * WAVES) + c.wv * 32 + j;
@@ -32,33 +33,29 @@
   const int ray = mc / a.N;
 
   const float* rf = a.rayf + (size_t)ray * RAYF;
-  float p[3], dw[3];
+  float p[3];
   sample_point(rf, a.t[mc], p);
-#pragma unroll
-  for (int i = 0; i < 3; ++i) dw[i] = rf[RF_DWRD + i];
-#pragma unroll
-  for (int i = 0; i < 3; ++i) asm volatile("" : "+v"(p[i]), "+v"(dw[i]));
+  u32x4 gd[2];
+#pragma unroll
+  for (int ks = 0; ks < 2; ++ks) gd[ks] = *reinterpret_cast<const u32x4*>(a.dvec + (size_t)ray * HALF + DENC_T_HI + 8 * ks + 4 * h);
+#pragma unroll
+  for (int i = 0; i < 3; ++i) asm volatile("" : "+v"(p[i]));
+#pragma unroll
+  for (int ks = 0; ks < 2; ++ks) asm volatile("" : "+v"(gd[ks]));
 
   using S = std::conditional_t<WAVES == 4, FourWaves<FwdStream<SAVE>>, FwdStream<SAVE>>;
   bf_stream_start<S>(c);
 
-  u32x4 gp[4], gd[2];
-#pragma unroll
-  for (int ks = 0; ks < 4; ++ks)
-#pragma unroll
-    for (int q = 0; q < 4; ++q) {
-      float sv, cv;
-      encode_point_pair(p, 8 * ks + 2 * h + (q & 1) + 4 * (q >> 1), sv, cv);
-      gp[ks][q] = pack2(sv, cv);
-    }
-#pragma unroll
-  for (int ks = 0; ks < 2; ++ks)
-#pragma unroll
-    for (int q = 0; q < 4; ++q) {
-      float sv, cv;
-      encode_dir_pair(dw, 8 * ks + 2 * h + (q & 1) + 4 * (q >> 1), sv, cv);
-      gd[ks][q] = pack2(sv, cv);
-    }
+  u32x4 gp[4];
+  static_for<16>([&](auto I) {
+    constexpr int ks = I / 4, q = I % 4;
+    float sv, cv;
+    if constexpr (LITERAL_ENCODE)
+      encode_pair<false, 8 * ks + (q & 1) + 4 * (q >> 1), 2>(p, h, sv, cv);
+    else
+      encode_point_pair_table(p, 8 * ks + 2 * h + (q & 1) + 4 * (q >> 1), sv, cv);
+    gp[ks][q] = pack2(sv, cv);
+  });
 
   const int wb = a.wb0 + blockIdx.x * WAVES + c.wv;
   unsigned mw[4];
diff --git a/nerf-tiny_amd/csrc/field_fwd_bf16x.hip b/nerf-tiny_amd/csrc/field_fwd_bf16x.hip
--- a/nerf-tiny_amd/csrc/field_fwd_bf16x.hip
+++ b/nerf-tiny_amd/csrc/field_fwd_bf16x.hip
@@ -70,9 +70,9 @@
   });
 }
 
-template <class S, int NH, class Mid>
-__device__ __forceinline__ void bx_field_pass(const BfCtx& c, unsigned char* lds, const float (&p)[NH][3], const float (&dw)[NH][3], Mid&& mid,
-                                              float (&cpre)[NH][3]) {
+template <class S, int NH, class Park, class Fetch, class Mid>
+__device__ __forceinline__ void bx_field_pass(const BfCtx& c, unsigned char* lds, const float (&p)[NH][3], Park&& park_dirs, Fetch&& fetch_dirs,
+                                              Mid&& mid, float (&cpre)[NH][3]) {
   using Acc = AccN<NH>;
   const int q = c.lane >> 4;
   bf_stream_start<S>(c);
@@ -80,35 +80,14 @@
   u32x4 gp[NH][8], gd[NH][8];
 #pragma unroll
   for (int h = 0; h < NH; ++h) {
-#pragma unroll
-    for (int s = 0; s < 2; ++s)
-#pragma unroll
-      for (int e = 0; e < 4; ++e) {
-        const int pi = 16 * s + 8 * (e >> 1) + 2 * q + (e & 1);
-        float sv = 0.f, cv = 0.f;
-        if (pi < 30) {
-          const int cc = pi / 10, l = pi - 10 * cc;
-          const float x = (cc == 0) ? p[h][0] : ((cc == 1) ? p[h][1] : p[h][2]);
-          sincos_phase(x * __uint_as_float(kFreqPointBits[l]), sv, cv);
-        }
-        gp[h][s][e] = pack2(sv, cv);
-      }
-#pragma unroll
-    for (int e = 0; e < 4; ++e) {
-      const int pi = 8 * (e >> 1) + 2 * q + (e & 1);
-      float sv = 0.f, cv = 0.f;
-      if (pi < 12) {
-        const int cc = pi / 4, l = pi - 4 * cc;
-        const float x = (cc == 0) ? dw[h][0] : ((cc == 1) ? dw[h][1] : dw[h][2]);
-        sincos_phase(x * __uint_as_float(kFreqDirBits[l]), sv, cv);
-      }
-      gd[h][0][e] = pack2(sv, cv);
-    }
-  }
-
-  u32x4* const gd_park = reinterpret_cast<u32x4*>(lds + BF_LDS_BYTES) + NH * (c.wv * 64 + c.lane);
-#pragma unroll
-  for (int h = 0; h < NH; ++h) gd_park[h] = gd[h][0];
+    static_for<8>([&](auto I) {
+      constexpr int s = I / 4, e = I % 4;
+      float sv, cv;
+      encode_pair<false, 16 * s + 8 * (e >> 1) + (e & 1), 4>(p[h], q, sv, cv);
+      gp[h][s][e] = pack2(sv, cv);
+    });
+  }
+  park_dirs(reinterpret_cast<u32x4*>(lds + BF_LDS_BYTES));
 
   u32x4 fr[BF_D];
   bf_stream_first<S>(c, fr);
@@ -149,9 +128,8 @@
   bx_segment<S, NH, BXS_SIG, 1, 8, 0, BXB_SIGMA, 0, BXB_DIR>(c, fr, acc, Y, nullptr, nothing_f, last_of(relu_to(Y), 15));
   {
     const int lane_d = __builtin_amdgcn_mbcnt_hi(~0u, __builtin_amdgcn_mbcnt_lo(~0u, 0u));
-    const u32x4* const back = reinterpret_cast<const u32x4*>(lds + BF_LDS_BYTES) + NH * (c.wv * 64 + lane_d);
-#pragma unroll
-    for (int h = 0; h < NH; ++h) gd[h][0] = back[h];
+#pragma unroll
+    for (int h = 0; h < NH; ++h) gd[h][0] = fetch_dirs(reinterpret_cast<const u32x4*>(lds + BF_LDS_BYTES), h, lane_d);
   }
   bx_segment<S, NH, BXS_DIR, 8, 1, 8, BXB_DIR, 1, BXB_COL>(c, fr, acc, gd, Y, relu_to(X), sig_epi);
   mid(spre);
@@ -172,24 +150,31 @@
 
   int ms[NH];
   bool valid[NH];
-  float p[NH][3], dw[NH][3];
+  float p[NH][3];
+  u32x4 gdr[NH];
 #pragma unroll
   for (int h = 0; h < NH; ++h) {
     ms[h] = m0 + 16 * h + n;
     valid[h] = ms[h] < a.M;
     const int mc = valid[h] ? ms[h] : a.M - 1;
-    const float* rf = a.rayf + (size_t)(mc / a.N) * RAYF;
-    sample_point(rf, a.t[mc], p[h]);
-#pragma unroll
-    for (int i = 0; i < 3; ++i) dw[h][i] = rf[RF_DWRD + i];
-  }
-#pragma unroll
-  for (int h = 0; h < NH; ++h)
-#pragma unroll
-    for (int i = 0; i < 3; ++i) asm volatile("" : "+v"(p[h][i]), "+v"(dw[h][i]));
+    const int ray = mc / a.N;
+    sample_point(a.rayf + (size_t)ray * RAYF, a.t[mc], p[h]);
+    gdr[h] = *reinterpret_cast<const u32x4*>(a.dvec + (size_t)ray * HALF + DENC_X + 4 * (lane >> 4));
+  }
+#pragma unroll
+  for (int h = 0; h < NH; ++h) {
+#pragma unroll
+    for (int i = 0; i < 3; ++i) asm volatile("" : "+v"(p[h][i]));
+    asm volatile("" : "+v"(gdr[h]));
+  }
 
   float cpre[NH][3];
-  bx_field_pass<S, NH>(c, lds, p, dw, [&](const float (&spre)[NH]) {
+  auto park = [&](u32x4* area) {
+#pragma unroll
+    for (int h = 0; h < NH; ++h) area[NH * (c.wv * 64 + c.lane) + h] = gdr[h];
+  };
+  auto fetch = [&](const u32x4* area, int h, int lane_d) { return area[NH * (c.wv * 64 + lane_d) + h]; };
+  bx_field_pass<S, NH>(c, lds, p, park, fetch, [&](const float (&spre)[NH]) {
     const int lane_e = __builtin_amdgcn_mbcnt_hi(~0u, __builtin_amdgcn_mbcnt_lo(~0u, 0u));
     const int n_e = lane_e & 15;
     const bool q0_e = lane_e < 16;
@@ -255,6 +240,18 @@
   lds = d.lds;
   return d;
 }
+__device__ __forceinline__ unsigned pair_dir_word(const float (&dw)[3], int j) {
+  const int q = j >> 2, e = j & 3, pi = 8 * (e >> 1) + 2 * q + (e & 1);
+  const int cc = pi / L_DIR, l = pi - L_DIR * cc;
+  const float x = (cc == 0) ? dw[0] : ((cc == 1) ? dw[1] : dw[2]);
+  float f = __uint_as_float(kFreqDirLit[0]);
+  static_for<L_DIR - 1>([&](auto K) { f = l == K + 1 ? __uint_as_float(kFreqDirLit[K + 1]) : f; });
+  float sv, cv;
+  sincos_phase(x * f, sv, cv);
+  return pi < 3 * L_DIR ? pack2(sv, cv) : 0u;
+}
+__device__ __forceinline__ u32x4 pair_fetch_dirs(const BfCtx& c, const u32x4* area, int lane_d) { return area[4 * (c.wv >> 2) + (lane_d >> 4)]; }
+
 __device__ __forceinline__ void pair_coarse_pass(const PairArgs& a, const BfCtx& c, unsigned char* lds, const int r0) {
   float* const res = reinterpret_cast<float*>(lds);
   {
@@ -270,7 +267,14 @@
 #pragma unroll
     for (int k = 0; k < 3; ++k) asm volatile("" : "+v"(p[0][k]), "+v"(dw[0][k]));
     float cpre[1][3];
-    bx_field_pass<BxStream, 1>(c, lds, p, dw, [&](const float (&spre)[1]) {
+    auto park = [&](u32x4* area) {
+      if ((c.wv & 3) == 0) {
+        const unsigned word = pair_dir_word(dw[0], c.lane & 15);
+        if (c.lane < 16) reinterpret_cast<unsigned*>(area)[16 * (c.wv >> 2) + c.lane] = word;
+      }
+    };
+    auto fetch = [&](const u32x4* area, int, int lane_d) { return pair_fetch_dirs(c, area, lane_d); };
+    bx_field_pass<BxStream, 1>(c, lds, p, park, fetch, [&](const float (&spre)[1]) {
       const int le = lane_id_builtin();
       if (le < 16) res[PR_SIGC + 16 * c.wv + le] = fabsf(spre[0]);
     }, cpre);
@@ -287,7 +291,7 @@
   float* const res = reinterpret_cast<float*>(lds);
   {
     const int n = c.lane & 15;
-    float p[2][3], dw[2][3];
+    float p[2][3];
 #pragma unroll
     for (int h = 0; h < 2; ++h) {
       const int s = 32 * c.wv + 16 * h + n, rl = s >> 7;
@@ -295,15 +299,14 @@
       float rf[RAYF];
       ray_record(a.rays, ray, rf);
       sample_point(rf, res[PR_TF + s], p[h]);
-#pragma unroll
-      for (int k = 0; k < 3; ++k) dw[h][k] = rf[RF_DWRD + k];
     }
 #pragma unroll
     for (int h = 0; h < 2; ++h)
 #pragma unroll
-      for (int k = 0; k < 3; ++k) asm volatile("" : "+v"(p[h][k]), "+v"(dw[h][k]));
+      for (int k = 0; k < 3; ++k) asm volatile("" : "+v"(p[h][k]));
     float cpre[2][3];
-    bx_field_pass<BxStreamNoBias, 2>(c, lds, p, dw, [&](const float (&spre)[2]) {
+    auto fetch = [&](const u32x4* area, int, int lane_d) { return pair_fetch_dirs(c, area, lane_d); };
+    bx_field_pass<BxStreamNoBias, 2>(c, lds, p, [](u32x4*) {}, fetch, [&](const float (&spre)[2]) {
       const int le = lane_id_builtin();
       if (le < 16) {
 #pragma unroll
diff --git a/nerf-tiny_amd/csrc/field_fwd_split.hip b/nerf-tiny_amd/csrc/field_fwd_split.hip
--- a/nerf-tiny_amd/csrc/field_fwd_split.hip
+++ b/nerf-tiny_amd/csrc/field_fwd_split.hip
@@ -33,36 +33,30 @@
   const int ray = mc / a.N;
 
   const float* rf = a.rayf + (size_t)ray * RAYF;
-  float p[3], dw[3];
+  float p[3];
   sample_point(rf, a.t[mc], p);
+  u32x4 gd_hi[2], gd_mid[2];
 #pragma unroll
-  for (int i = 0; i < 3; ++i) dw[i] = rf[RF_DWRD + i];
+  for (int ks = 0; ks < 2; ++ks) {
+    gd_hi[ks] = *reinterpret_cast<const u32x4*>(a.dvec + (size_t)ray * HALF + DENC_T_HI + 8 * ks + 4 * h);
+    gd_mid[ks] = *reinterpret_cast<const u32x4*>(a.dvec + (size_t)ray * HALF + DENC_T_MID + 8 * ks + 4 * h);
+  }
 #pragma unroll
-  for (int i = 0; i < 3; ++i) asm volatile("" : "+v"(p[i]), "+v"(dw[i]));
+  for (int i = 0; i < 3; ++i) asm volatile("" : "+v"(p[i]));
+#pragma unroll
+  for (int ks = 0; ks < 2; ++ks) asm volatile("" : "+v"(gd_hi[ks]), "+v"(gd_mid[ks]));
 
   bf_stream_start<S>(c);
 
-  u32x4 gp_hi[4], gp_mid[4], gd_hi[2], gd_mid[2];
-#pragma unroll
-  for (int ks = 0; ks < 4; ++ks)
-#pragma unroll
-    for (int q = 0; q < 4; ++q) {
-      float sv, cv;
-      encode_point_pair(p, 8 * ks + 2 * h + (q & 1) + 4 * (q >> 1), sv, cv);
-      const HiMid e = split2(sv, cv);
-      gp_hi[ks][q] = e.hi;
-      gp_mid[ks][q] = e.mid;
-    }
-#pragma unroll
-  for (int ks = 0; ks < 2; ++ks)
-#pragma unroll
-    for (int q = 0; q < 4; ++q) {
-      float sv, cv;
-      encode_dir_pair(dw, 8 * ks + 2 * h + (q & 1) + 4 * (q >> 1), sv, cv);
-      const HiMid e = split2(sv, cv);
-      gd_hi[ks][q] = e.hi;
-      gd_mid[ks][q] = e.mid;
-    }
+  u32x4 gp_hi[4], gp_mid[4];
+  static_for<16>([&](auto I) {
+    constexpr int ks = I / 4, q = I % 4;
+    float sv, cv;
+    encode_pair<false, 8 * ks + (q & 1) + 4 * (q >> 1), 2>(p, h, sv, cv);
+    const HiMid e = split2(sv, cv);
+    gp_hi[ks][q] = e.hi;
+    gp_mid[ks][q] = e.mid;
+  });
 
   const int wb = a.wb0 + blockIdx.x * (SP_WG / 64) + c.wv;
   unsigned mw[4];
diff --git a/nerf-tiny_amd/csrc/kernels.h b/nerf-tiny_amd/csrc/kernels.h
--- a/nerf-tiny_amd/csrc/kernels.h
+++ b/nerf-tiny_amd/csrc/kernels.h
@@ -83,6 +83,7 @@
   float* d_cam;
   float* d_wrd;
   unsigned* status;
+  unsigned* denc;
 };
 
 struct CoarseArgs {
diff --git a/nerf-tiny_amd/csrc/prep_parts.h b/nerf-tiny_amd/csrc/prep_parts.h
--- a/nerf-tiny_amd/csrc/prep_parts.h
+++ b/nerf-tiny_amd/csrc/prep_parts.h
@@ -1,5 +1,6 @@
 #pragma once
 #include "kernels.h"
+#include "bf16_split.h"
 
 namespace nerf {
 
@@ -94,6 +95,22 @@
   out[tid] = s;
 }
 
+__device__ __forceinline__ void denc_block(const float (&dw)[3], const int tid, unsigned* row) {
+  if (tid >= DENC_WORDS) return;
+  const int part = tid >> 4, j = tid & 15;
+  const int pi = part == 0 ? 8 * ((j >> 1) & 1) + 2 * (j >> 2) + (j & 1) : 8 * (j >> 3) + 2 * ((j >> 2) & 1) + (j & 1) + 4 * ((j >> 1) & 1);
+  unsigned word = 0u;
+  if (pi < 3 * L_DIR) {
+    const int c = pi / L_DIR, l = pi - L_DIR * c;
+    const float x = (c == 0) ? dw[0] : ((c == 1) ? dw[1] : dw[2]);
+    float sv, cv;
+    sincos_phase(x * __uint_as_float(kFreqDirBits[l]), sv, cv);
+    const HiMid e = split2(sv, cv);
+    word = part == 2 ? e.mid : e.hi;
+  }
+  row[tid] = word;
+}
+
 __device__ __forceinline__ void ray_block(const RaysArgs& a, const int ray, const int tid, float* gd ) {
   if (a.status && ray == 0 && tid < STATUS_STICKY_WORD) a.status[tid] = 0u;
   float rec[RAYF];
@@ -114,6 +131,10 @@
     for (int i = tid; i < a.Nc; i += 128) a.t_c[(size_t)ray * a.Nc + i] = coarse_depth(near, far, step, i, a.Nc);
   }
   if (a.dvec) dvec_block(rec + RF_DWRD, a.w_dir, a.b_dir, a.b_fold, tid, gd, a.dvec + (size_t)ray * HALF);
+  if (a.denc) {
+    const float dw[3] = {rec[RF_DWRD], rec[RF_DWRD + 1], rec[RF_DWRD + 2]};
+    denc_block(dw, tid, a.denc + (size_t)ray * HALF);
+  }
 }
 
 }
```

New measurement: 732,500 (median of 2 runs). About the same (+0.0%).
